# yumcyaWiz/fredholm

Measured on AMD Instinct MI355X. Metric: Msamples/s at 1920x1080, max_depth=8, higher is better.
Workload: dtype f32; 1 GPU; configs[2]: 1M random-triangle soup (PCG32 seed 0x853c49e6748fea9b), Hosek sky turbidity 3 albedo 0.3, 1920x1080, max_depth 8, seed 1; triangles=1000000, parallelism=single GPU, gather=none, post=none

## Files before the change

fredholm_amd/csrc/capi.hip:

```cpp
#include <hip/hip_runtime.h>

#include <cmath>
#include <cstdlib>
#include <cstring>

#include "../../include/fredholm/image_io.h"
#include <hip/hip_gl_interop.h>

#include "context.h"
#include "fh_bsdf.h"
#include "fh_trace.h"

#include "gen/tables.inc"

namespace fh {

static thread_local std::string g_create_error;

int fail(fh_ctx* ctx, int code, const std::string& msg)
{
  g_create_error = msg;
  if (ctx) ctx->err = msg;
  if (ctx && ctx->owner) ctx->owner->err = "member " + std::to_string(ctx->member_index) + ": " + msg;
  return code;
// ... 342 lines not shown
          for (uint32_t x = bx; x < bx + blk && x < x0 + tw && x < width; ++x) { owned.push_back(x + width * y); if (owned_xy) owned_xy->push_back(x | (y << 16)); }
  }
}

int rebuild_ownership(fh_ctx* ctx)
{
  if (ctx->d_owned) { (void)hipFree(ctx->d_owned); ctx->d_owned = nullptr; }
  if (ctx->d_owned_xy) { (void)hipFree(ctx->d_owned_xy); ctx->d_owned_xy = nullptr; }
  ctx->n_owned = 0;
  if (ctx->width == 0 || ctx->height == 0) return FH_OK;
  if (ctx->width > 65535u || ctx->height > 65535u) return fail(ctx, FH_E_UNSUPPORTED, "frames wider or higher than 65535 pixels are not supported");
  std::vector<uint32_t> owned, owned_xy;
  owned_list(ctx->width, ctx->height, ctx->tile_w, ctx->tile_h, ctx->shard_rank, ctx->shard_world, owned, &owned_xy);
  ctx->n_owned = (uint32_t)owned.size();
  FH_HIP(hipMalloc((void**)&ctx->d_owned, owned.empty() ? 16 : owned.size() * 4));
  FH_HIP(hipMalloc((void**)&ctx->d_owned_xy, owned.empty() ? 16 : owned.size() * 4));
  if (!owned.empty()) FH_HIP(hipMemcpy(ctx->d_owned, owned.data(), owned.size() * 4, hipMemcpyHostToDevice));
  if (!owned.empty()) FH_HIP(hipMemcpy(ctx->d_owned_xy, owned_xy.data(), owned_xy.size() * 4, hipMemcpyHostToDevice));
  return FH_OK;
}

}

int frame_map_ensure(fh_ctx* ctx, uint32_t world)
{
  fh_ctx::FrameMap& fm = ctx->frame_map;
  if (!(fm.d_all && fm.world == world && fm.width == ctx->width && fm.height == ctx->height && fm.tile_w == ctx->tile_w && fm.tile_h == ctx->tile_h)) {
    (void)hipStreamSynchronize(ctx->stream);
    if (fm.d_all) (void)hipFree(fm.d_all);
    fm = fh_ctx::FrameMap{};
    std::vector<uint32_t> all;
    fm.start.assign(world + 1u, 0u);
    for (uint32_t r = 0; r < world; ++r) { owned_list(ctx->width, ctx->height, ctx->tile_w, ctx->tile_h, r, world, all, nullptr); fm.start[r + 1u] = (uint32_t)all.size(); }
    FH_HIP(hipMalloc((void**)&fm.d_all, all.empty() ? 16 : all.size() * 4));
    if (!all.empty()) FH_HIP(hipMemcpy(fm.d_all, all.data(), all.size() * 4, hipMemcpyHostToDevice));
    fm.world = world; fm.width = ctx->width; fm.height = ctx->height; fm.tile_w = ctx->tile_w; fm.tile_h = ctx->tile_h;
  }
  return FH_OK;
}

uint32_t owned_count(uint32_t width, uint32_t height, uint32_t tw, uint32_t th, uint32_t rank, uint32_t world)
{
  std::vector<uint32_t> owned;
  owned_list(width, height, tw, th, rank, world, owned, nullptr);
  return (uint32_t)owned.size();
}

namespace {

__global__ void k_pack(const float* layer, const uint32_t* owned, uint32_t n, uint32_t fpp, float* packed)
{
  for (uint32_t i = blockIdx.x * blockDim.x + threadIdx.x; i < n * fpp; i += gridDim.x * blockDim.x) packed[i] = layer[(size_t)owned[i / fpp] * fpp + i % fpp];
}
__global__ void k_unpack(const float* packed, const uint32_t* owned, uint32_t n, uint32_t fpp, float* layer)
{
  for (uint32_t i = blockIdx.x * blockDim.x + threadIdx.x; i < n * fpp; i += gridDim.x * blockDim.x) layer[(size_t)owned[i / fpp] * fpp + i % fpp] = packed[i];
}
struct ShardSources { const float* packed[kMaxShardsPerLaunch]; uint32_t start[kMaxShardsPerLaunch + 1]; uint32_t world; };
__global__ void k_unpack_all(ShardSources src, const uint32_t* all_owned, uint32_t n, uint32_t fpp, float* layer)
{
  for (uint32_t i = blockIdx.x * blockDim.x + threadIdx.x; i < n * fpp; i += gridDim.x * blockDim.x) {
    const uint32_t j = i / fpp, c = i % fpp;
    uint32_t r = 0;
    while (r + 1u < src.world && j >= src.start[r + 1u]) ++r;
    layer[(size_t)all_owned[j] * fpp + c] = src.packed[r][(size_t)(j - src.start[r]) * fpp + c];
  }
}

}
}

using namespace fh;

#define CTX_CHECK(ctx)                      \
  if (!(ctx)) return FH_E_INVALID;          \
  if (hipSetDevice((ctx)->device) != hipSuccess) return fh::fail(ctx, FH_E_HIP, "hipSetDevice failed")

namespace fh {
uint64_t pool_bytes_per_path(const fh_ctx* ctx)
{
  const uint32_t sec = 2u + (ctx->has_dir ? 1u : 0u) + (ctx->n_lights > 0 ? 1u : 0u);
  const uint32_t classes = ctx->n_classes < 1u ? 1u : ctx->n_classes;
  return 64u + 16u + 8u + 4u + 64u + 48u * sec + (ctx->n_lights > 0 ? 32u : 0u) + 20u + 4u + 4u + 4u * classes;
}
}

extern "C" {

int fh_ctx_create(int device, fh_ctx** out)
{
  if (!out) return FH_E_INVALID;
  *out = nullptr;
  int n_dev = 0;
  if (hipGetDeviceCount(&n_dev) != hipSuccess || n_dev <= 0) { g_create_error = "no HIP device available: the fredholm HIP path has no CPU fallback"; return FH_E_HIP; }
  if (device < 0 || device >= n_dev) { g_create_error = "device index out of range"; return FH_E_INVALID; }
  if (hipSetDevice(device) != hipSuccess) { g_create_error = "hipSetDevice failed"; return FH_E_HIP; }
  fh_ctx* ctx = new fh_ctx;
  ctx->device = device;
  auto bail = [&](const char* what) { g_create_error = what; delete ctx; return FH_E_HIP; };
  auto make_stream = [&](hipStream_t* s) { return hipStreamCreateWithFlags(s, hipStreamNonBlocking); };
  if (make_stream(&ctx->stream) != hipSuccess) return bail("hipStreamCreate failed");
  if (hipMalloc((void**)&ctx->d_sobol, kSobolMatricesBytes) != hipSuccess) return bail("hipMalloc failed");
  if (hipMalloc((void**)&ctx->d_lut_refl, kLutReflectionBytes) != hipSuccess) return bail("hipMalloc failed");
  if (hipMalloc((void**)&ctx->d_lut_sheen, kLutSheenBytes) != hipSuccess) return bail("hipMalloc failed");
  if (hipMalloc((void**)&ctx->d_trace_counters, 32 * sizeof(unsigned long long)) != hipSuccess) return bail("hipMalloc failed");
  if (hipMalloc((void**)&ctx->d_hosek, sizeof(fh::HosekSky)) != hipSuccess || hipMemsetAsync(ctx->d_hosek, 0, sizeof(fh::HosekSky), ctx->stream) != hipSuccess) return bail("hipMalloc failed");
  if (hipMemcpy(ctx->d_sobol, kSobolMatrices, kSobolMatricesBytes, hipMemcpyHostToDevice) != hipSuccess) return bail("table upload failed");
  {
    std::vector<uint32_t> bytes((size_t)1024 * 4 * 256);
    const uint32_t* mat = kSobolMatrices;
    for (uint32_t dim = 0; dim < 1024u; ++dim)
      for (uint32_t k = 0; k < 4u; ++k) {
        uint32_t* t = &bytes[((size_t)dim * 4 + k) * 256];
        t[0] = 0u;
        for (uint32_t b = 1; b < 256u; ++b) t[b] = t[b & (b - 1u)] ^ mat[dim * 52u + 8u * k + (uint32_t)__builtin_ctz(b)];
      }
    if (hipMalloc((void**)&ctx->d_sobol_bytes, bytes.size() * sizeof(uint32_t)) != hipSuccess) return bail("hipMalloc failed");
    if (hipMemcpy(ctx->d_sobol_bytes, bytes.data(), bytes.size() * sizeof(uint32_t), hipMemcpyHostToDevice) != hipSuccess) return bail("table upload failed");
  }
  if (hipMemcpy(ctx->d_lut_refl, kLutReflection, kLutReflectionBytes, hipMemcpyHostToDevice) != hipSuccess) return bail("table upload failed");
  if (hipMemcpy(ctx->d_lut_sheen, kLutSheen, kLutSheenBytes, hipMemcpyHostToDevice) != hipSuccess) return bail("table upload failed");
  (void)hipMemsetAsync(ctx->d_trace_counters, 0, 32 * sizeof(unsigned long long), ctx->stream);
  for (int k = 0; k < 2; ++k)
    if (make_stream(&ctx->aux_stream[k]) != hipSuccess) return bail("hipStreamCreate failed");
  for (int k = 0; k < 3; ++k) {
    (void)hipHostMalloc((void**)&ctx->h_counters[k], sizeof(uint32_t) * fh::kCounterStride * 66);
    (void)hipEventCreate(&ctx->ev_counters[k]);
    (void)hipEventCreateWithFlags(&ctx->ev_gen[k], hipEventDisableTiming);
    (void)hipEventCreateWithFlags(&ctx->ev_acc[k], hipEventDisableTiming);
  }
  (void)hipEventCreateWithFlags(&ctx->ev_enter, hipEventDisableTiming);
  if (const char* e = getenv("FH_PIPELINE")) ctx->n_slots = e[0] == '0' ? 1 : (e[0] == '2' ? 2 : 3);
  {
    fh_ctx::Tunables& t = ctx->tun;
    hipDeviceProp_t prop;
    if (hipGetDeviceProperties(&prop, device) == hipSuccess && prop.multiProcessorCount > 0) t.n_cus = (uint32_t)prop.multiProcessorCount;
    int v = 0;
    if (hipDeviceGetAttribute(&v, hipDeviceAttributeMaxSharedMemoryPerMultiprocessor, device) == hipSuccess && v >= 64 * 1024) t.lds_per_cu = (uint32_t)v;
    if (hipDeviceGetAttribute(&v, hipDeviceAttributeSharedMemPerBlockOptin, device) == hipSuccess && v >= 64 * 1024) t.lds_per_block = (uint32_t)v;
    if (t.lds_per_block > t.lds_per_cu) t.lds_per_block = t.lds_per_cu;
    auto env_uint = [](const char* name, int lo, int hi, uint32_t& dst) { if (const char* e = getenv(name)) { const int v = atoi(e); if (v >= lo && v <= hi) dst = (uint32_t)v; } };
    auto env_off = [](const char* name, bool& dst) { if (const char* e = getenv(name)) dst = e[0] != '0'; };
    env_uint("FH_COOP_T", 1, 64, t.coop_flush);
    t.coop_flush_fixed = getenv("FH_COOP_T") != nullptr;
    env_off("FH_COOP", t.coop);
    env_off("FH_STREAM", t.stream);
    t.stream_forced = t.stream && getenv("FH_STREAM") != nullptr;
    env_uint("FH_STREAM_REFILL", 1, 64, t.stream_refill);
    env_uint("FH_STREAM_MIN_RAYS", 0, 65535, t.stream_min_rays);
    env_off("FH_SORT_SMALL", t.sort_small);
    env_off("FH_OVERLAP", t.overlap_secondary);
    env_off("FH_MERGE", t.merge_trace);
    env_uint("FH_SKY_BLOCKS", 0, 64, t.sky_blocks_per_cu);
    if (const char* e = getenv("FH_POISON")) t.poison_pools = e[0] == '1';
    env_off("FH_SKY_SPLIT", t.sky_split);
    env_uint("FH_SKY_SPLIT_MIN_LOG2", 0, 40, t.sky_split_min_log2);
    env_uint("FH_STACK_LDS", 1, 99, t.stack_lds_entries);
    env_uint("FH_SHADE_WGS", 2, 3, t.shade_wgs);
    env_uint("FH_STREAM_CHUNK", 16, 65535, t.stream_chunk);
    t.stream_chunk_fixed = getenv("FH_STREAM_CHUNK") != nullptr;
    if (t.stream_chunk_fixed) t.stream_chunk_closest = t.stream_chunk;
    env_uint("FH_STREAM_CHUNK_CLOSEST", 16, 65535, t.stream_chunk_closest);
    env_uint("FH_TAIL_DEPTH", 0, 64, t.tail_depth);
    env_uint("FH_TAIL_PATHS", 64, 1 << 30, t.tail_paths);
    env_off("FH_SORT", t.sort_queues);
    env_uint("FH_SORT_ONEPASS", 0, 2, t.sort_onepass);
    env_uint("FH_BOTTOM_UP", 0, 2, t.bottom_up);
    t.debug_tail = getenv("FH_DEBUG_TAIL") != nullptr;
    if (const char* e = getenv("FH_FORCE_ALPHA")) t.force_alpha = e[0] == '1';
  }
  {
    int least = 0, greatest = 0;
    const char* e = getenv("FH_SKY_PRIO");
    const bool low = !(e && e[0] == '0') && hipDeviceGetStreamPriorityRange(&least, &greatest) == hipSuccess;
    if ((low ? hipStreamCreateWithPriority(&ctx->sky_stream, hipStreamNonBlocking, least) : hipStreamCreateWithFlags(&ctx->sky_stream, hipStreamNonBlocking)) != hipSuccess) return bail("hipStreamCreate failed");
  }
  (void)hipEventCreateWithFlags(&ctx->ev_sky, hipEventDisableTiming);
  if (hipMalloc((void**)&ctx->d_split_counters, 16) != hipSuccess) return bail("hipMalloc failed");
  (void)hipMemsetAsync(ctx->d_split_counters, 0, 16, ctx->stream);
  (void)hipEventCreate(&ctx->ev_render_begin);
  (void)hipEventCreate(&ctx->ev_render_end);
  if (hipStreamSynchronize(ctx->stream) != hipSuccess) return bail("hipStreamSynchronize failed");
  *out = ctx;
  return FH_OK;
}

int fh_ctx_destroy(fh_ctx* ctx)
{
  FH_GROUP(ctx, group_destroy(ctx));
  if (!ctx) return FH_E_INVALID;
  (void)hipSetDevice(ctx->device);
  (void)hipStreamSynchronize(ctx->stream);
  pool_release(ctx);
  void* ptrs[] = {ctx->d_sample_issued, ctx->d_sobol, ctx->d_sobol_bytes, ctx->d_alpha_rec, ctx->d_lut_refl, ctx->d_lut_sheen, ctx->d_face_rec, ctx->d_face_cls, ctx->d_materials, ctx->d_lights, ctx->d_bvh2_nodes, ctx->d_bvh2_tris,
                  ctx->d_bvh8_nodes, ctx->d_bvh8_tris, ctx->d_sample_count, ctx->d_owned, ctx->d_trace_counters, ctx->d_texels, ctx->d_textures, ctx->d_srgb_lut, ctx->d_ibl,
                  ctx->d_bloom_weights, ctx->d_quirk_seen, ctx->d_quirk_aov, ctx->d_obj_vertices, ctx->d_obj_normals, ctx->d_obj_texcoords, ctx->d_obj_indices, ctx->d_face_meta, ctx->d_o2w, ctx->d_w2o,
                  ctx->d_bvh8_box, ctx->d_denoise_tmp[0], ctx->d_denoise_tmp[1], ctx->d_hosek, ctx->d_owned_xy, ctx->d_stack_spill, ctx->d_bvh8_parent, ctx->d_face_node,
                  ctx->d_moments, ctx->d_active[0], ctx->d_active[1], ctx->d_active[2], ctx->d_active[3], ctx->d_block_marks, ctx->d_active_blocks, ctx->d_sky_taken, ctx->d_sky_adaptive};
  for (void* p : ptrs)
    if (p) (void)hipFree(p);
  for (fh_ctx::ShardList& c : ctx->shard_lists)
    if (c.d_owned) (void)hipFree(c.d_owned);
  if (ctx->frame_map.d_all) (void)hipFree(ctx->frame_map.d_all);
  for (int k = 0; k < 4; ++k) if (ctx->d_split[k]) (void)hipFree(ctx->d_split[k]);
  if (ctx->d_split_counters) (void)hipFree(ctx->d_split_counters);
  if (ctx->h_active_count) (void)hipHostFree(ctx->h_active_count);
  if (ctx->sky_stream) { (void)hipStreamSynchronize(ctx->sky_stream); (void)hipStreamDestroy(ctx->sky_stream); }
  if (ctx->ev_sky) (void)hipEventDestroy(ctx->ev_sky);
  for (auto& s : ctx->spans) { (void)hipEventDestroy(s.a); (void)hipEventDestroy(s.b); }
  for (auto e : ctx->event_pool) (void)hipEventDestroy(e);
  for (auto e : ctx->ev_bounce) (void)hipEventDestroy(e);
  for (int k = 0; k < 3; ++k) {
  }
  for (int k = 0; k < 3; ++k) {
    if (ctx->h_counters[k]) (void)hipHostFree(ctx->h_counters[k]);
    (void)hipEventDestroy(ctx->ev_counters[k]);
    (void)hipEventDestroy(ctx->ev_gen[k]);
    (void)hipEventDestroy(ctx->ev_acc[k]);
  }
  (void)hipEventDestroy(ctx->ev_enter);
  for (int k = 0; k < 2; ++k) (void)hipStreamDestroy(ctx->aux_stream[k]);
  (void)hipEventDestroy(ctx->ev_render_begin);
  (void)hipEventDestroy(ctx->ev_render_end);
  (void)hipStreamDestroy(ctx->stream);
  delete ctx;
  return FH_OK;
}

const char* fh_last_error(fh_ctx* ctx) { return ctx ? ctx->err.c_str() : g_create_error.c_str(); }

int fh_set_flags(fh_ctx* ctx, uint32_t flags)
{
  FH_GROUP_EACH(ctx, kGroupCallPlain, fh_set_flags(m_, flags));
  CTX_CHECK(ctx);
  ctx->flags = flags;
  return FH_OK;
}
int fh_get_flags(fh_ctx* ctx, uint32_t* flags)
{
  FH_GROUP_LEAD(ctx);
  CTX_CHECK(ctx);
  if (!flags) return fail(ctx, FH_E_INVALID, "fh_get_flags: null argument");
  *flags = ctx->flags;
  return FH_OK;
}

int fh_set_path_pool(fh_ctx* ctx, uint32_t target)
{
  FH_GROUP_EACH(ctx, kGroupCallFrame, fh_set_path_pool(m_, target));
  CTX_CHECK(ctx);
  if (target == 0) return fail(ctx, FH_E_INVALID, "fh_set_path_pool: zero");
  (void)hipStreamSynchronize(ctx->stream);
  pool_release(ctx);
  ctx->pool_target = target;
  ctx->pool_target_by_caller = true;
  return FH_OK;
}

int fh_path_pool_bytes(fh_ctx* ctx, uint64_t* bytes_per_path, uint32_t* pools)
{
  FH_GROUP_LEAD(ctx);
  CTX_CHECK(ctx);
  if (!bytes_per_path || !pools) return fail(ctx, FH_E_INVALID, "fh_path_pool_bytes: null argument");
  *bytes_per_path = pool_bytes_per_path(ctx);
  *pools = (uint32_t)ctx->n_slots;
  return FH_OK;
}

int fh_kat_face_classes(fh_ctx* ctx, uint8_t* out, uint32_t n)
{
  FH_GROUP_REFUSE(ctx, "fh_kat_face_classes");
  CTX_CHECK(ctx);
  if (!out || n != ctx->n_faces) return fail(ctx, FH_E_INVALID, "fh_kat_face_classes: one byte per face of the uploaded scene");
  if (n) FH_HIP(hipMemcpy(out, ctx->d_face_cls, n, hipMemcpyDeviceToHost));
  return FH_OK;
}

int fh_alpha_face_counts(fh_ctx* ctx, uint32_t counts[4])
{
  FH_GROUP_LEAD(ctx);
  CTX_CHECK(ctx);
  if (!counts) return fail(ctx, FH_E_INVALID, "fh_alpha_face_counts: null argument");
  for (int k = 0; k < 4; ++k) counts[k] = ctx->alpha_face_counts[k];
  return FH_OK;
}

int fh_alpha_cell_counts(fh_ctx* ctx, uint64_t counts[3])
{
  FH_GROUP_LEAD(ctx);
  CTX_CHECK(ctx);
  if (!counts) return fail(ctx, FH_E_INVALID, "fh_alpha_cell_counts: null argument");
  for (int k = 0; k < 3; ++k) counts[k] = ctx->alpha_cell_counts[k];
  return FH_OK;
}

int fh_kat_alpha_records(fh_ctx* ctx, uint32_t* out, uint32_t n_faces)
{
  FH_GROUP_REFUSE(ctx, "fh_kat_alpha_records");
  CTX_CHECK(ctx);
  if (!out || n_faces != ctx->n_faces) return fail(ctx, FH_E_INVALID, "fh_kat_alpha_records: 32 words per face of the uploaded scene");
  if (!ctx->d_alpha_rec) { std::memset(out, 0, 128ull * n_faces); return FH_OK; }
  FH_HIP(hipMemcpy(out, ctx->d_alpha_rec, 128ull * n_faces, hipMemcpyDeviceToHost));
  return FH_OK;
}

int fh_path_pool_allocated(fh_ctx* ctx, uint64_t* bytes, uint64_t* paths)
{
  FH_GROUP(ctx, group_path_pool_allocated(ctx, bytes, paths));
  CTX_CHECK(ctx);
  if (!bytes || !paths) return fail(ctx, FH_E_INVALID, "fh_path_pool_allocated: null argument");
  *bytes = 0; *paths = 0;
  for (int k = 0; k < 3; ++k) { *bytes += ctx->pool_alloc_bytes[k]; *paths += ctx->pool[k].capacity; }
  return FH_OK;
}

int fh_set_tail_depth(fh_ctx* ctx, uint32_t depth)
{
  FH_GROUP_EACH(ctx, kGroupCallPlain, fh_set_tail_depth(m_, depth));
  CTX_CHECK(ctx);
  ctx->tail_depth = depth;
  return FH_OK;
}

int fh_scene_upload(fh_ctx* ctx, const fh_scene_desc* s)
{
  FH_GROUP_EACH(ctx, kGroupCallUpload, fh_scene_upload(m_, s));
  CTX_CHECK(ctx);
  if (!s || !s->vertices || !s->normals || !s->texcoords || !s->indices || !s->material_ids || !s->materials || s->n_materials == 0)
    return fail(ctx, FH_E_INVALID, "fh_scene_upload: missing arrays");
  for (uint32_t i = 0; i < s->n_materials; ++i) {
    const fh_material& m = s->materials[i];
    const int32_t ids[11] = {m.base_color_texture_id, m.specular_color_texture_id, m.specular_roughness_texture_id, m.metalness_texture_id, m.metallic_roughness_texture_id, m.coat_texture_id,
                             m.coat_roughness_texture_id, m.emission_texture_id, m.heightmap_texture_id, m.normalmap_texture_id, m.alpha_texture_id};
    for (int32_t id : ids)
      if (id < -1 || id >= (int32_t)s->n_textures) return fail(ctx, FH_E_INVALID, "fh_scene_upload: material references a texture id outside [0, n_textures)");
  }
  if (s->n_textures && !s->textures) return fail(ctx, FH_E_INVALID, "fh_scene_upload: n_textures > 0 but textures == NULL");
  {
    const int rc = upload_textures(ctx, s->n_textures, s->textures);
    if (rc) return rc;
  }
  ctx->h_vertices.assign(s->vertices, s->vertices + 3ull * s->n_vertices);
  ctx->h_normals.assign(s->normals, s->normals + 3ull * s->n_vertices);
  ctx->h_texcoords.assign(s->texcoords, s->texcoords + 2ull * s->n_vertices);
  ctx->h_indices.assign(s->indices, s->indices + 3ull * s->n_faces);
  ctx->h_material_ids.assign(s->material_ids, s->material_ids + s->n_faces);
  if (s->instance_ids) ctx->h_instance_ids.assign(s->instance_ids, s->instance_ids + s->n_faces);
  else ctx->h_instance_ids.clear();
  ctx->h_materials.assign(s->materials, s->materials + s->n_materials);
  if (s->n_instances && s->object_to_world && s->world_to_object) {
    ctx->h_o2w.assign(s->object_to_world, s->object_to_world + 12ull * s->n_instances);
    ctx->h_w2o.assign(s->world_to_object, s->world_to_object + 12ull * s->n_instances);
  } else {
    ctx->h_o2w.assign(kIdentity12, kIdentity12 + 12);
    ctx->h_w2o.assign(kIdentity12, kIdentity12 + 12);
  }
  const int rc = rebuild_device_scene(ctx);
  if (rc) return rc;
  ctx->scene_loaded = true;
  ctx->builder_choice = 0;
  return FH_OK;
// ... 580 lines not shown
```

fredholm_amd/csrc/context.h:

```cpp
#pragma once
#include <hip/hip_runtime.h>

#include <functional>
#include <string>
#include <vector>

#include "../../include/fredholm_hip.h"
#include "fh_device.h"

struct fh_group;

struct fh_ctx {
  fh_group* group = nullptr;
  fh_ctx* owner = nullptr;
  uint32_t member_index = 0;
  int device = 0;
  hipStream_t stream = nullptr;
  hipStream_t aux_stream[2] = {nullptr, nullptr};
  std::string err;
  uint32_t flags = 0;

  uint32_t* d_sobol = nullptr;
  uint32_t* d_sobol_bytes = nullptr;
  float* d_lut_refl = nullptr;
  float* d_lut_sheen = nullptr;

  std::vector<float> h_vertices, h_normals, h_texcoords;
  std::vector<uint32_t> h_indices, h_material_ids, h_instance_ids;
  std::vector<fh_material> h_materials;
  std::vector<float> h_o2w, h_w2o;
  bool scene_loaded = false, bvh_valid = false;

  float4* d_face_rec = nullptr;
  uint8_t* d_face_cls = nullptr;
  fh::MaterialDev* d_materials = nullptr;
  fh::AreaLightDev* d_lights = nullptr;
  float* d_obj_vertices = nullptr;
  float* d_obj_normals = nullptr;
  float* d_obj_texcoords = nullptr;
  uint32_t* d_obj_indices = nullptr;
  uint2* d_face_meta = nullptr;
  float4* d_o2w = nullptr;
  float4* d_w2o = nullptr;
  uint32_t n_xf_alloc = 0;
  std::vector<uint8_t> h_tex_alpha_cuts, h_tex_red_cuts;
  std::vector<fht_texture> h_tex_desc;
  struct HostTexture { uint32_t width = 0, height = 0, srgb = 0; std::vector<uint8_t> rgba8; };
  std::vector<HostTexture> h_tex_host;
  unsigned long long alpha_cell_counts[3] = {0, 0, 0};
  uint32_t alpha_face_counts[4] = {0, 0, 0, 0};
  uint4* d_alpha_rec = nullptr;
  uint8_t* d_texels = nullptr;
  fht_texture* d_textures = nullptr;
  float* d_srgb_lut = nullptr;
  uint32_t n_textures = 0;
  bool has_alpha = false;
  float* d_ibl = nullptr;
  uint32_t ibl_w = 0, ibl_h = 0;
  uint32_t n_faces = 0, n_lights = 0, n_materials = 0;
  uint32_t n_classes = 0;
  uint32_t class_lobes[fh::kMaxClasses] = {};

  float4* d_bvh2_nodes = nullptr;
  float4* d_bvh2_tris = nullptr;
  uint32_t bvh2_n_nodes = 0, bvh2_n_tris = 0;
  uint4* d_bvh8_nodes = nullptr;
  float4* d_bvh8_tris = nullptr;
  uint32_t bvh8_n_nodes = 0, bvh8_n_tris = 0;
  uint32_t* d_bvh8_parent = nullptr;
  uint32_t* d_face_node = nullptr;
  float4* d_bvh8_box = nullptr;
  std::vector<uint32_t> bvh8_level_start;
  bool refit_ok = false;
  double bvh8_area_built = 0.0;
  uint32_t n_refits = 0;
  uint32_t bvh8_depth = 0;
  uint32_t occupancy_key = 0xffffffffu, occupancy_blocks = 0, occupancy_blocks_secondary = 0;
  uint32_t info_blocks[2] = {0, 0}, info_entries[2] = {0, 0};
  uint32_t lds_configured_bytes = 0;
  uint32_t stream_lds_entries = 0, stream_lds_entries_secondary = 0;
  uint2* d_stack_spill = nullptr;
  size_t stack_spill_capacity = 0;
  uint32_t lds_static_max = 0;
  bool use_bvh8 = false;
  int builder_choice = 0;
  double bvh_build_ms = 0.0;
  float scene_lo[3] = {0, 0, 0}, scene_hi[3] = {0, 0, 0};

  uint32_t width = 0, height = 0;
  uint32_t* d_sample_count = nullptr;
  uint32_t* d_sample_issued = nullptr;
  uint32_t shard_rank = 0, shard_world = 1, tile_w = 32, tile_h = 32;
  uint32_t* d_owned = nullptr;
  uint32_t* d_owned_xy = nullptr;
  uint32_t n_owned = 0;
  uint32_t* d_split[4] = {nullptr, nullptr, nullptr, nullptr};
  uint32_t split_capacity = 0, n_wave_px = 0, n_sky_px = 0;
  uint32_t* d_split_counters = nullptr;
  bool split_valid = false;
  float split_key[32] = {};
  hipStream_t sky_stream = nullptr;
  hipEvent_t ev_sky = nullptr;
  struct ShardList { uint32_t rank, world, width, height, tile_w, tile_h; uint32_t* d_owned; uint32_t n_owned; };
  struct FrameMap { uint32_t world = 0, width = 0, height = 0, tile_w = 0, tile_h = 0; uint32_t* d_all = nullptr; std::vector<uint32_t> start; };
  FrameMap frame_map;
  std::vector<ShardList> shard_lists;
  bool adaptive = false;
  fh_adaptive_params adapt{};
  float2* d_moments = nullptr;
  bool accumulated = false;
  uint32_t adapt_total = 0;
  uint32_t* d_active[4] = {nullptr, nullptr, nullptr, nullptr};
  uint32_t* d_active_blocks = nullptr;
  uint32_t active_capacity = 0;
  uint32_t* h_active_count = nullptr;
  uint32_t adapt_block = 1, adapt_growth = 1;
  uint32_t* d_block_marks = nullptr;
  size_t marks_capacity = 0;
  uint32_t mark_seq = 0;
  unsigned long long* d_sky_taken = nullptr;
  bool sky_taken_pending = false;
  void* d_sky_adaptive = nullptr;

  bool has_dir = false;
  float dir_le[3] = {0, 0, 0}, dir_dir[3] = {0, 1, 0}, dir_angle = 0;
  float sky_intensity = 1.0f;
  float sun_dir[3] = {0.0f, 1.0f, 0.0f};
  bool has_hosek = false;
  fh::HosekSky hosek{};
  fh::HosekSky* d_hosek = nullptr;

  fh::PoolDev pool[3] = {};
  struct PoolShape { bool dir = false, lights = false; uint32_t classes = 0; };
  PoolShape pool_shape[3];
  std::vector<void*> pool_allocs[3];
  unsigned long long pool_alloc_bytes[3] = {0, 0, 0};
  uint32_t pool_target_default = 1u << 25, pool_target = 1u << 25;
  bool pool_target_by_caller = false;
  uint32_t pool_share = 1;
  uint32_t tail_depth = 0;
  uint32_t auto_wave_depth = 2;
  double survival[66] = {};
  uint32_t survival_n = 0;
  uint32_t* h_counters[3] = {nullptr, nullptr, nullptr};
  hipEvent_t ev_counters[3] = {nullptr, nullptr, nullptr};
  bool counters_in_flight[3] = {false, false, false};
  uint32_t counters_wave_depth[3] = {0, 0, 0};
  uint32_t counters_paths[3] = {0, 0, 0};
  int counters_bu[3] = {-1, -1, -1};
  int bu_choice = 0;
  uint32_t bu_toggle = 0;
  double bu_cost[2] = {0.0, 0.0}, bu_items[2] = {0.0, 0.0};
  unsigned long long pass_seq = 0;
  hipEvent_t ev_gen[3] = {nullptr, nullptr, nullptr}, ev_acc[3] = {nullptr, nullptr, nullptr}, ev_enter = nullptr;
  bool gen_valid[3] = {false, false, false}, acc_valid[3] = {false, false, false};
  int n_slots = 3;
  int last_slot_used = 0;
  std::vector<hipEvent_t> ev_bounce;
  uint32_t* d_quirk_seen = nullptr;
  float4* d_quirk_aov = nullptr;
  size_t quirk_pixels = 0;

  struct Tunables {
    uint32_t n_cus = 256;
    uint32_t lds_per_cu = 160u * 1024u, lds_per_block = 160u * 1024u;
    uint32_t coop_flush = 48;
    bool coop_flush_fixed = false;
    bool coop = true;
    bool stream = true;
    bool stream_forced = false;
    uint32_t stream_refill = 24;
    uint32_t stream_min_rays = 64;
    bool overlap_secondary = true;
    bool sky_split = true;
    uint32_t sky_split_min_log2 = 27;
    uint32_t sky_blocks_per_cu = 0;
    bool poison_pools = false;
    bool merge_trace = true;
    uint32_t shade_wgs = 0;
    uint32_t stack_lds_entries = 0;
    bool sort_small = false;
    uint32_t stream_chunk = 64;
    bool stream_chunk_fixed = false;
    uint32_t stream_chunk_closest = 128;
    uint32_t tail_depth = 0;
    uint32_t tail_paths = 0;
    uint32_t bottom_up = 2;
    bool sort_queues = true;
    uint32_t sort_onepass = 2;
    bool debug_tail = false;
    bool force_alpha = false;
  } tun;

  float* d_bloom_weights = nullptr;
  float bloom_sigma_cached = -1.0f, bloom_wsum = 0.0f;

  float4* d_denoise_tmp[2] = {nullptr, nullptr};
  size_t denoise_pixels = 0;

  fh_stats stats{};
  unsigned long long* d_trace_counters = nullptr;
  struct TimedSpan { hipEvent_t a, b; int kind; };
  std::vector<TimedSpan> spans;
  std::vector<hipEvent_t> event_pool;
  hipEvent_t ev_render_begin = nullptr, ev_render_end = nullptr;
  bool render_pending = false;
};

namespace fh {
int fail(fh_ctx* ctx, int code, const std::string& msg);
#define FH_HIP(call)                                                                                                   \
  do {                                                                                                                 \
    hipError_t e_ = (call);                                                                                            \
    if (e_ != hipSuccess) return fh::fail(ctx, FH_E_HIP, std::string(#call) + ": " + hipGetErrorString(e_));            \
  } while (0)

#define FH_GROUP(ctx, call) \
  if ((ctx) && (ctx)->group) return fh::call
#define FH_GROUP_EACH(ctx, kind, call) \
  if ((ctx) && (ctx)->group) return fh::group_each(ctx, kind, [&](fh_ctx* m_, uint32_t i_) { (void)i_; return call; })
#define FH_GROUP_LEAD(ctx) \
  if ((ctx) && (ctx)->group) ctx = fh::group_lead(ctx)
#define FH_GROUP_REFUSE(ctx, name) \
  if ((ctx) && (ctx)->group) return fh::fail(ctx, FH_E_UNSUPPORTED, name ": not available on a group (a plain context does hand-rolled gathers and known-answer runs)")
enum { kGroupCallPlain = 0, kGroupCallScene = 1, kGroupCallFrame = 2, kGroupCallUpload = 3 };
fh_ctx* group_lead(fh_ctx* g);
int group_each(fh_ctx* g, int kind, const std::function<int(fh_ctx*, uint32_t)>& call);
int group_destroy(fh_ctx* g);
int group_set_resolution(fh_ctx* g, uint32_t w, uint32_t h);
int group_set_tile_shard(fh_ctx* g, uint32_t rank, uint32_t world, uint32_t tw, uint32_t th);
int group_init_render_states(fh_ctx* g);
int group_render(fh_ctx* g, const fh_camera* cam, const float* bg, const fh_render_layers* layers, uint32_t n_samples, uint32_t max_depth, uint32_t seed);
int group_get_sample_counts(fh_ctx* g, uint32_t* counts);
int group_get_luminance_moments(fh_ctx* g, float* moments);
int group_active_pixel_count(fh_ctx* g, uint32_t* out);
int group_owned_pixel_count(fh_ctx* g, uint32_t* out);
int group_get_stats(fh_ctx* g, fh_stats* out);
int group_path_pool_allocated(fh_ctx* g, uint64_t* bytes, uint64_t* paths);
int frame_map_ensure(fh_ctx* ctx, uint32_t world);
uint32_t owned_count(uint32_t width, uint32_t height, uint32_t tw, uint32_t th, uint32_t rank, uint32_t world);

SceneDev scene_dev(const fh_ctx* ctx);
int bvh_build_device(fh_ctx* ctx);
int render_submit(fh_ctx* ctx, const fh_camera* cam, const float* bg, const fh_render_layers* layers, uint32_t n_samples, uint32_t max_depth, uint32_t seed);
int adaptive_upload(fh_ctx* ctx);
int adaptive_select(fh_ctx* ctx, hipStream_t st, const uint32_t* base_px, const uint32_t* base_xy, uint32_t n_base, uint32_t* n_active, const uint32_t* sky_px = nullptr,
                    const uint32_t* sky_xy = nullptr, uint32_t n_sky = 0, uint32_t* n_sky_active = nullptr);
uint32_t adaptive_to_boundary(const fh_ctx* ctx);
int pool_ensure(fh_ctx* ctx, int slot, uint32_t capacity);
uint64_t pool_bytes_per_path(const fh_ctx* ctx);
void pool_release(fh_ctx* ctx);
int kernel_info(fh_ctx* ctx, int which, uint32_t out[6]);
int post_process_submit(fh_ctx* ctx, const float* in, float* hi, float* tmp, int w, int h, const fh_post_params* pp, float* out);
int denoise_submit(fh_ctx* ctx, int w, int h, const float* beauty, const float* normal, const float* albedo, float* out, int upscale);
}
```

fredholm_amd/csrc/fh_sky.h:

```cpp
#pragma once
#include "../../include/fh_elementary.h"
#include "fh_vec.h"

namespace fh {

struct HosekSky { float cfg[3][9]; float rad[3]; };

inline float hosek_bezier(const float* m, int stride, float e)
{
  const float ie = 1.0f - e;
  return fhe_pow(ie, 5.0f) * m[0] + 5.0f * fhe_pow(ie, 4.0f) * e * m[stride] + 10.0f * fhe_pow(ie, 3.0f) * fhe_pow(e, 2.0f) * m[2 * stride] +
         10.0f * fhe_pow(ie, 2.0f) * fhe_pow(e, 3.0f) * m[3 * stride] + 5.0f * ie * fhe_pow(e, 4.0f) * m[4 * stride] + fhe_pow(e, 5.0f) * m[5 * stride];
}

inline HosekSky hosek_cook(const float* table, float turbidity, float albedo, float elevation)
{
  HosekSky st{};
  const int it = (int)turbidity;
  const float tr = turbidity - (float)it;
  const float e = fhe_pow(elevation / (kPi / 2.0f), (1.0f / 3.0f));
  for (int ch = 0; ch < 3; ++ch) {
    const float* ds = table + 1080 * ch;
    const float* dr = table + 3240 + 120 * ch;
    for (int i = 0; i < 9; ++i) {
      float c = (1.0f - albedo) * (1.0f - tr) * hosek_bezier(ds + 54 * (it - 1) + i, 9, e);
      c += albedo * (1.0f - tr) * hosek_bezier(ds + 540 + 54 * (it - 1) + i, 9, e);
      if (it != 10) {
        c += (1.0f - albedo) * tr * hosek_bezier(ds + 54 * it + i, 9, e);
        c += albedo * tr * hosek_bezier(ds + 540 + 54 * it + i, 9, e);
      }
      st.cfg[ch][i] = c;
    }
    float r = (1.0f - albedo) * (1.0f - tr) * hosek_bezier(dr + 6 * (it - 1), 1, e);
    r += albedo * (1.0f - tr) * hosek_bezier(dr + 60 + 6 * (it - 1), 1, e);
    if (it != 10) {
      r += (1.0f - albedo) * tr * hosek_bezier(dr + 6 * it, 1, e);
      r += albedo * tr * hosek_bezier(dr + 60 + 6 * it, 1, e);
    }
    st.rad[ch] = r;
  }
  return st;
}

FH_HD f3 hosek_radiance(const HosekSky& st, f3 sun_dir, float intensity, f3 v)
{
  const float theta = fhe_acos(clampf(v.y, -1.0f, 1.0f));
  const float gamma = fhe_acos(dot(sun_dir, v));
  const float cg = fhe_cos(gamma), ct = fhe_cos(theta);
  const float rayM = cg * cg;
  const float zenith = sqrt_cr(ct);
  float out[3];
#pragma unroll
  for (int ch = 0; ch < 3; ++ch) {
    const float* c = st.cfg[ch];
    const float expM = fhe_exp(c[4] * gamma);
    const float mieM = (1.0f + cg * cg) / fhe_pow1p5(1.0f + c[8] * c[8] - 2.0f * c[8] * cg);
    out[ch] = (1.0f + c[0] * fhe_exp(c[1] / (ct + 0.01f))) * (c[2] + c[3] * expM + c[5] * rayM + c[6] * mieM + c[7] * zenith) * st.rad[ch];
  }
  return intensity * mk3(out[0], out[1], out[2]);
}

}
```

fredholm_amd/csrc/render.hip:

```cpp
#include <hip/hip_runtime.h>

#include <cmath>
#include <cstdio>
#include <cstdlib>
#include <cstring>
#include <type_traits>

#include "context.h"
#include "fh_bsdf.h"
#include "fh_tonemap.h"
#include "fh_trace.h"

namespace fh {

namespace {

constexpr int kBlock = 256;
constexpr uint32_t kLutReflFloats = 16 * 16 * 2, kLutSheenFloats = 16 * 16;
constexpr uint32_t kMatLds = 32;
#ifndef FH_SECONDARY_BLOCKS_HEAVY
#define FH_SECONDARY_BLOCKS_HEAVY 5
#endif
#ifndef FH_STREAM_BLOCKS
#define FH_STREAM_BLOCKS 7
#endif
#ifndef FH_STREAM_BLOCKS_ALPHA
#define FH_STREAM_BLOCKS_ALPHA FH_STREAM_BLOCKS
#endif
#ifndef FH_STREAM_BLOCKS_CLOSEST
#define FH_STREAM_BLOCKS_CLOSEST FH_STREAM_BLOCKS
#endif
#ifndef FH_SHADE_BLOCKS
#define FH_SHADE_BLOCKS 2
#endif

template <int N>
struct SobolRows {
  uint32_t m[N][1024];
};

template <int N>
FH_D void load_sobol_rows(SobolRows<N>& rows, const uint32_t* tables, const uint32_t* dims)
{
  static_assert(kBlock == 256, "one uint4 per thread and dimension");
#pragma unroll
  for (int r = 0; r < N; ++r)
    reinterpret_cast<uint4*>(rows.m[r])[threadIdx.x] = reinterpret_cast<const uint4*>(tables + (size_t)(dims[r] & 1023u) * 1024u)[threadIdx.x];
  __syncthreads();
}

FH_D void stage_sky(FrameDev& fr, HosekSky& lds_sky)
{
  if (!fr.has_hosek) return;
  if (threadIdx.x < sizeof(HosekSky) / 4u) reinterpret_cast<float*>(&lds_sky)[threadIdx.x] = reinterpret_cast<const float*>(fr.hosek)[threadIdx.x];
  fr.hosek = &lds_sky;
}

FH_D f3 env_radiance(const FrameDev& fr, f3 d)
{
  if (fr.has_ibl) {
    const float theta = fhe_acos(clampf(d.y, -1.0f, 1.0f));
    float phi = fhe_atan2(d.z, d.x);
    if (phi < 0) phi += 2.0f * kPi;
    float o[4];
    fht_tex2d(&fr.ibl, nullptr, phi / (2.0f * kPi), theta / kPi, o);
    return fr.sky_intensity * mk3(o[0], o[1], o[2]);
  }
  return fr.has_hosek ? hosek_radiance(*fr.hosek, fr.sun_dir, fr.sky_intensity, d) : fr.bg;
}

FH_D bool camera_ray(const FrameDev& fr, const uint32_t* sobol_dim1, uint32_t image_idx, uint32_t px, uint32_t py, uint32_t n_spp, f2 u, f2 u_lens, f3& org, f3& dir);
FH_D bool camera_sample(const FrameDev& fr, const uint32_t* sobol_dim1, uint32_t image_idx, uint32_t px, uint32_t py, uint32_t n_spp, f3& org, f3& dir)
{
  return camera_ray(fr, sobol_dim1, image_idx, px, py, n_spp, cmj_draw(n_spp, image_idx, 0u, fr.seed_hash), cmj_draw(n_spp, image_idx, 1u, fr.seed_hash), org, dir);
}
FH_D bool camera_ray(const FrameDev& fr, const uint32_t* sobol_dim1, uint32_t image_idx, uint32_t px, uint32_t py, uint32_t n_spp, f2 u, f2 u_lens, f3& org, f3& dir)
{
  float uvx = (2.0f * (px + u.x) - fr.width) / fr.height;
  const float uvy = (2.0f * (py + u.y) - fr.height) / fr.height;
  uvx = -uvx;
  u = u_lens;
  const float f = fr.cam_inv_tan;
  const f3 p_sensor = mk3(uvx, uvy, 0.0f);
  const f3 p_lens_center = mk3(0.0f, 0.0f, f);
  const f2 pd = fr.cam_lens_radius * concentric_disk(u);
  const f3 p_lens = p_lens_center + mk3(pd.x, pd.y, 0.0f);
  const f3 s2c = normalize(p_lens_center - p_sensor);
  const f3 p_object = p_sensor + (fr.cam_a_plus_b / s2c.z) * s2c;
  org = xform_point(fr.cam_xf, p_lens);
  f3 d = normalize(p_object - p_lens);
  d.z *= -1.0f;
  dir = xform_dir(fr.cam_xf, d);
  const uint32_t sidx = image_idx + n_spp * fr.width * fr.height;
  const float rr = sobol_draw_bytes(sobol_dim1, sidx, 1u, fr.seed_hash);
  return fr.max_depth > 0 && !(rr >= 1.0f);
}

constexpr int kGenChunks = 4;
__global__ void __launch_bounds__(kBlock) k_generate(FrameDev fr, PoolDev pool, const uint32_t* issued, const uint32_t* owned, const uint32_t* owned_xy, uint32_t n_owned)
{
  __shared__ SobolRows<1> rows;
  __shared__ HosekSky s_sky;
  stage_sky(fr, s_sky);
  const uint32_t dims[1] = {1u};
  load_sobol_rows<1>(rows, fr.sobol_bytes, dims);
  const uint32_t stride = gridDim.x * blockDim.x * kGenChunks;
  const uint32_t k = blockIdx.y;
  __shared__ uint32_t s_reserve[2][5 * kGenChunks];
  uint32_t iter = 0;
  for (uint32_t base = blockIdx.x * blockDim.x * kGenChunks; base < n_owned; base += stride) {
   uint32_t packed = 0u;
   uint32_t* const scratch = s_reserve[iter & 1u];
#pragma unroll 1
   for (int c = 0; c < kGenChunks; ++c) {
    const uint32_t i = base + (uint32_t)c * blockDim.x + threadIdx.x;
    const bool valid = i < n_owned;
    const uint32_t p = k * n_owned + i;
    bool enter = false;
    if (valid) {
      const uint32_t image_idx = owned[i];
      const uint32_t n_spp = issued[image_idx] + k;
      const uint32_t xy = owned_xy[i];
      f3 org, dir;
      const bool alive = camera_sample(fr, rows.m[0], image_idx, xy & 0xffffu, xy >> 16, n_spp, org, dir);
      RayPre rp;
      rp.o = org;
      rp.inv = safe_reciprocal(dir);
      float tn;
      enter = alive && slab_test(rp, fr.scene_lo.x, fr.scene_lo.y, fr.scene_lo.z, fr.scene_hi.x, fr.scene_hi.y, fr.scene_hi.z, 1e9f, tn);
      if (enter) {
        pool.ray_o[p] = mk4(org, 1e9f);
        pool.ray_d[p] = mk4(dir, 0.0f);
        pool.thr[p] = make_float4(1.0f, 1.0f, 1.0f, 0.0f);
        pool.rad[p] = make_float4(0.0f, 0.0f, 0.0f, 0.0f);
        pool.pixel[p] = image_idx;
        pool.nspp[p] = n_spp;
        pool.flags[p] = 0u;
      } else {
        const f3 r = alive ? mk3(0.0f) + mk3(1.0f) * env_radiance(fr, dir) : mk3(0.0f);
        pool.rad[p] = mk4(r, 0.0f);
        pool.flags[p] = 2u;
      }
    }
    const unsigned long long m = __ballot(enter);
    if ((threadIdx.x & 63u) == 0u) scratch[4 * c + (threadIdx.x >> 6)] = (uint32_t)__popcll(m);
    packed |= ((enter ? 0x80u : 0u) | (uint32_t)__popcll(m & ((1ull << (threadIdx.x & 63u)) - 1ull))) << (8 * c);
   }
   __syncthreads();
   if (threadIdx.x == 0u) {
     uint32_t total = 0;
     for (uint32_t c = 0; c < 4u * kGenChunks; ++c) { const uint32_t v = scratch[c]; scratch[c] = total; total += v; }
     scratch[4 * kGenChunks] = total ? atomicAdd(&pool.counters[CNT_RAD], total) : 0u;
   }
   __syncthreads();
   ++iter;
#pragma unroll
   for (int c = 0; c < kGenChunks; ++c)
     if ((packed >> (8 * c)) & 0x80u)
       pool.q_rad[0][scratch[4 * kGenChunks] + scratch[4 * c + (threadIdx.x >> 6)] + ((packed >> (8 * c)) & 63u)] = k * n_owned + base + (uint32_t)c * blockDim.x + threadIdx.x;
  }
}

__global__ void __launch_bounds__(kBlock) k_bump_issued(uint32_t* issued, const uint32_t* owned, uint32_t n_owned, uint32_t n_batch)
{
  const uint32_t i = blockIdx.x * blockDim.x + threadIdx.x;
  if (i < n_owned) issued[owned[i]] += n_batch;
}

struct SplitDev {
  f3 centre;
  float radius;
  float far;
  uint32_t* wave_px; uint32_t* wave_xy; uint32_t* sky_px; uint32_t* sky_xy;
  uint32_t* counters;
};
__global__ void __launch_bounds__(kBlock) k_split_pixels(FrameDev fr, SplitDev sp, const uint32_t* owned, const uint32_t* owned_xy, uint32_t n_owned)
{
  __shared__ uint32_t s_reserve[2][10];
  uint32_t iter = 0;
  for (uint32_t base = blockIdx.x * blockDim.x; base < n_owned; base += gridDim.x * blockDim.x) {
    const uint32_t i = base + threadIdx.x;
    bool sky = false, wave = false;
    uint32_t px = 0, xy = 0;
    if (i < n_owned) {
      px = owned[i]; xy = owned_xy[i];
      const float x = (float)(xy & 0xffffu) + 0.5f, y = (float)(xy >> 16) + 0.5f;
      const float uvx = -(2.0f * x - (float)fr.width) / (float)fr.height, uvy = (2.0f * y - (float)fr.height) / (float)fr.height;
      const float f = fr.cam_inv_tan, k = 1.0f - fr.cam_a_plus_b / f;
      const f3 a0 = mk3(0.0f, 0.0f, f), b0 = mk3(k * uvx, k * uvy, 2.0f * f - fr.cam_a_plus_b);
      const f3 ab = b0 - a0;
      const float L = length(ab);
      const float m = fabsf(fr.cam_lens_radius) + 1.41421357f * fabsf(k) / (float)fr.height * 1.001f;
      const f3 w = sp.centre - a0;
      const float tau = dot(w, ab) / L;
      const float d0 = sqrt_cr(fmaxf(dot(w, w) - tau * tau, 0.0f));
      const float q = 1.0f - (m / L) * (m / L);
      const float nearest = d0 * sqrt_cr(fmaxf(q, 0.0f)) - fabsf(fr.cam_lens_radius) - m * fabsf(tau) / L;
      sky = L > 0.0f && q > 0.0f && nearest > sp.radius * 1.001f + 1e-3f * (length(w) + 1.0f);
      if (!sky && L > m * 1.01f) {
        const float d = (fabsf(fr.cam_lens_radius) + m * (sp.far + fabsf(fr.cam_lens_radius)) / (L - m)) * 1.001f + 1e-3f * (sp.far + 1.0f);
        const f3 o = xform_point(fr.cam_xf, a0), dir = xform_dir(fr.cam_xf, (1.0f / L) * ab);
        float tn = -3.0e38f, tf = 3.0e38f;
        bool miss = false;
        const float oo[3] = {o.x, o.y, o.z}, dd[3] = {dir.x, dir.y, dir.z}, lo[3] = {fr.scene_lo.x - d, fr.scene_lo.y - d, fr.scene_lo.z - d}, hi[3] = {fr.scene_hi.x + d, fr.scene_hi.y + d, fr.scene_hi.z + d};
#pragma unroll
        for (int a = 0; a < 3; ++a) {
          if (fabsf(dd[a]) < 1e-12f) miss = miss || oo[a] < lo[a] || oo[a] > hi[a];
          else {
            const float t0 = (lo[a] - oo[a]) / dd[a], t1 = (hi[a] - oo[a]) / dd[a];
            tn = fmaxf(tn, fminf(t0, t1)); tf = fminf(tf, fmaxf(t0, t1));
          }
        }
        miss = miss || tn - 1e-3f * (fabsf(tn) + sp.far) > tf + 1e-3f * (fabsf(tf) + sp.far);
        sky = miss && dd[0] == dd[0] && dd[1] == dd[1] && dd[2] == dd[2] && d == d;
      }
      wave = !sky;
    }
    uint32_t* const counters2[2] = {sp.counters, sp.counters + 1};
    const bool act[2] = {wave, sky};
    uint32_t pos[2];
    block_queue_reserve<2>(counters2, act, pos, s_reserve[iter & 1u]);
    ++iter;
    if (wave) { sp.wave_px[pos[0]] = px; sp.wave_xy[pos[0]] = xy; }
    if (sky) { sp.sky_px[pos[1]] = px; sp.sky_xy[pos[1]] = xy; }
  }
}

struct AdaptiveDev {
  float2* moments;
  const uint32_t* count;
  float threshold, floor;
  uint32_t min_samples, step;
  uint32_t growth, b0;
  uint32_t* marks;
  uint32_t tag, block_shift, blocks_x, width;
};

FH_D bool adaptive_boundary(const AdaptiveDev& ad, uint32_t n)
{
  if (ad.growth == 1u) return n >= ad.min_samples && n % ad.step == 0u;
  if (ad.b0 == 0u || n < ad.b0 || n % ad.b0 != 0u) return false;
  const uint32_t q = n / ad.b0;
  return (q & (q - 1u)) == 0u;
}

FH_D bool adaptive_converged(const AdaptiveDev& ad, uint32_t n, float m1, float m2)
{
  if (!adaptive_boundary(ad, n)) return false;
  float d = m2 - m1 * m1;
  if (d < 0.0f) d = 0.0f;
  const float var = d * ((float)n / (float)(n - 1u));
  const float e2 = var / (float)n;
  const float ref = m1 > ad.floor ? m1 : ad.floor;
  const float t = ad.threshold * ref;
  return ad.threshold > 0.0f && e2 <= t * t;
}

FH_D void moments_update(float& m1, float& m2, float coef, float fn, f3 radiance)
{
  const float y = luminance_rgb(radiance.x, radiance.y, radiance.z);
  m1 = coef * (fn * m1 + y);
  m2 = coef * (fn * m2 + y * y);
}

struct SkyAdaptive {
  AdaptiveDev ad;
  uint32_t* violations;
  unsigned long long* taken;
};
template <bool ADAPTIVE>
__global__ void __launch_bounds__(kBlock) k_sky_pixels(FrameDev fr, LayersDev layers, uint32_t* issued, const uint32_t* sky_px, const uint32_t* sky_xy, uint32_t n_sky, uint32_t n_samples,
                                                     std::conditional_t<ADAPTIVE, const SkyAdaptive*, uint32_t*> violations_or_adaptive)
{
  uint32_t* violations;
  AdaptiveDev ad{};
  if constexpr (ADAPTIVE) { ad = violations_or_adaptive->ad; violations = violations_or_adaptive->violations; }
  else violations = violations_or_adaptive;
  unsigned long long n_taken = 0;
  __shared__ SobolRows<1> rows;
  __shared__ HosekSky s_sky;
  stage_sky(fr, s_sky);
  const uint32_t dims[1] = {1u};
  load_sobol_rows<1>(rows, fr.sobol_bytes, dims);
  for (uint32_t i = blockIdx.x * blockDim.x + threadIdx.x; i < n_sky; i += gridDim.x * blockDim.x) {
    const uint32_t image_idx = sky_px[i], xy = sky_xy[i];
    const uint32_t first = issued[image_idx];
    uint32_t n_spp = layers.sample_count[image_idx];
    f3 beauty = mk3(layers.beauty[image_idx]), position = mk3(layers.position[image_idx]), normal = mk3(layers.normal[image_idx]), albedo = mk3(layers.albedo[image_idx]);
    float depth = layers.depth[image_idx];
    const float4 tc4 = layers.texcoord[image_idx];
    float tcx = tc4.x, tcy = tc4.y;
    bool violated = false;
    uint32_t blk = 0xffffffffu;
    CmjBlock b0{}, b1{};
    float2 m = make_float2(0.0f, 0.0f);
    if constexpr (ADAPTIVE) m = ad.moments[image_idx];
    uint32_t taken = n_samples;
    for (uint32_t k = 0; k < n_samples; ++k) {
      if constexpr (ADAPTIVE) { if (!ad.marks && adaptive_converged(ad, n_spp, m.x, m.y)) { taken = k; break; } }
      f3 org, dir;
      const uint32_t n = first + k;
      if ((n >> 4) != blk) {
        blk = n >> 4;
        b0 = cmj_block(blk, image_idx, 0u, fr.seed_hash);
        b1 = cmj_block(blk, image_idx, 1u, fr.seed_hash);
      }
      const bool alive = camera_ray(fr, rows.m[0], image_idx, xy & 0xffffu, xy >> 16, n, cmj_draw_in_block(b0, n), cmj_draw_in_block(b1, n), org, dir);
      RayPre rp;
      rp.o = org;
      rp.inv = safe_reciprocal(dir);
      float tn;
      violated = violated || (alive && slab_test(rp, fr.scene_lo.x, fr.scene_lo.y, fr.scene_lo.z, fr.scene_hi.x, fr.scene_hi.y, fr.scene_hi.z, 1e9f, tn));
      const f3 L = alive ? mk3(0.0f) + mk3(1.0f) * env_radiance(fr, dir) : mk3(0.0f);
      const f3 radiance = bad3(L) ? mk3(0.0f) : L;
      const float coef = 1.0f / (n_spp + 1.0f);
      const float fn = (float)n_spp;
      beauty = coef * (fn * beauty + radiance);
      position = coef * (fn * position + mk3(0.0f));
      normal = coef * (fn * normal + mk3(0.0f));
      depth = coef * (fn * depth + 0.0f);
      tcx = coef * (fn * tcx + 0.0f);
      tcy = coef * (fn * tcy + 0.0f);
      albedo = coef * (fn * albedo + mk3(0.0f));
      if constexpr (ADAPTIVE) moments_update(m.x, m.y, coef, fn, radiance);
      n_spp++;
    }
    if (violated) atomicAdd(violations, 1u);
    if constexpr (ADAPTIVE) { ad.moments[image_idx] = m; n_taken += taken; issued[image_idx] = first + taken; }
    else issued[image_idx] = first + n_samples;
    layers.sample_count[image_idx] = n_spp;
    layers.beauty[image_idx] = mk4(beauty, 1.0f);
    layers.position[image_idx] = mk4(position, 1.0f);
    layers.normal[image_idx] = mk4(normal, 1.0f);
    layers.depth[image_idx] = depth;
    layers.texcoord[image_idx] = make_float4(tcx, tcy, 0.0f, 1.0f);
    layers.albedo[image_idx] = mk4(albedo, 1.0f);
  }  if constexpr (ADAPTIVE) {
    __shared__ unsigned long long s_taken;
    if (threadIdx.x == 0u) s_taken = 0ull;
    __syncthreads();
    if (n_taken) atomicAdd(&s_taken, n_taken);
    __syncthreads();
    if (threadIdx.x == 0u && s_taken) atomicAdd(violations_or_adaptive->taken, s_taken);
  }
}

FH_D bool adaptive_unconverged(const AdaptiveDev& ad, uint32_t image_idx)
{
  const float2 m = ad.moments[image_idx];
  return !adaptive_converged(ad, ad.count[image_idx], m.x, m.y);
}

FH_D bool adaptive_active(const AdaptiveDev& ad, uint32_t image_idx)
{
  if (ad.marks) {
    const uint32_t y = image_idx / ad.width, x = image_idx - y * ad.width;
    return ad.marks[(y >> ad.block_shift) * ad.blocks_x + (x >> ad.block_shift)] == ad.tag;
  }
  return adaptive_unconverged(ad, image_idx);
}

__global__ void __launch_bounds__(kBlock) k_adaptive_mark(AdaptiveDev ad, const uint32_t* owned_px, const uint32_t* owned_xy, uint32_t n_owned)
{
  const uint32_t i = blockIdx.x * kBlock + threadIdx.x;
  uint32_t key = 0xffffffffu;
  if (i < n_owned && adaptive_unconverged(ad, owned_px[i])) {
    const uint32_t xy = owned_xy[i];
    key = ((xy >> 16) >> ad.block_shift) * ad.blocks_x + ((xy & 0xffffu) >> ad.block_shift);
  }
  const uint32_t below = __shfl_up(key, 1);
  if (key != 0xffffffffu && ((threadIdx.x & 63u) == 0u || below != key)) ad.marks[key] = ad.tag;
}

__global__ void __launch_bounds__(kBlock) k_adaptive_count(AdaptiveDev ad, const uint32_t* base_px, uint32_t n_base, uint32_t* blocks)
{
  __shared__ uint32_t s_w[kBlock / 64];
  const uint32_t i = blockIdx.x * kBlock + threadIdx.x;
  const bool act = i < n_base && adaptive_active(ad, base_px[i]);
  const unsigned long long m = __ballot(act);
  if ((threadIdx.x & 63u) == 0u) s_w[threadIdx.x >> 6] = (uint32_t)__popcll(m);
  __syncthreads();
  if (threadIdx.x == 0u) blocks[blockIdx.x] = s_w[0] + s_w[1] + s_w[2] + s_w[3];
}

__global__ void __launch_bounds__(kBlock) k_adaptive_scan(uint32_t* blocks, uint32_t n_blocks)
{
  __shared__ uint32_t s[kBlock];
  const uint32_t per = (n_blocks + kBlock - 1u) / kBlock;
  const uint32_t lo = threadIdx.x * per < n_blocks ? threadIdx.x * per : n_blocks;
  const uint32_t hi = lo + per < n_blocks ? lo + per : n_blocks;
  uint32_t sum = 0;
  for (uint32_t b = lo; b < hi; ++b) sum += blocks[b];
  s[threadIdx.x] = sum;
  __syncthreads();
  if (threadIdx.x == 0u) {
    uint32_t t = 0;
    for (uint32_t k = 0; k < (uint32_t)kBlock; ++k) { const uint32_t v = s[k]; s[k] = t; t += v; }
    blocks[n_blocks] = t;
  }
  __syncthreads();
  uint32_t run = s[threadIdx.x];
  for (uint32_t b = lo; b < hi; ++b) { const uint32_t v = blocks[b]; blocks[b] = run; run += v; }
}

__global__ void __launch_bounds__(kBlock) k_adaptive_select(AdaptiveDev ad, const uint32_t* base_px, const uint32_t* base_xy, uint32_t n_base, const uint32_t* blocks,
                                                          uint32_t* out_px, uint32_t* out_xy)
{
  __shared__ uint32_t s_w[kBlock / 64];
  const uint32_t i = blockIdx.x * kBlock + threadIdx.x;
  const uint32_t lane = threadIdx.x & 63u, wave = threadIdx.x >> 6;
  uint32_t px = 0;
  bool act = false;
  if (i < n_base) { px = base_px[i]; act = adaptive_active(ad, px); }
  const unsigned long long m = __ballot(act);
  if (lane == 0u) s_w[wave] = (uint32_t)__popcll(m);
  __syncthreads();
  uint32_t pos = blocks[blockIdx.x] + (uint32_t)__popcll(m & ((1ull << lane) - 1ull));
  for (uint32_t w = 0; w < wave; ++w) pos += s_w[w];
  if (act) { out_px[pos] = px; out_xy[pos] = base_xy[i]; }
}

template <bool COUNT, bool WIDE, bool ALPHA>
__global__ void __launch_bounds__(kBlock) k_trace_closest_static(SceneDev sc, PoolDev pool, uint32_t depth, TraceCounters tc)
{
  const uint32_t* cnt = pool.counters + depth * kCounterStride;
  const uint32_t count = cnt[CNT_RAD];
  const uint32_t* q = pool.q_rad[depth & 1u];
  uint32_t nn = 0, nt = 0, nr = 0;
  WaveSteps ws;
  for (uint32_t i = blockIdx.x * blockDim.x + threadIdx.x; i < count; i += gridDim.x * blockDim.x) {
    const uint32_t p = q[i];
    if (COUNT) nr++;
    const float4 o = pool.ray_o[p], d = pool.ray_d[p];
    HitRec h;
    const uint32_t nn0 = nn;
    if (WIDE) traverse_bvh8<false, COUNT, false, ALPHA>(sc.bvh8, mk3(o), mk3(d), o.w, h, nn, nt, &ws, nullptr, 0, &sc);
    else traverse_bvh2<false, COUNT, ALPHA>(sc.bvh2, mk3(o), mk3(d), o.w, h, nn, nt, &sc);
    if (COUNT) { const uint32_t k = nn - nn0; int b = 0; while (b < 7 && k > (8u << b)) ++b; atomicAdd(tc.hist + b, 1ull); }
    pool.hit[p] = make_float4(h.t, h.u, h.v, __uint_as_float(h.prim));
    pool.q_prim[i] = h.prim;
  }
  if (COUNT) {
    atomicAdd(tc.nodes, (unsigned long long)nn);
    atomicAdd(tc.tris, (unsigned long long)nt);
    atomicAdd(tc.rays, (unsigned long long)nr);
    if (ws.node) atomicAdd(tc.wave_nodes, (unsigned long long)ws.node);
    if (ws.tri) atomicAdd(tc.wave_tris, (unsigned long long)ws.tri);
  }
}

template <bool COUNT, bool ALPHA>
__global__ void __launch_bounds__(kBlock) k_trace_closest_coop(SceneDev sc, PoolDev pool, uint32_t depth, TraceCounters tc, uint32_t flush)
{
  extern __shared__ __attribute__((aligned(16))) uint2 lds_stack[];
  __shared__ __attribute__((aligned(16))) unsigned char lds[(kBlock / 64) * kCoopLdsBytesPerWave];
  const CoopLds cl = coop_lds(lds, threadIdx.x >> 6);
  const uint32_t* cnt = pool.counters + depth * kCounterStride;
  const uint32_t count = cnt[CNT_RAD];
  const uint32_t* q = pool.q_rad[depth & 1u];
  uint32_t nn = 0, nt = 0, nr = 0;
  WaveSteps ws;
  for (uint32_t base = blockIdx.x * blockDim.x + (threadIdx.x & ~63u); base < count; base += gridDim.x * blockDim.x) {
    const uint32_t i = base + (threadIdx.x & 63u);
    const bool valid = i < count;
    const uint32_t p = valid ? q[i] : 0u;
    if (COUNT && valid) nr++;
    const float4 o = valid ? pool.ray_o[p] : make_float4(0.0f, 0.0f, 0.0f, 0.0f), d = valid ? pool.ray_d[p] : make_float4(0.0f, 0.0f, 1.0f, 0.0f);
    HitRec h;
    const uint32_t nn0 = nn;
    traverse_bvh8_coop<false, COUNT, true, ALPHA>(sc.bvh8, valid, mk3(o), mk3(d), o.w, h, nn, nt, &ws, cl, flush, lds_stack, (int)sc.bvh8.depth, &sc);
    if (COUNT && valid) { const uint32_t k = nn - nn0; int b = 0; while (b < 7 && k > (8u << b)) ++b; atomicAdd(tc.hist + b, 1ull); }
    if (valid) { pool.hit[p] = make_float4(h.t, h.u, h.v, __uint_as_float(h.prim)); pool.q_prim[i] = h.prim; }
  }
  if (COUNT) {
    atomicAdd(tc.nodes, (unsigned long long)nn);
    atomicAdd(tc.tris, (unsigned long long)nt);
    atomicAdd(tc.rays, (unsigned long long)nr);
    if (ws.node) atomicAdd(tc.wave_nodes, (unsigned long long)ws.node);
    if (ws.tri) atomicAdd(tc.wave_tris, (unsigned long long)ws.tri);
  }
}


struct HistPack {
  unsigned long long w[2] = {0ull, 0ull};
  FH_D void add(uint32_t nodes) { int b = 0; while (b < 7 && nodes > (8u << b)) ++b; if (b < 4) w[0] += 1ull << (16 * b); else w[1] += 1ull << (16 * (b - 4)); }
  FH_D void flush(unsigned long long* hist) const
  {
    for (int b = 0; b < 8; ++b) { const unsigned long long v = (w[b >> 2] >> (16 * (b & 3))) & 0xffffull; if (v) atomicAdd(hist + b, v); }
  }
};

FH_D uint32_t stream_chunk_for(uint32_t count, uint32_t chunk)
{
  const uint32_t lo = chunk & 0xffffu, hi = chunk >> 16;
  if (hi <= lo) return lo;
  const uint32_t share = count / (gridDim.x * (kBlock / 64u) * 4u);
  const uint32_t c = share & ~63u;
  return c < lo ? lo : (c > hi ? hi : c);
}

FH_D bool stream_block_idle(uint32_t count, uint32_t min_rays) { return blockIdx.x != 0u && (unsigned long long)blockIdx.x * (kBlock / 64u) * min_rays >= count; }

template <bool ALPHA>
struct AlphaLds { static FH_D void attach(CoopLds&) {} };
template <>
struct AlphaLds<true> {
  static FH_D void attach(CoopLds& cl)
  {
    __shared__ __attribute__((aligned(16))) unsigned char lds_alpha[kAlphaLdsBytesPerBlock];
    alpha_ring(cl, lds_alpha, threadIdx.x >> 6);
  }
};

FH_D bool sec_present(const float4& d4) { return __float_as_uint(d4.w) != 0u; }
FH_D uint32_t start_node_of(const float4& d4) { const uint32_t b = __float_as_uint(d4.w); return b ? b - 1u : 0u; }

template <bool COUNT>
struct ClosestStream {
  static constexpr bool all_any = false;
  static constexpr bool can_climb = false;
  const PoolDev& pool;
  const uint32_t* q;
  ChunkFeed feed;
  uint32_t p = 0, qi = 0;
  uint32_t start = 0;
  uint32_t n_rays = 0;
  unsigned long long* hist;
  HistPack hp;
  FH_D ClosestStream(const PoolDev& pl, const uint32_t* qq, const ChunkFeed& f, unsigned long long* hs) : pool(pl), q(qq), feed(f), hist(hs) {}
  FH_D bool advance(f3&, f3&, float&, bool&) { return false; }
  FH_D bool take(uint32_t i, f3& o, f3& d, float& tmax, bool& any)
  {
    if (i >= feed.end) return false;
    p = q[i];
    qi = i;
    const float4 o4 = pool.ray_o[p], d4 = pool.ray_d[p];
    o = mk3(o4); d = mk3(d4); tmax = o4.w; any = false;
    start = start_node_of(d4);
    if (COUNT) n_rays++;
    return true;
  }
  FH_D void commit(bool, const HitRec& h, uint32_t nodes)
  {
    pool.hit[p] = make_float4(h.t, h.u, h.v, __uint_as_float(h.prim));
    pool.q_prim[qi] = h.prim;
    if (COUNT) hp.add(nodes);
  }
  FH_D bool drained() const { return feed.drained(); }
  FH_D bool followup() const { return false; }
  FH_D uint32_t start_node() const { return start; }
};

template <bool COUNT, bool ALPHA>
__global__ void __launch_bounds__(kBlock, COUNT ? 1 : FH_STREAM_BLOCKS_CLOSEST) k_trace_closest_stream(SceneDev sc, PoolDev pool, uint32_t depth, TraceCounters tc, uint32_t flush, uint32_t refill, uint32_t chunk, uint32_t min_rays,
                                                                 StackSpill spill)
{
  __shared__ __attribute__((aligned(16))) unsigned char lds[(kBlock / 64) * kCoopLdsBytesPerWave];
  const uint32_t count = pool.counters[depth * kCounterStride + CNT_RAD];
  if (stream_block_idle(count, min_rays)) return;
  const ClockStamp stamp;
  CoopLds cl = coop_lds(lds, threadIdx.x >> 6);
  AlphaLds<AlphaDefer<false, ALPHA>::value>::attach(cl);
  uint32_t nn = 0, nt = 0;
  WaveSteps ws;
  ClosestStream<COUNT> pol(pool, pool.q_rad[depth & 1u], ChunkFeed(pool.counters + depth * kCounterStride + CNT_CUR_CLOSEST, count, stream_chunk_for(count, chunk)), tc.hist);
  extern __shared__ __attribute__((aligned(16))) uint2 lds_stack[];
  traverse_stream<false, COUNT, true, ALPHA>(sc.bvh8, pol, nn, nt, &ws, cl, flush, refill, lds_stack, (int)sc.bvh8.depth, &sc, spill);
  stamp.commit(tc.clk);
  if (COUNT) {
    atomicAdd(tc.nodes, (unsigned long long)nn);
    atomicAdd(tc.tris, (unsigned long long)nt);
    atomicAdd(tc.rays, (unsigned long long)pol.n_rays);
    pol.hp.flush(tc.hist);
    if (ws.node) atomicAdd(tc.wave_nodes, (unsigned long long)ws.node);
    if (ws.tri) atomicAdd(tc.wave_tris, (unsigned long long)ws.tri);
  }
}

constexpr int kRouteChunks = 8;
__global__ void __launch_bounds__(kBlock) k_route(SceneDev sc, PoolDev pool, uint32_t depth, uint32_t n_classes, unsigned long long* hit_counter)
{
  __shared__ uint32_t wave_cnt[kMaxClasses][kRouteChunks * (kBlock / 64)];
  __shared__ uint32_t block_base[kMaxClasses];
  uint32_t* cnt = pool.counters + depth * kCounterStride;
  const uint32_t count = cnt[CNT_RAD];
  const uint32_t* q = pool.q_rad[depth & 1u];
  const uint32_t lane = threadIdx.x & 63u, wave = threadIdx.x >> 6;
  for (uint32_t base = blockIdx.x * blockDim.x * kRouteChunks; base < count; base += gridDim.x * blockDim.x * kRouteChunks) {
    uint32_t p[kRouteChunks], cls[kRouteChunks], rank[kRouteChunks];
#pragma unroll
    for (int c = 0; c < kRouteChunks; ++c) {
      const uint32_t i = base + (uint32_t)c * blockDim.x + threadIdx.x;
      p[c] = 0u; cls[c] = 0xffu; rank[c] = 0u;
      if (i < count) {
        p[c] = q[i];
        const uint32_t prim = pool.q_prim[i];
        if (prim != 0xffffffffu) cls[c] = sc.face_cls[prim] & 0x1fu;
      }
    }
#pragma unroll
    for (int c = 0; c < kRouteChunks; ++c)
      for (uint32_t k = 0; k < n_classes; ++k) {
        const unsigned long long m = __ballot(cls[c] == k);
        if (lane == 0) wave_cnt[k][c * (kBlock / 64) + wave] = (uint32_t)__popcll(m);
        if (cls[c] == k) rank[c] = (uint32_t)__popcll(m & ((1ull << lane) - 1ull));
      }
    __syncthreads();
    if (threadIdx.x < n_classes) {
      uint32_t total = 0;
      for (uint32_t w = 0; w < kRouteChunks * (kBlock / 64); ++w) { const uint32_t v = wave_cnt[threadIdx.x][w]; wave_cnt[threadIdx.x][w] = total; total += v; }
      block_base[threadIdx.x] = total ? atomicAdd(&cnt[CNT_CLS + threadIdx.x], total) : 0u;
      if (hit_counter && total) atomicAdd(hit_counter, (unsigned long long)total);
    }
    __syncthreads();
#pragma unroll
    for (int c = 0; c < kRouteChunks; ++c)
      if (cls[c] < n_classes) pool.q_cls[(size_t)cls[c] * pool.capacity + block_base[cls[c]] + wave_cnt[cls[c]][c * (kBlock / 64) + wave] + rank[c]] = p[c];
    __syncthreads();
  }
}

__global__ void __launch_bounds__(kBlock) k_miss_primary(FrameDev fr, PoolDev pool)
{
  __shared__ HosekSky s_sky;
  stage_sky(fr, s_sky);
  __syncthreads();
  const uint32_t count = pool.counters[CNT_RAD];
  const uint32_t* q = pool.q_rad[0];
  for (uint32_t i = blockIdx.x * blockDim.x + threadIdx.x; i < count; i += gridDim.x * blockDim.x) {
    if (pool.q_prim[i] != 0xffffffffu) continue;
    const uint32_t p = q[i];
    if (pool.flags[p] & 4u) continue;
    const f3 T = mk3(pool.thr[p]);
    const f3 d = mk3(pool.ray_d[p]);
    const f3 r = mk3(pool.rad[p]) + T * env_radiance(fr, d);
    pool.rad[p] = mk4(r, 0.0f);
  }
}

FH_D int tex_id(const MaterialDev& m, int word) { return __float_as_int(m.w[word]); }

FH_D MatParams load_params(const SceneDev& sc, const MaterialDev& m, float tu, float tv)
{
  MatParams p;
  p.diffuse = m.w[0];
  p.base_color = tex_id(m, 4) >= 0 ? tex_rgb(sc, tex_id(m, 4), tu, tv) : mk3(m.w[1], m.w[2], m.w[3]);
  p.diffuse_roughness = m.w[5];
  p.specular = m.w[6];
  p.specular_color = tex_id(m, 10) >= 0 ? tex_rgb(sc, tex_id(m, 10), tu, tv) : mk3(m.w[7], m.w[8], m.w[9]);
  p.specular_roughness = clampf(tex_id(m, 12) >= 0 ? tex_rgba(sc, tex_id(m, 12), tu, tv).x : m.w[11], 0.01f, 1.0f);
  p.metalness = tex_id(m, 14) >= 0 ? tex_rgba(sc, tex_id(m, 14), tu, tv).x : m.w[13];
  if (tex_id(m, 15) >= 0) {
    const float4 mr = tex_rgba(sc, tex_id(m, 15), tu, tv);
    p.specular_roughness = clampf(mr.y, 0.01f, 1.0f);
    p.metalness = clampf(mr.z, 0.0f, 1.0f);
  }
  p.coat = clampf(tex_id(m, 17) >= 0 ? tex_rgba(sc, tex_id(m, 17), tu, tv).x : m.w[16], 0.0f, 1.0f);
  p.coat_color = mk3(1.0f, 1.0f, 1.0f);
  p.coat_roughness = clampf(tex_id(m, 22) >= 0 ? tex_rgba(sc, tex_id(m, 22), tu, tv).y : m.w[21], 0.0f, 1.0f);
  p.transmission = m.w[23];
  p.transmission_color = mk3(m.w[24], m.w[25], m.w[26]);
  p.sheen = m.w[27];
  p.sheen_color = mk3(m.w[28], m.w[29], m.w[30]);
  p.sheen_roughness = m.w[31];
  p.subsurface = m.w[32];
  p.subsurface_color = mk3(m.w[33], m.w[34], m.w[35]);
  p.thin_walled = m.w[36];
  return p;
}

FH_D f3 emission_of(const SceneDev& sc, const MaterialDev& m, float tu, float tv)
{
  return tex_id(m, 41) >= 0 ? tex_rgb(sc, tex_id(m, 41), tu, tv) : mk3(m.w[38], m.w[39], m.w[40]);
}

FH_D void store_secondary(const PoolDev& pool, uint32_t slot, uint32_t p, f3 o, float tmax, f3 d, bool active, f3 c, uint32_t start_bits = 1u)
{
  const size_t k = pool.sec_at(slot, p);
  pool.sec[k + 1] = mk4(d, __uint_as_float(active ? start_bits : 0u));
  if (!active) return;
  pool.sec[k] = mk4(o, tmax);
  pool.sec[k + 2] = mk4(c, 0.0f);
}


struct BounceSlots {
  uint32_t has_lights;
  uint32_t dim_area, dim_light, dim_next, dim_rr;
  uint32_t slot_dir, slot_sky, slot_area, slot_light, slot_next;
  FH_D void set(const FrameDev& fr, uint32_t n_lights, uint32_t depth)
  {
    has_lights = n_lights > 0 ? 1u : 0u;
    const uint32_t dim0 = 1u + depth * fr.n1;
    dim_area = dim0 + 1u;
    dim_light = dim0 + 1u + has_lights;
    dim_next = dim_light + 1u;
    dim_rr = 1u + (depth + 1u) * fr.n1;
    const uint32_t slot0 = 2u + depth * fr.n2;
    slot_dir = slot0;
    slot_sky = slot0 + fr.has_dir;
    slot_area = slot_sky + 1u;
    slot_light = slot_sky + 1u + has_lights;
    slot_next = slot_light + 1u;
  }
  FH_D void load_rows(SobolRows<4>& rows, const uint32_t* tables) const
  {
    const uint32_t dims[4] = {dim_area, dim_light, dim_next, dim_rr};
    load_sobol_rows<4>(rows, tables, dims);
  }
};

struct SecRay { f3 o; float tmax; f3 d; bool active; f3 c; };

FH_D bool contributes(f3 c) { return !(c.x == 0.0f && c.y == 0.0f && c.z == 0.0f); }

struct ShadeOut {
  bool emissive_done = false;
  bool shaded = false;
  bool cont = false;
  f3 L;
  f3 T;
  SecRay sec[SEC_COUNT];
  f3 lp_T, lp_f;
  float lp_cos, lp_pdf;
  f3 next_o, next_d;
  FH_D ShadeOut() { for (uint32_t k = 0; k < SEC_COUNT; ++k) sec[k].active = false; }
  FH_D void aov(f3, f3, f3, float, float) {}
  FH_D void emissive(f3 l) { L = l; emissive_done = true; }
  FH_D void secondary(uint32_t slot, f3 o, float tmax, f3 d, bool active, f3 c) { shaded = true; sec[slot] = SecRay{o, tmax, d, active, c}; }
  FH_D void light_pending(f3 t, float c, f3 f, float pdf) { lp_T = t; lp_cos = c; lp_f = f; lp_pdf = pdf; }
  FH_D void next(f3 o, f3 d, f3 t) { cont = true; next_o = o; next_d = d; T = t; }
  FH_D void start_node(uint32_t) {}
};

struct PoolSink {
  const PoolDev& pool;
  uint32_t p;
  float hit_t;
  bool shaded = false, cont = false;
  f3 origin;
  uint32_t start_bits;
  FH_D PoolSink(const PoolDev& pl, uint32_t slot, float t, uint32_t sb = 1u) : pool(pl), p(slot), hit_t(t), origin(mk3(0.0f)), start_bits(sb) {}
  FH_D void aov(f3 position, f3 normal, f3 albedo, float u, float v)
  {
    pool.aov_position[p] = mk4(position, 0.0f);
    pool.aov_normal[p] = mk4(normal, 0.0f);
    pool.aov_albedo[p] = mk4(albedo, 0.0f);
    pool.aov_texdepth[p] = make_float4(u, v, hit_t, 0.0f);
    pool.flags[p] |= 1u;
  }
  FH_D void emissive(f3 l) { pool.rad[p] = mk4(l, 0.0f); }
  FH_D void start_node(uint32_t bits) { start_bits = bits ? bits : 1u; }
  FH_D void secondary(uint32_t slot, f3 o, float tmax, f3 d, bool active, f3 c)
  {
    store_secondary(pool, slot, p, o, tmax, d, active, c, start_bits);
    if (!shaded) origin = o;
    shaded = true;
  }
  FH_D void light_pending(f3 t, float c, f3 f, float pdf) { pool.lp_a[p] = mk4(t, c); pool.lp_b[p] = mk4(f, pdf); }
  FH_D void next(f3 o, f3 d, f3 t)
  {
    pool.ray_o[p] = mk4(o, 1e9f);
    pool.ray_d[p] = mk4(d, __uint_as_float(start_bits));
    pool.thr[p] = mk4(t, 0.0f);
    if (!shaded) origin = o;
    cont = true;
  }
};

template <uint32_t LOBES, class Sink>
FH_D void shade_hit(const SceneDev& sc, const FrameDev& fr, const SobolRows<4>& rows, const BounceSlots& bs, uint32_t depth, float4 hit, f3 rd, f3 T, f3 L, uint32_t image_idx, uint32_t n_spp,
                    Sink& out, bool first = true)
{
  const uint32_t has_lights = bs.has_lights;
  const uint32_t prim = __float_as_uint(hit.w);
  const float bu = hit.y, bv = hit.z;
// ... 2 lines not shown
  const float4 r0 = sc.face_rec[kFaceRec * (size_t)prim], r1 = sc.face_rec[kFaceRec * (size_t)prim + 1], r2 = sc.face_rec[kFaceRec * (size_t)prim + 2];
  const float4 r3 = sc.face_rec[kFaceRec * (size_t)prim + 3], r4 = sc.face_rec[kFaceRec * (size_t)prim + 4], r5 = sc.face_rec[kFaceRec * (size_t)prim + 5];
  const float4 r6 = sc.face_rec[kFaceRec * (size_t)prim + 6];
  out.start_node(sc.face_node ? __float_as_uint(r6.z) : 0u);
  const f3 p0 = mk3(r0), p1 = mk3(r1), p2 = mk3(r2);
  const float bw = 1.0f - bu - bv;
  const f3 x = bw * p0 + bu * p1 + bv * p2;
  f3 ng = normalize(cross(p1 - p0, p2 - p0));
  f3 ns = normalize(bw * mk3(r3) + bu * mk3(r4) + bv * mk3(r5));
  const float tu = bw * r0.w + bu * r2.w + bv * r4.w;
  const float tv = bw * r1.w + bu * r3.w + bv * r5.w;
  const bool entering = dot(-rd, ng) > 0;
  ns = entering ? ns : -ns;
  ng = entering ? ng : -ng;
  f3 tangent, bitangent;
  onb(ns, tangent, bitangent);
  const MaterialDev& mat = sc.materials[__float_as_uint(r6.x)];
  const MatParams sp = load_params(sc, mat, tu, tv);
  const f3 ns_geo = ns, tangent_geo = tangent, bitangent_geo = bitangent;
  if (tex_id(mat, 42) >= 0) {
    const fht_texture& hm = sc.textures[tex_id(mat, 42)];
    const float du = 1.0f / hm.width, dv = 1.0f / hm.height;
    const float hv = tex_rgba(sc, tex_id(mat, 42), tu, tv).x;
    const float dfdu = tex_rgba(sc, tex_id(mat, 42), tu + du, tv).x - hv;
    const float dfdv = tex_rgba(sc, tex_id(mat, 42), tu, tv + dv).x - hv;
    tangent = normalize(tangent_geo + dfdu * ns_geo);
    bitangent = normalize(bitangent_geo + dfdv * ns_geo);
    ns = normalize(cross(tangent, bitangent));
  }
  if (tex_id(mat, 43) >= 0) {
    f3 value = tex_rgb(sc, tex_id(mat, 43), tu, tv);
    value = 2.0f * value - 1.0f;
    ns = normalize(to_world(value, tangent_geo, bitangent_geo, ns_geo));
    onb(ns, tangent, bitangent);
  }

  if (depth == 0 && first) {
    out.aov(x, ns, sp.base_color, tu, tv);
    if (mat.emissive) {
      out.emissive(L + T * emission_of(sc, mat, tu, tv));
      return;
    }
  }
  const f3 wo = to_local(-rd, tangent, ns, bitangent);
  Bsdf<LOBES> bsdf;
  bsdf.init(wo, sp, entering, fr.lut);
  const f3 so = offset_origin(x, ng);

  if (fr.has_dir) {
    const f2 pdisk = concentric_disk(cmj_draw(n_spp, image_idx, bs.slot_dir, fr.seed_hash));
    f3 t, b;
    onb(fr.dir_dir, t, b);
    const f3 pl = 1e9f * fr.dir_dir + fr.dir_disk_radius * (t * pdisk.x + b * pdisk.y);
    const f3 sd = normalize(pl - so);
    const f3 wi = to_local(sd, tangent, ns, bitangent);
    const f3 f = bsdf.eval(wo, wi);
    const float pdf = 1.0f;
    const float w = pdf / (pdf + bsdf.eval_pdf(wo, wi));
    const f3 c = clamp01(T * w * f * abs_cos(wi) / pdf) * fr.dir_le;
    out.secondary(SEC_DIR, so, 1e9f - 0.001f, sd, contributes(c), c);
  }
  {
    const f3 wi = cosine_hemisphere(cmj_draw(n_spp, image_idx, bs.slot_sky, fr.seed_hash));
    const f3 sd = to_world(wi, tangent, ns, bitangent);
    const f3 f = bsdf.eval(wo, wi);
    const float pdf = abs_cos(wi) / kPi;
    const float w = pdf / (pdf + bsdf.eval_pdf(wo, wi));
    const f3 c = clamp01(T * w * f * abs_cos(wi) / pdf) * env_radiance(fr, sd);
    out.secondary(SEC_SKY, so, 1e9f - 0.001f, sd, contributes(c), c);
  }
  if (has_lights) {
    const float u1 = sobol_draw_bytes(rows.m[0], sidx, bs.dim_area, fr.seed_hash);
    const f2 u2 = cmj_draw(n_spp, image_idx, bs.slot_area, fr.seed_hash);
    uint32_t li = (uint32_t)(u1 * sc.n_lights);
    li = li < sc.n_lights - 1u ? li : sc.n_lights - 1u;
    const AreaLightDev lt = sc.lights[li];
    const f2 bc = triangle_barycentric(u2);
    const float4 l0 = sc.face_rec[kFaceRec * (size_t)lt.face], l1 = sc.face_rec[kFaceRec * (size_t)lt.face + 1], l2 = sc.face_rec[kFaceRec * (size_t)lt.face + 2];
    const float4 l3 = sc.face_rec[kFaceRec * (size_t)lt.face + 3], l4 = sc.face_rec[kFaceRec * (size_t)lt.face + 4], l5 = sc.face_rec[kFaceRec * (size_t)lt.face + 5];
    const float lw = 1.0f - bc.x - bc.y;
    const f3 lp = lw * mk3(l0) + bc.x * mk3(l1) + bc.y * mk3(l2);
    const f3 ln = lw * mk3(l3) + bc.x * mk3(l4) + bc.y * mk3(l5);
    const float area = 0.5f * length(cross(mk3(l1) - mk3(l0), mk3(l2) - mk3(l0)));
    const MaterialDev& lm = sc.materials[lt.material];
    const f3 le = emission_of(sc, lm, lw * l0.w + bc.x * l2.w + bc.y * l4.w, lw * l1.w + bc.x * l3.w + bc.y * l5.w);
    const float pdf_area = 1.0f / (sc.n_lights * area);
    const f3 sd = normalize(lp - so);
    const float r = length(lp - so);
    const bool facing = dot(-sd, ln) > 0.0f;
    const f3 wi = to_local(sd, tangent, ns, bitangent);
    const f3 f = bsdf.eval(wo, wi);
    const float pdf = r * r / fabsf(dot(-sd, ln)) * pdf_area;
    const float w = pdf / (pdf + bsdf.eval_pdf(wo, wi));
    const f3 c = clamp01(T * w * f * abs_cos(wi) / pdf) * le;
    out.secondary(SEC_AREA, so, r - 0.001f, sd, facing && contributes(c), c);
  }
  {
    f3 f;
    float pdf;
    const float u1 = sobol_draw_bytes(rows.m[1], sidx, bs.dim_light, fr.seed_hash);
    const f2 u2 = cmj_draw(n_spp, image_idx, bs.slot_light, fr.seed_hash);
    const f3 wi = bsdf.sample(wo, u1, u2, f, pdf);
    const f3 ld = to_world(wi, tangent, ns, bitangent);
    const bool transmitted = dot(ld, ng) < 0;
    const f3 lo = offset_origin(x, transmitted ? -ng : ng);
    if (has_lights) {
      out.light_pending(T, abs_cos(wi), f, pdf);
      out.secondary(SEC_LIGHT, lo, 1e9f, ld, true, mk3(0.0f));
    } else {
      const float pdf_light = abs_cos(wi) / kPi;
      const float w = pdf / (pdf + pdf_light);
      const f3 c = clamp01(T * w * f * abs_cos(wi) / pdf) * env_radiance(fr, ld);
      out.secondary(SEC_LIGHT, lo, 1e9f, ld, contributes(c), c);
    }
  }
  {
    f3 f;
    float pdf;
    const float u1 = sobol_draw_bytes(rows.m[2], sidx, bs.dim_next, fr.seed_hash);
    const f2 u2 = cmj_draw(n_spp, image_idx, bs.slot_next, fr.seed_hash);
    const f3 wi = bsdf.sample(wo, u1, u2, f, pdf);
    const f3 wd = to_world(wi, tangent, ns, bitangent);
    f3 Tn = T;
    Tn *= f * abs_cos(wi) / pdf;
    const bool transmitted = dot(wd, ng) < 0;
    const f3 no = offset_origin(x, transmitted ? -ng : ng);
    if (!bad3(Tn) && depth + 1u < fr.max_depth) {
      const float prr = clampf(lum(Tn), 0.0f, 1.0f);
      const float u = sobol_draw_bytes(rows.m[3], sidx, bs.dim_rr, fr.seed_hash);
      if (!(u >= prr)) out.next(no, wd, Tn / prr);
    }
  }
}

FH_D uint32_t spread3(uint32_t v) { return (v & 1u) | ((v & 2u) << 2) | ((v & 4u) << 4) | ((v & 8u) << 6); }
FH_D uint32_t cell_of(const FrameDev& fr, f3 p)
{
  const float m = (float)((1u << kCellBits) - 1u);
  const float fx = fminf(fmaxf((p.x - fr.scene_lo.x) * fr.cell_scale.x, 0.0f), m), fy = fminf(fmaxf((p.y - fr.scene_lo.y) * fr.cell_scale.y, 0.0f), m),
              fz = fminf(fmaxf((p.z - fr.scene_lo.z) * fr.cell_scale.z, 0.0f), m);
  return spread3((uint32_t)fx) | (spread3((uint32_t)fy) << 1) | (spread3((uint32_t)fz) << 2);
}

constexpr int kSortBlock = 1024;
FH_D void block_share(uint32_t n, uint32_t& lo, uint32_t& hi)
{
  const uint32_t per = (n + gridDim.x - 1u) / gridDim.x;
  lo = blockIdx.x * per < n ? blockIdx.x * per : n;
  hi = lo + per < n ? lo + per : n;
}

__global__ void __launch_bounds__(kSortBlock) k_cell_hist(const uint32_t* count_ptr, const uint16_t* keys, uint32_t* hist)
{
  __shared__ uint32_t h[kCells];
  for (uint32_t b = threadIdx.x; b < kCells; b += kSortBlock) h[b] = 0u;
  __syncthreads();
  uint32_t lo, hi;
  block_share(*count_ptr, lo, hi);
  for (uint32_t i = lo + threadIdx.x; i < hi; i += kSortBlock) atomicAdd(&h[keys[i] & (kCells - 1u)], 1u);
  __syncthreads();
  for (uint32_t b = threadIdx.x; b < kCells; b += kSortBlock)
    if (h[b]) atomicAdd(&hist[b], h[b]);
}

__global__ void __launch_bounds__(kSortBlock) k_cell_scan(uint32_t* hist, uint32_t* cursor)
{
  __shared__ uint32_t part[kSortBlock];
  constexpr uint32_t per = kCells / kSortBlock;
  uint32_t v[per], sum = 0;
  for (uint32_t k = 0; k < per; ++k) { v[k] = hist[threadIdx.x * per + k]; hist[threadIdx.x * per + k] = 0u; sum += v[k]; }
  part[threadIdx.x] = sum;
  __syncthreads();
  for (uint32_t off = 1; off < kSortBlock; off <<= 1) {
    const uint32_t add = threadIdx.x >= off ? part[threadIdx.x - off] : 0u;
    __syncthreads();
    part[threadIdx.x] += add;
    __syncthreads();
  }
  uint32_t run = part[threadIdx.x] - sum;
  for (uint32_t k = 0; k < per; ++k) { cursor[threadIdx.x * per + k] = run; run += v[k]; }
}

__global__ void __launch_bounds__(kSortBlock) k_cell_scatter(const uint32_t* count_ptr, const uint32_t* q_in, const uint16_t* keys, uint32_t* cursor, uint32_t* q_out)
{
  __shared__ uint32_t h[kCells];
  __shared__ uint32_t base[kCells];
  for (uint32_t b = threadIdx.x; b < kCells; b += kSortBlock) h[b] = 0u;
  __syncthreads();
  uint32_t lo, hi;
  block_share(*count_ptr, lo, hi);
  for (uint32_t i = lo + threadIdx.x; i < hi; i += kSortBlock) atomicAdd(&h[keys[i] & (kCells - 1u)], 1u);
  __syncthreads();
  for (uint32_t b = threadIdx.x; b < kCells; b += kSortBlock) {
    base[b] = h[b] ? atomicAdd(&cursor[b], h[b]) : 0u;
    h[b] = 0u;
  }
  __syncthreads();
  for (uint32_t i = lo + threadIdx.x; i < hi; i += kSortBlock) {
    const uint32_t b = keys[i] & (kCells - 1u);
    q_out[base[b] + atomicAdd(&h[b], 1u)] = q_in[i];
  }
}

template <uint32_t LOBES, int BLOCKS = FH_SHADE_BLOCKS>
__global__ void __launch_bounds__(kBlock, (LOBES == L_ALL ? 1 : BLOCKS)) k_shade(SceneDev sc, FrameDev fr, PoolDev pool, uint32_t cls, uint32_t depth)
{
  if (blockIdx.x * blockDim.x >= pool.counters[depth * kCounterStride + CNT_CLS + cls]) return;
  __shared__ SobolRows<4> rows;
  __shared__ float s_lut[kLutReflFloats + kLutSheenFloats];
  __shared__ MaterialDev s_mat[kMatLds];
  for (uint32_t i = threadIdx.x; i < kLutReflFloats; i += blockDim.x) s_lut[i] = fr.lut.reflection[i];
  for (uint32_t i = threadIdx.x; i < kLutSheenFloats; i += blockDim.x) s_lut[kLutReflFloats + i] = fr.lut.sheen[i];
  fr.lut.reflection = s_lut;
  fr.lut.sheen = s_lut + kLutReflFloats;
  if (sc.n_materials <= kMatLds) {
    const uint32_t* src = reinterpret_cast<const uint32_t*>(sc.materials);
    uint32_t* dst = reinterpret_cast<uint32_t*>(s_mat);
    for (uint32_t i = threadIdx.x; i < sc.n_materials * (uint32_t)(sizeof(MaterialDev) / 4); i += blockDim.x) dst[i] = src[i];
    sc.materials = s_mat;
  }
  __shared__ float s_srgb[256];
  if (sc.n_textures) {
    s_srgb[threadIdx.x] = sc.srgb_lut[threadIdx.x];
    sc.srgb_lut = s_srgb;
  }
  __shared__ HosekSky s_sky;
  stage_sky(fr, s_sky);
  BounceSlots bs;
  bs.set(fr, sc.n_lights, depth);
  bs.load_rows(rows, fr.sobol_bytes);

  uint32_t* cnt = pool.counters + depth * kCounterStride;
  uint32_t* cnt_next = cnt + kCounterStride;
  const uint32_t count = cnt[CNT_CLS + cls];
  const uint32_t* q = pool.q_cls + (size_t)cls * pool.capacity;
  const uint32_t qnext = (depth + 1u) & 1u;
  const uint32_t stride = gridDim.x * blockDim.x;
  __shared__ uint32_t s_reserve[2][10];
  uint32_t iter = 0;
  for (uint32_t base = blockIdx.x * blockDim.x; base < count; base += stride) {
    const uint32_t i = base + threadIdx.x;
    const bool valid = i < count;
    bool shaded = false, cont = false;
    uint32_t p = 0, cell = 0;
    if (valid) {
      p = q[i];
      const float4 hit = pool.hit[p];
      PoolSink o(pool, p, hit.x);
      const bool first = depth != 0 || (pool.flags[p] & 4u) == 0u;
      const f3 L = depth == 0u ? mk3(pool.rad[p]) : mk3(0.0f);
      shade_hit<LOBES>(sc, fr, rows, bs, depth, hit, mk3(pool.ray_d[p]), mk3(pool.thr[p]), L, pool.pixel[p], pool.nspp[p], o, first);
      shaded = o.shaded;
      cont = o.cont;
      if (shaded || cont) cell = cell_of(fr, o.origin);
    }
    uint32_t* const counters2[2] = {&cnt[CNT_SEC], &cnt_next[CNT_RAD]};
    const bool act[2] = {shaded, cont};
    uint32_t pos[2];
    block_queue_reserve<2>(counters2, act, pos, s_reserve[iter & 1u]);
    ++iter;
    if (shaded) { pool.q_sec[pos[0]] = p; pool.key_sec[pos[0]] = (uint16_t)cell; }
    if (cont) { pool.q_rad[qnext][pos[1]] = p; pool.key_rad[pos[1]] = (uint16_t)cell; }
  }
}

FH_D f3 resolve_light_ray(const SceneDev& sc, const FrameDev& fr, f3 T, float cosw, f3 f, float pdf, f3 ro, f3 ld, bool hit, const HitRec& h)
{
  f3 le = mk3(0.0f);
  float pdf_light = cosw / kPi;
  bool add = false;
  if (hit) {
    if (sc.face_cls[h.prim] & 0x80u) {
      const size_t fb = kFaceRec * (size_t)h.prim;
      const float4 l0 = sc.face_rec[fb], l1 = sc.face_rec[fb + 1], l2 = sc.face_rec[fb + 2], l3 = sc.face_rec[fb + 3], l4 = sc.face_rec[fb + 4], l5 = sc.face_rec[fb + 5];
      const float lw = 1.0f - h.u - h.v;
      const f3 lp = lw * mk3(l0) + h.u * mk3(l1) + h.v * mk3(l2);
      const f3 ln = lw * mk3(l3) + h.u * mk3(l4) + h.v * mk3(l5);
      if (dot(-ld, ln) > 0.0f) {
        const MaterialDev& lm = sc.materials[__float_as_uint(sc.face_rec[fb + 6].x)];
        le = emission_of(sc, lm, lw * l0.w + h.u * l2.w + h.v * l4.w, lw * l1.w + h.u * l3.w + h.v * l5.w);
        const float area = 0.5f * length(cross(mk3(l1) - mk3(l0), mk3(l2) - mk3(l0)));
        const f3 dl = lp - ro;
        const float r2 = dot(dl, dl);
        const float pdf_area = 1.0f / (sc.n_lights * area);
        pdf_light = r2 / fabsf(dot(-ld, ln)) * pdf_area;
        add = true;
      }
    }
  } else {
    le = env_radiance(fr, ld);
    add = true;
  }
  if (!add) return mk3(0.0f);
  const float w = pdf / (pdf + pdf_light);
  return clamp01(T * w * f * cosw / pdf) * le;
}

template <bool COUNT, bool WIDE, bool LIGHTS, bool ALPHA>
__global__ void __launch_bounds__(kBlock) k_trace_secondary_static(SceneDev sc, FrameDev fr, PoolDev pool, uint32_t depth, TraceCounters tc)
{
  extern __shared__ __attribute__((aligned(16))) uint2 lds_stack[];
  __shared__ HosekSky s_sky;
  if (LIGHTS) { stage_sky(fr, s_sky); __syncthreads(); }
  const uint32_t count = pool.counters[depth * kCounterStride + CNT_SEC];
  constexpr bool has_lights = LIGHTS;
  uint32_t nn = 0, nt = 0, nr = 0;
  WaveSteps ws;
  for (uint32_t i = blockIdx.x * blockDim.x + threadIdx.x; i < count; i += gridDim.x * blockDim.x) {
    const uint32_t p = pool.q_sec[i];
    f3 L = mk3(pool.rad[p]);
#pragma unroll
    for (uint32_t slot = SEC_DIR; slot <= SEC_LIGHT; ++slot) {
      if (slot == SEC_DIR && !fr.has_dir) continue;
      if (slot == SEC_AREA && !has_lights) continue;
      const size_t k = pool.sec_at(slot, p);
      const float4 d = pool.sec[k + 1];
      if (!sec_present(d)) continue;
      const float4 o = pool.sec[k];
      HitRec h;
      if (COUNT) nr++;
      if (slot == SEC_LIGHT && has_lights) {
        const bool hit = WIDE ? traverse_bvh8<false, COUNT, true, ALPHA>(sc.bvh8, mk3(o), mk3(d), o.w, h, nn, nt, &ws, lds_stack, (int)sc.bvh8.depth, &sc)
                              : traverse_bvh2<false, COUNT, ALPHA>(sc.bvh2, mk3(o), mk3(d), o.w, h, nn, nt, &sc);
        const float4 la = pool.lp_a[p], lb = pool.lp_b[p];
        L += resolve_light_ray(sc, fr, mk3(la), la.w, mk3(lb), lb.w, mk3(o), mk3(d), hit, h);
      } else {
        const uint32_t nn0 = nn;
        const bool occluded = WIDE ? traverse_bvh8<true, COUNT, true, ALPHA>(sc.bvh8, mk3(o), mk3(d), o.w, h, nn, nt, &ws, lds_stack, (int)sc.bvh8.depth, &sc)
                                   : traverse_bvh2<true, COUNT, ALPHA>(sc.bvh2, mk3(o), mk3(d), o.w, h, nn, nt, &sc);
        if (COUNT) { const uint32_t kk = nn - nn0; int b = 0; while (b < 7 && kk > (8u << b)) ++b; atomicAdd(tc.hist + b, 1ull); }
        if (!occluded) L += mk3(pool.sec[k + 2]);
      }
    }
    pool.rad[p] = mk4(L, 0.0f);
  }
  if (COUNT) {
    atomicAdd(tc.nodes, (unsigned long long)nn);
    atomicAdd(tc.tris, (unsigned long long)nt);
    atomicAdd(tc.rays, (unsigned long long)nr);
    if (ws.node) atomicAdd(tc.wave_nodes, (unsigned long long)ws.node);
    if (ws.tri) atomicAdd(tc.wave_tris, (unsigned long long)ws.tri);
  }
}

template <bool COUNT, bool LIGHTS, bool ALPHA>
__global__ void __launch_bounds__(kBlock, COUNT ? 1 : (LIGHTS ? 5 : 6)) k_trace_secondary_coop(SceneDev sc, FrameDev fr, PoolDev pool, uint32_t depth, TraceCounters tc, uint32_t flush)
{
  extern __shared__ __attribute__((aligned(16))) uint2 lds_stack[];
  __shared__ __attribute__((aligned(16))) unsigned char lds[(kBlock / 64) * kCoopLdsBytesPerWave];
  const CoopLds cl = coop_lds(lds, threadIdx.x >> 6);
  __shared__ HosekSky s_sky;
  if (LIGHTS) { stage_sky(fr, s_sky); __syncthreads(); }
  const uint32_t count = pool.counters[depth * kCounterStride + CNT_SEC];
  constexpr bool has_lights = LIGHTS;
  uint32_t nn = 0, nt = 0, nr = 0;
  WaveSteps ws;
  for (uint32_t base = blockIdx.x * blockDim.x + (threadIdx.x & ~63u); base < count; base += gridDim.x * blockDim.x) {
    const uint32_t i = base + (threadIdx.x & 63u);
    const bool in_range = i < count;
    const uint32_t p = in_range ? pool.q_sec[i] : 0u;
    f3 L = in_range ? mk3(pool.rad[p]) : mk3(0.0f);
#pragma unroll
    for (uint32_t slot = SEC_DIR; slot <= SEC_LIGHT; ++slot) {
      if (slot == SEC_DIR && !fr.has_dir) continue;
      if (slot == SEC_AREA && !has_lights) continue;
      const size_t k = pool.sec_at(slot, p);
      const float4 d = in_range ? pool.sec[k + 1] : make_float4(0.0f, 0.0f, 1.0f, 0.0f);
      const bool valid = in_range && sec_present(d);
      if (__ballot(valid) == 0ull) continue;
      const float4 o = valid ? pool.sec[k] : make_float4(0.0f, 0.0f, 0.0f, 0.0f);
      HitRec h;
      if (COUNT && valid) nr++;
      if (slot == SEC_LIGHT && has_lights) {
        const bool hit = traverse_bvh8_coop<false, COUNT, true, ALPHA>(sc.bvh8, valid, mk3(o), mk3(d), o.w, h, nn, nt, &ws, cl, flush, lds_stack, (int)sc.bvh8.depth, &sc);
        if (valid) {
          const float4 la = pool.lp_a[p], lb = pool.lp_b[p];
          L += resolve_light_ray(sc, fr, mk3(la), la.w, mk3(lb), lb.w, mk3(o), mk3(d), hit, h);
        }
      } else {
        const uint32_t nn0 = nn;
        const bool occluded = traverse_bvh8_coop<true, COUNT, true, ALPHA>(sc.bvh8, valid, mk3(o), mk3(d), o.w, h, nn, nt, &ws, cl, flush, lds_stack, (int)sc.bvh8.depth, &sc);
        if (COUNT && valid) { const uint32_t kk = nn - nn0; int b = 0; while (b < 7 && kk > (8u << b)) ++b; atomicAdd(tc.hist + b, 1ull); }
        if (valid && !occluded) L += mk3(pool.sec[k + 2]);
      }
    }
    if (in_range) pool.rad[p] = mk4(L, 0.0f);
  }
  if (COUNT) {
    atomicAdd(tc.nodes, (unsigned long long)nn);
    atomicAdd(tc.tris, (unsigned long long)nt);
    atomicAdd(tc.rays, (unsigned long long)nr);
    if (ws.node) atomicAdd(tc.wave_nodes, (unsigned long long)ws.node);
    if (ws.tri) atomicAdd(tc.wave_tris, (unsigned long long)ws.tri);
  }
}

template <bool COUNT, bool LIGHTS>
struct SecondaryStream {
  static constexpr bool all_any = !LIGHTS;
  static constexpr bool can_climb = true;
  const SceneDev& sc;
  const FrameDev& fr;
  const PoolDev& pool;
  ChunkFeed feed;
  uint32_t p = 0, slot = 0;
  uint32_t start = 0;
  bool active = false;
  f3 L;
  uint32_t n_rays = 0;
  unsigned long long* hist;
  HistPack hp;
  FH_D SecondaryStream(const SceneDev& s, const FrameDev& f, const PoolDev& pl, const ChunkFeed& cf, unsigned long long* hs) : sc(s), fr(f), pool(pl), feed(cf), L(mk3(0.0f)), hist(hs) {}
  FH_D bool scan(uint32_t from, f3& o, f3& d, float& tmax, bool& any)
  {
    for (uint32_t s = from; s <= SEC_LIGHT; ++s) {
      if (s == SEC_DIR && !fr.has_dir) continue;
      if (s == SEC_AREA && !LIGHTS) continue;
      const size_t k = pool.sec_at(s, p);
      const float4 d4 = pool.sec[k + 1];
      if (!sec_present(d4)) continue;
      const float4 o4 = pool.sec[k];
      o = mk3(o4); d = mk3(d4); tmax = o4.w;
      start = start_node_of(d4);
      any = !(s == SEC_LIGHT && LIGHTS);
      slot = s;
      if (COUNT) n_rays++;
      return true;
    }
    return false;
  }
  FH_D void finish() { if (active) { pool.rad[p] = mk4(L, 0.0f); active = false; } }
  FH_D bool advance(f3& o, f3& d, float& tmax, bool& any)
  {
    if (!active) return false;
    if (scan(slot + 1u, o, d, tmax, any)) return true;
    finish();
    return false;
  }
  FH_D bool take(uint32_t i, f3& o, f3& d, float& tmax, bool& any)
  {
    if (i >= feed.end) return false;
    return take_item(i, o, d, tmax, any);
  }
  FH_D bool take_item(uint32_t i, f3& o, f3& d, float& tmax, bool& any)
  {
    p = pool.q_sec[i];
    L = mk3(pool.rad[p]);
    active = true;
    if (scan(0u, o, d, tmax, any)) return true;
    active = false;
    return false;
  }
  FH_D void commit(bool hit, const HitRec& h, uint32_t nodes)
  {
    const size_t k = pool.sec_at(slot, p);
    if (slot == SEC_LIGHT && LIGHTS) {
      const float4 o = pool.sec[k], d = pool.sec[k + 1];
      const float4 la = pool.lp_a[p], lb = pool.lp_b[p];
      L += resolve_light_ray(sc, fr, mk3(la), la.w, mk3(lb), lb.w, mk3(o), mk3(d), hit, h);
    } else {
      if (COUNT) hp.add(nodes);
      if (!hit) L += mk3(pool.sec[k + 2]);
    }
  }
  FH_D bool drained() const { return feed.drained(); }
  FH_D bool followup() const { return active && slot < SEC_LIGHT; }
  FH_D uint32_t start_node() const { return start; }
};

template <bool COUNT, bool LIGHTS, bool ALPHA>
__global__ void __launch_bounds__(kBlock, COUNT ? 1 : (LIGHTS ? FH_SECONDARY_BLOCKS_HEAVY : (ALPHA ? FH_STREAM_BLOCKS_ALPHA : FH_STREAM_BLOCKS))) k_trace_secondary_stream(SceneDev sc, FrameDev fr, PoolDev pool, uint32_t depth, TraceCounters tc, uint32_t flush, uint32_t refill, uint32_t chunk, uint32_t min_rays, StackSpill spill)
{
  extern __shared__ __attribute__((aligned(16))) uint2 lds_stack[];
  __shared__ __attribute__((aligned(16))) unsigned char lds[(kBlock / 64) * kCoopLdsBytesPerWave];
  const uint32_t count = pool.counters[depth * kCounterStride + CNT_SEC];
  if (stream_block_idle(count, min_rays)) return;
  __shared__ HosekSky s_sky;
  if (LIGHTS) { stage_sky(fr, s_sky); __syncthreads(); }
  const ClockStamp stamp;
  CoopLds cl = coop_lds(lds, threadIdx.x >> 6);
  AlphaLds<AlphaDefer<true, ALPHA>::value>::attach(cl);
  uint32_t nn = 0, nt = 0;
  WaveSteps ws;
  SecondaryStream<COUNT, LIGHTS> pol(sc, fr, pool, ChunkFeed(pool.counters + depth * kCounterStride + CNT_CUR_SEC, count, stream_chunk_for(count, chunk)), tc.hist);
  __shared__ uint4 lds_top[kTopNodes * 4];
  stage_top_nodes(sc.bvh8, lds_top);
  traverse_stream<true, COUNT, true, ALPHA>(sc.bvh8, pol, nn, nt, &ws, cl, flush, refill, lds_stack, (int)sc.bvh8.depth, &sc, spill, lds_top,
                                            spill.probe ? pool.counters + depth * kCounterStride + CNT_COST_NODE : nullptr);
  pol.finish();
  stamp.commit(tc.clk);
  if (COUNT) {
    atomicAdd(tc.nodes, (unsigned long long)nn);
    atomicAdd(tc.tris, (unsigned long long)nt);
    atomicAdd(tc.rays, (unsigned long long)pol.n_rays);
    pol.hp.flush(tc.hist);
    if (ws.node) atomicAdd(tc.wave_nodes, (unsigned long long)ws.node);
    if (ws.tri) atomicAdd(tc.wave_tris, (unsigned long long)ws.tri);
  }
}

template <bool LIGHTS>
struct MergedStream {
  static constexpr bool all_any = false;
  static constexpr bool can_climb = false;
  SecondaryStream<false, LIGHTS> sec;
  const PoolDev& next;
  const uint32_t* q_closest;
  uint32_t n_sec;
  ChunkFeed feed;
  uint32_t pc = 0, qc = 0;
  uint32_t start_closest = 0;
  bool closest = false;
  FH_D MergedStream(const SceneDev& s, const FrameDev& f, const PoolDev& ps, const PoolDev& pn, const uint32_t* qc, uint32_t ns, const ChunkFeed& cf)
      : sec(s, f, ps, cf, nullptr), next(pn), q_closest(qc), n_sec(ns), feed(cf) {}
  FH_D bool advance(f3& o, f3& d, float& tmax, bool& any) { return closest ? false : sec.advance(o, d, tmax, any); }
  FH_D bool take(uint32_t i, f3& o, f3& d, float& tmax, bool& any)
  {
    if (i >= feed.end) return false;
    if (i < n_sec) { closest = false; return sec.take_item(i, o, d, tmax, any); }
    closest = true;
    qc = i - n_sec;
    pc = q_closest[qc];
    const float4 o4 = next.ray_o[pc], d4 = next.ray_d[pc];
    o = mk3(o4); d = mk3(d4); tmax = o4.w; any = false;
    start_closest = start_node_of(d4);
    return true;
  }
  FH_D uint32_t start_node() const { return closest ? start_closest : sec.start; }
  FH_D void commit(bool hit, const HitRec& h, uint32_t nodes)
  {
    if (closest) { next.hit[pc] = make_float4(h.t, h.u, h.v, __uint_as_float(h.prim)); next.q_prim[qc] = h.prim; }
    else sec.commit(hit, h, nodes);
  }
  FH_D bool drained() const { return feed.drained(); }
  FH_D bool followup() const { return !closest && sec.followup(); }
};

template <bool LIGHTS, bool ALPHA>
__global__ void __launch_bounds__(kBlock, LIGHTS ? FH_SECONDARY_BLOCKS_HEAVY : (ALPHA ? FH_STREAM_BLOCKS_ALPHA : FH_STREAM_BLOCKS)) k_trace_merged_stream(SceneDev sc, FrameDev fr, PoolDev ps, PoolDev pn, uint32_t depth, TraceCounters tc, uint32_t flush, uint32_t refill, uint32_t chunk, uint32_t min_rays, StackSpill spill)
{
  extern __shared__ __attribute__((aligned(16))) uint2 lds_stack[];
  __shared__ __attribute__((aligned(16))) unsigned char lds[(kBlock / 64) * kCoopLdsBytesPerWave];
  const uint32_t n_sec = ps.counters[depth * kCounterStride + CNT_SEC], n_closest = ps.counters[(depth + 1u) * kCounterStride + CNT_RAD];
  const uint32_t count = n_sec + n_closest;
  if (stream_block_idle(count, min_rays)) return;
  __shared__ HosekSky s_sky;
  if (LIGHTS) { stage_sky(fr, s_sky); __syncthreads(); }
  const ClockStamp stamp;
  CoopLds cl = coop_lds(lds, threadIdx.x >> 6);
  AlphaLds<AlphaDefer<true, ALPHA>::value>::attach(cl);
  uint32_t nn = 0, nt = 0;
  MergedStream<LIGHTS> pol(sc, fr, ps, pn, pn.q_rad[(depth + 1u) & 1u], n_sec, ChunkFeed(ps.counters + depth * kCounterStride + CNT_CUR_SEC, count, stream_chunk_for(count, chunk)));
  __shared__ uint4 lds_top[kTopNodes * 4];
  stage_top_nodes(sc.bvh8, lds_top);
  traverse_stream<true, false, true, ALPHA>(sc.bvh8, pol, nn, nt, nullptr, cl, flush, refill, lds_stack, (int)sc.bvh8.depth, &sc, spill, lds_top,
                                            spill.probe ? ps.counters + depth * kCounterStride + CNT_COST_NODE : nullptr);
  pol.sec.finish();
  stamp.commit(tc.clk);
}

constexpr uint32_t kTailRays = SEC_COUNT + 1u;
static_assert(kTailRays == 5u, "trace_all spells its per-lane fallback out ray by ray");
__device__ __attribute__((noinline)) bool tail_trace_lane(const SceneDev& sc, uint2* lds_stack, bool any, f3 o, f3 d, float tmax, HitRec& h)
{
  uint32_t a = 0, b = 0;
  if (!sc.use_bvh8) return any ? traverse<true, false>(sc, o, d, tmax, h, a, b) : traverse<false, false>(sc, o, d, tmax, h, a, b);
  if (sc.has_alpha) return any ? traverse_bvh8<true, false, true, true>(sc.bvh8, o, d, tmax, h, a, b, nullptr, lds_stack, (int)sc.bvh8.depth, &sc)
                               : traverse_bvh8<false, false, true, true>(sc.bvh8, o, d, tmax, h, a, b, nullptr, lds_stack, (int)sc.bvh8.depth, &sc);
  return any ? traverse_bvh8<true, false, true, false>(sc.bvh8, o, d, tmax, h, a, b, nullptr, lds_stack, (int)sc.bvh8.depth, &sc)
             : traverse_bvh8<false, false, true, false>(sc.bvh8, o, d, tmax, h, a, b, nullptr, lds_stack, (int)sc.bvh8.depth, &sc);
}
struct TailRay { bool has = false; bool any = true; f3 o = mk3(0.0f), d = mk3(0.0f, 0.0f, 1.0f); float tmax = 0.0f; HitRec h = HitRec{0.0f, 0.0f, 0.0f, 0xffffffffu}; bool hit = false; };

template <uint32_t LOBES>
__global__ void __launch_bounds__(kBlock, LOBES == L_ALL ? 1 : 2) k_tail(SceneDev sc, FrameDev fr, PoolDev pool, uint32_t first_depth, uint32_t coop_flush)
{
  extern __shared__ __attribute__((aligned(16))) uint2 lds_stack[];
  __shared__ __attribute__((aligned(16))) unsigned char lds_coop[(kBlock / 64) * kCoopLdsBytesPerWave];
  __shared__ float4 s_in[kBlock / 64][2][64];
  __shared__ float4 s_out[kBlock / 64][64];
  if (blockIdx.x * blockDim.x >= pool.counters[first_depth * kCounterStride + CNT_RAD]) return;
  const CoopLds cl = coop_lds(lds_coop, threadIdx.x >> 6);
  const uint32_t lane = threadIdx.x & 63u, wave = threadIdx.x >> 6;
  const bool coop = sc.use_bvh8 && coop_flush != 0u;
  auto trace_all = [&](TailRay (&rays)[kTailRays]) {
    if (!coop) {
      HitRec t;
      if (rays[0].has) { rays[0].hit = tail_trace_lane(sc, lds_stack, rays[0].any, rays[0].o, rays[0].d, rays[0].tmax, t); rays[0].h = t; }
      if (rays[1].has) { rays[1].hit = tail_trace_lane(sc, lds_stack, rays[1].any, rays[1].o, rays[1].d, rays[1].tmax, t); rays[1].h = t; }
      if (rays[2].has) { rays[2].hit = tail_trace_lane(sc, lds_stack, rays[2].any, rays[2].o, rays[2].d, rays[2].tmax, t); rays[2].h = t; }
      if (rays[3].has) { rays[3].hit = tail_trace_lane(sc, lds_stack, rays[3].any, rays[3].o, rays[3].d, rays[3].tmax, t); rays[3].h = t; }
      if (rays[4].has) { rays[4].hit = tail_trace_lane(sc, lds_stack, rays[4].any, rays[4].o, rays[4].d, rays[4].tmax, t); rays[4].h = t; }
      return;
    }
    uint32_t idx[kTailRays], total = 0;
#pragma unroll
    for (uint32_t k = 0; k < kTailRays; ++k) {
      const unsigned long long m = __ballot(rays[k].has);
      idx[k] = total + __builtin_amdgcn_mbcnt_hi((uint32_t)(m >> 32), __builtin_amdgcn_mbcnt_lo((uint32_t)m, 0u));
      total += (uint32_t)__popcll(m);
    }
    for (uint32_t lo = 0; lo < total; lo += 64u) {
#pragma unroll
      for (uint32_t k = 0; k < kTailRays; ++k)
        if (rays[k].has && idx[k] - lo < 64u) {
          s_in[wave][0][idx[k] - lo] = mk4(rays[k].o, rays[k].tmax);
          s_in[wave][1][idx[k] - lo] = mk4(rays[k].d, rays[k].any ? 1.0f : 0.0f);
        }
      const bool valid = lo + lane < total;
      const float4 a = valid ? s_in[wave][0][lane] : make_float4(0.0f, 0.0f, 0.0f, 0.0f), b = valid ? s_in[wave][1][lane] : make_float4(0.0f, 0.0f, 1.0f, 0.0f);
      HitRec h;
      uint32_t na = 0, nb = 0;
      if (sc.has_alpha) traverse_bvh8_coop_mode<2, false, true, true>(sc.bvh8, valid, b.w != 0.0f, mk3(a), mk3(b), a.w, h, na, nb, nullptr, cl, coop_flush, lds_stack, (int)sc.bvh8.depth, &sc);
      else traverse_bvh8_coop_mode<2, false, true, false>(sc.bvh8, valid, b.w != 0.0f, mk3(a), mk3(b), a.w, h, na, nb, nullptr, cl, coop_flush, lds_stack, (int)sc.bvh8.depth, &sc);
      if (valid) s_out[wave][lane] = make_float4(h.t, h.u, h.v, __uint_as_float(h.prim));
#pragma unroll
      for (uint32_t k = 0; k < kTailRays; ++k)
        if (rays[k].has && idx[k] - lo < 64u) {
          const float4 r = s_out[wave][idx[k] - lo];
          rays[k].h.t = r.x; rays[k].h.u = r.y; rays[k].h.v = r.z; rays[k].h.prim = __float_as_uint(r.w);
          rays[k].hit = rays[k].h.prim != 0xffffffffu;
        }
    }
  };
  __shared__ SobolRows<4> rows;
  __shared__ float s_lut[kLutReflFloats + kLutSheenFloats];
  __shared__ MaterialDev s_mat[kMatLds];
  for (uint32_t i = threadIdx.x; i < kLutReflFloats; i += blockDim.x) s_lut[i] = fr.lut.reflection[i];
  for (uint32_t i = threadIdx.x; i < kLutSheenFloats; i += blockDim.x) s_lut[kLutReflFloats + i] = fr.lut.sheen[i];
  fr.lut.reflection = s_lut;
  fr.lut.sheen = s_lut + kLutReflFloats;
  if (sc.n_materials <= kMatLds) {
    const uint32_t* src = reinterpret_cast<const uint32_t*>(sc.materials);
    uint32_t* dst = reinterpret_cast<uint32_t*>(s_mat);
    for (uint32_t i = threadIdx.x; i < sc.n_materials * (uint32_t)(sizeof(MaterialDev) / 4); i += blockDim.x) dst[i] = src[i];
    sc.materials = s_mat;
  }
  __shared__ HosekSky s_sky;
  stage_sky(fr, s_sky);
  __syncthreads();
  const uint32_t count = pool.counters[first_depth * kCounterStride + CNT_RAD];
  const uint32_t* q = pool.q_rad[first_depth & 1u];
  const bool has_lights = sc.n_lights > 0;
  const uint32_t stride = gridDim.x * blockDim.x;
  for (uint32_t base = blockIdx.x * blockDim.x; base < count; base += stride) {
    const uint32_t i = base + threadIdx.x;
    bool alive = i < count;
    uint32_t p = 0, image_idx = 0, n_spp = 0;
    f3 ro = mk3(0.0f), rd = mk3(0.0f, 0.0f, 1.0f), T = mk3(0.0f), L = mk3(0.0f);
    if (alive) {
      p = q[i];
      const float4 o = pool.ray_o[p];
      ro = mk3(o); rd = mk3(pool.ray_d[p]); T = mk3(pool.thr[p]); L = mk3(pool.rad[p]);
      image_idx = pool.pixel[p]; n_spp = pool.nspp[p];
    }
    HitRec h;
    bool hit = false;
    {
      TailRay rays[kTailRays];
      rays[SEC_COUNT].has = alive; rays[SEC_COUNT].any = false; rays[SEC_COUNT].o = ro; rays[SEC_COUNT].d = rd; rays[SEC_COUNT].tmax = 1e9f;
      trace_all(rays);
      h = rays[SEC_COUNT].h; hit = rays[SEC_COUNT].hit;
    }
    for (uint32_t depth = first_depth; depth < fr.max_depth; ++depth) {
      BounceSlots bs;
      bs.set(fr, sc.n_lights, depth);
      __syncthreads();
      bs.load_rows(rows, fr.sobol_bytes);
      if (__ballot(alive) == 0ull) continue;
      ShadeOut o;
      if (alive) {
        if (!hit) alive = false;
        else shade_hit<LOBES>(sc, fr, rows, bs, depth, make_float4(h.t, h.u, h.v, __uint_as_float(h.prim)), rd, T, L, image_idx, n_spp, o);
      }
      TailRay rays[kTailRays];
#pragma unroll
      for (uint32_t slot = SEC_DIR; slot <= SEC_LIGHT; ++slot) {
        if (slot == SEC_DIR && !fr.has_dir) continue;
        if (slot == SEC_AREA && !has_lights) continue;
        rays[slot].has = alive && o.sec[slot].active;
        rays[slot].any = !(slot == SEC_LIGHT && has_lights);
        rays[slot].o = o.sec[slot].o; rays[slot].d = o.sec[slot].d; rays[slot].tmax = o.sec[slot].tmax;
      }
      rays[SEC_COUNT].has = alive && o.cont; rays[SEC_COUNT].any = false; rays[SEC_COUNT].o = o.next_o; rays[SEC_COUNT].d = o.next_d; rays[SEC_COUNT].tmax = 1e9f;
      trace_all(rays);
#pragma unroll
      for (uint32_t slot = SEC_DIR; slot <= SEC_LIGHT; ++slot) {
        if (!rays[slot].has) continue;
        if (slot == SEC_LIGHT && has_lights) L += resolve_light_ray(sc, fr, o.lp_T, o.lp_cos, o.lp_f, o.lp_pdf, o.sec[slot].o, o.sec[slot].d, rays[slot].hit, rays[slot].h);
        else if (!rays[slot].hit) L += o.sec[slot].c;
      }
      if (alive) {
        if (o.cont) { rd = o.next_d; T = o.T; h = rays[SEC_COUNT].h; hit = rays[SEC_COUNT].hit; }
        else alive = false;
      }
    }
    if (i < count) pool.rad[p] = mk4(L, 0.0f);
  }
}

__global__ void __launch_bounds__(kBlock) k_firsthit_scan(PoolDev pool, const uint32_t* owned, uint32_t n_owned, uint32_t n_batch, uint32_t* seen_state)
{
  for (uint32_t i = blockIdx.x * blockDim.x + threadIdx.x; i < n_owned; i += gridDim.x * blockDim.x) {
    const uint32_t image_idx = owned[i];
    bool seen = seen_state[image_idx] != 0u;
    for (uint32_t k = 0; k < n_batch; ++k) {
      const uint32_t p = k * n_owned + i;
      const uint32_t fl = pool.flags[p];
      const bool in_queue = (fl & 2u) == 0u;
      if (seen) {
        pool.flags[p] = fl | 4u;
        if (!in_queue) pool.rad[p] = make_float4(0.0f, 0.0f, 0.0f, 0.0f);
      } else if (in_queue && __float_as_uint(pool.hit[p].w) != 0xffffffffu) {
        seen = true;
      }
    }
    seen_state[image_idx] = seen ? 1u : 0u;
  }
}

template <bool QUIRK, bool ADAPTIVE = false>
__global__ void __launch_bounds__(kBlock) k_accumulate(PoolDev pool, LayersDev layers, const uint32_t* owned, uint32_t n_owned, uint32_t n_batch,
                                                     std::conditional_t<ADAPTIVE, float2, float4>* carry)
{
  static_assert(!(QUIRK && ADAPTIVE), "FH_FLAG_REFERENCE_FIRSTHIT does not combine with adaptive sampling");
  for (uint32_t i = blockIdx.x * blockDim.x + threadIdx.x; i < n_owned; i += gridDim.x * blockDim.x) {
    const uint32_t image_idx = owned[i];
    uint32_t n_spp = layers.sample_count[image_idx];
    f3 beauty = mk3(layers.beauty[image_idx]), position = mk3(layers.position[image_idx]), normal = mk3(layers.normal[image_idx]), albedo = mk3(layers.albedo[image_idx]);
    float depth = layers.depth[image_idx];
    const float4 tc4 = layers.texcoord[image_idx];
    float tcx = tc4.x, tcy = tc4.y;
    f3 apos = mk3(0.0f), anrm = mk3(0.0f), aalb = mk3(0.0f);
    float au = 0.0f, av = 0.0f, ad = 0.0f;
    if constexpr (QUIRK) {
      apos = mk3(carry[4 * (size_t)image_idx]); anrm = mk3(carry[4 * (size_t)image_idx + 1]); aalb = mk3(carry[4 * (size_t)image_idx + 2]);
      const float4 td = carry[4 * (size_t)image_idx + 3];
      au = td.x; av = td.y; ad = td.z;
    }
    float2 m = make_float2(0.0f, 0.0f);
    if constexpr (ADAPTIVE) m = carry[image_idx];
    for (uint32_t k = 0; k < n_batch; ++k) {
      const uint32_t p = k * n_owned + i;
      const f3 L = mk3(pool.rad[p]);
      const f3 radiance = bad3(L) ? mk3(0.0f) : L;
      if (!QUIRK) { apos = mk3(0.0f); anrm = mk3(0.0f); aalb = mk3(0.0f); au = av = ad = 0.0f; }
      if (pool.flags[p] & 1u) {
        apos = mk3(pool.aov_position[p]);
        anrm = mk3(pool.aov_normal[p]);
        aalb = mk3(pool.aov_albedo[p]);
        const float4 td = pool.aov_texdepth[p];
        au = td.x; av = td.y; ad = td.z;
      }
      const float coef = 1.0f / (n_spp + 1.0f);
      const float fn = (float)n_spp;
      beauty = coef * (fn * beauty + radiance);
      position = coef * (fn * position + apos);
      normal = coef * (fn * normal + anrm);
      depth = coef * (fn * depth + ad);
      tcx = coef * (fn * tcx + au);
      tcy = coef * (fn * tcy + av);
      albedo = coef * (fn * albedo + aalb);
      if constexpr (ADAPTIVE) moments_update(m.x, m.y, coef, fn, radiance);
      n_spp++;
    }
    if constexpr (ADAPTIVE) carry[image_idx] = m;
    if constexpr (QUIRK) {
      carry[4 * (size_t)image_idx] = mk4(apos, 0.0f); carry[4 * (size_t)image_idx + 1] = mk4(anrm, 0.0f); carry[4 * (size_t)image_idx + 2] = mk4(aalb, 0.0f);
      carry[4 * (size_t)image_idx + 3] = make_float4(au, av, ad, 0.0f);
    }
    layers.sample_count[image_idx] = n_spp;
    layers.beauty[image_idx] = mk4(beauty, 1.0f);
    layers.position[image_idx] = mk4(position, 1.0f);
    layers.normal[image_idx] = mk4(normal, 1.0f);
    layers.depth[image_idx] = depth;
    layers.texcoord[image_idx] = make_float4(tcx, tcy, 0.0f, 1.0f);
    layers.albedo[image_idx] = mk4(albedo, 1.0f);
  }
}

void sort_queue_by_cell(hipStream_t st, uint32_t blocks, const uint32_t* count_ptr, const uint32_t* q_in, const uint16_t* keys, uint32_t* bins, uint32_t* q_out)
{
  hipLaunchKernelGGL(k_cell_hist, dim3(blocks), dim3(kSortBlock), 0, st, count_ptr, keys, bins);
  hipLaunchKernelGGL(k_cell_scan, dim3(1), dim3(kSortBlock), 0, st, bins, bins + kCells);
  hipLaunchKernelGGL(k_cell_scatter, dim3(blocks), dim3(kSortBlock), 0, st, count_ptr, q_in, keys, bins + kCells, q_out);
}

template <typename F>
void with_bool(bool b, F&& f)
{
  if (b) f(std::true_type{});
  else f(std::false_type{});
}

uint32_t grid_for(uint32_t n)
{
  uint32_t b = (n + kBlock - 1) / kBlock;
  b = (b + 7u) & ~7u;
  return b < 8 ? 8 : (b > 8192 ? 8192 : b);
}

template <uint32_t LOBES>
void launch_shade(hipStream_t st, uint32_t grid, const SceneDev& sc, const FrameDev& fr, const PoolDev& pool, uint32_t cls, uint32_t depth, bool three)
{
  if (three && LOBES != L_ALL) hipLaunchKernelGGL((k_shade<LOBES, (LOBES == L_ALL ? FH_SHADE_BLOCKS : 3)>), dim3(grid), dim3(kBlock), 0, st, sc, fr, pool, cls, depth);
  else hipLaunchKernelGGL(k_shade<LOBES>, dim3(grid), dim3(kBlock), 0, st, sc, fr, pool, cls, depth);
}

void dispatch_shade(hipStream_t st, uint32_t grid, uint32_t lobes, const SceneDev& sc, const FrameDev& fr, const PoolDev& pool, uint32_t cls, uint32_t depth, bool three)
{
  if ((lobes & ~(uint32_t)L_DIFF) == 0) return launch_shade<L_DIFF>(st, grid, sc, fr, pool, cls, depth, three);
  if ((lobes & ~(uint32_t)L_METAL) == 0) return launch_shade<L_METAL>(st, grid, sc, fr, pool, cls, depth, three);
  if ((lobes & ~(uint32_t)(L_SPEC | L_DIFF)) == 0) return launch_shade<L_SPEC | L_DIFF>(st, grid, sc, fr, pool, cls, depth, three);
  if ((lobes & ~(uint32_t)(L_METAL | L_SPEC | L_DIFF)) == 0) return launch_shade<L_METAL | L_SPEC | L_DIFF>(st, grid, sc, fr, pool, cls, depth, three);
  if ((lobes & ~(uint32_t)(L_COAT | L_METAL | L_SPEC | L_DIFF)) == 0) return launch_shade<L_COAT | L_METAL | L_SPEC | L_DIFF>(st, grid, sc, fr, pool, cls, depth, three);
  return launch_shade<L_ALL>(st, grid, sc, fr, pool, cls, depth, three);
}

template <uint32_t LOBES>
hipError_t shade_attributes_of(bool three, hipFuncAttributes& at, int& blocks)
{
  const void* fn = (three && LOBES != L_ALL) ? (const void*)k_shade<LOBES, (LOBES == L_ALL ? FH_SHADE_BLOCKS : 3)> : (const void*)k_shade<LOBES>;
  const hipError_t e = hipFuncGetAttributes(&at, fn);
  if (e != hipSuccess) return e;
  if (three && LOBES != L_ALL) return hipOccupancyMaxActiveBlocksPerMultiprocessor(&blocks, k_shade<LOBES, (LOBES == L_ALL ? FH_SHADE_BLOCKS : 3)>, kBlock, 0);
  return hipOccupancyMaxActiveBlocksPerMultiprocessor(&blocks, k_shade<LOBES>, kBlock, 0);
}
hipError_t shade_attributes(uint32_t lobes, bool three, hipFuncAttributes& at, int& blocks, uint32_t& compiled_lobes)
{
  if ((lobes & ~(uint32_t)L_DIFF) == 0) { compiled_lobes = L_DIFF; return shade_attributes_of<L_DIFF>(three, at, blocks); }
  if ((lobes & ~(uint32_t)L_METAL) == 0) { compiled_lobes = L_METAL; return shade_attributes_of<L_METAL>(three, at, blocks); }
  if ((lobes & ~(uint32_t)(L_SPEC | L_DIFF)) == 0) { compiled_lobes = L_SPEC | L_DIFF; return shade_attributes_of<L_SPEC | L_DIFF>(three, at, blocks); }
  if ((lobes & ~(uint32_t)(L_METAL | L_SPEC | L_DIFF)) == 0) { compiled_lobes = L_METAL | L_SPEC | L_DIFF; return shade_attributes_of<L_METAL | L_SPEC | L_DIFF>(three, at, blocks); }
  if ((lobes & ~(uint32_t)(L_COAT | L_METAL | L_SPEC | L_DIFF)) == 0) { compiled_lobes = L_COAT | L_METAL | L_SPEC | L_DIFF; return shade_attributes_of<L_COAT | L_METAL | L_SPEC | L_DIFF>(three, at, blocks); }
  compiled_lobes = L_ALL;
  return shade_attributes_of<L_ALL>(three, at, blocks);
}

hipEvent_t take_event(fh_ctx* ctx)
{
  if (!ctx->event_pool.empty()) { hipEvent_t e = ctx->event_pool.back(); ctx->event_pool.pop_back(); return e; }
  hipEvent_t e = nullptr;
  (void)hipEventCreate(&e);
  return e;
}

struct Span {
  fh_ctx* ctx; hipStream_t st; int kind; hipEvent_t a = nullptr, b = nullptr; bool on;
  Span(fh_ctx* c, hipStream_t s, int k) : ctx(c), st(s), kind(k), on((c->flags & FH_FLAG_TIME_KERNELS) != 0)
  {
    if (on) { a = take_event(ctx); b = take_event(ctx); (void)hipEventRecord(a, st); }
  }
  ~Span()
  {
    if (on) { (void)hipEventRecord(b, st); ctx->spans.push_back({a, b, kind}); }
  }
};

}

SceneDev scene_dev(const fh_ctx* ctx)
{
  SceneDev s{};
  s.face_rec = ctx->d_face_rec;
  s.face_cls = ctx->d_face_cls;
  s.materials = ctx->d_materials;
  s.lights = ctx->d_lights;
  s.n_faces = ctx->n_faces;
  s.n_lights = ctx->n_lights;
  s.n_materials = ctx->n_materials;
  s.textures = ctx->d_textures;
  s.srgb_lut = ctx->d_srgb_lut;
  s.n_textures = ctx->n_textures;
  s.alpha_rec = ctx->d_alpha_rec;
  s.has_alpha = (ctx->has_alpha || ctx->tun.force_alpha) ? 1u : 0u;
  s.bvh2.nodes = ctx->d_bvh2_nodes;
  s.bvh2.tris = ctx->d_bvh2_tris;
// ... 301 lines not shown
  auto compact = [&](const uint32_t* px, const uint32_t* xy, uint32_t n, uint32_t* scan, uint32_t* out_px, uint32_t* out_xy, uint32_t* h_count) -> int {
    const uint32_t n_blocks = (n + kBlock - 1u) / kBlock;
    hipLaunchKernelGGL(k_adaptive_count, dim3(n_blocks), dim3(kBlock), 0, st, ad, px, n, scan);
    hipLaunchKernelGGL(k_adaptive_scan, dim3(1), dim3(kBlock), 0, st, scan, n_blocks);
    hipLaunchKernelGGL(k_adaptive_select, dim3(n_blocks), dim3(kBlock), 0, st, ad, px, xy, n, scan, out_px, out_xy);
    FH_HIP(hipMemcpyAsync(h_count, scan + n_blocks, 4, hipMemcpyDeviceToHost, st));
    return FH_OK;
  };
  if (n_base) { const int rc = compact(base_px, base_xy, n_base, ctx->d_active_blocks, ctx->d_active[0], ctx->d_active[1], ctx->h_active_count); if (rc) return rc; }
  if (n_sky) { const int rc = compact(sky_px, sky_xy, n_sky, scan_sky, ctx->d_active[2], ctx->d_active[3], ctx->h_active_count + 1); if (rc) return rc; }
  FH_HIP(hipStreamSynchronize(st));
  if (n_base) *n_active = ctx->h_active_count[0];
  if (n_sky) *n_sky_active = ctx->h_active_count[1];
  if (*n_active > n_base || (n_sky && *n_sky_active > n_sky)) return fail(ctx, FH_E_HIP, "adaptive_select: count beyond the base list");
  return FH_OK;
}

int render_submit(fh_ctx* ctx, const fh_camera* cam, const float* bg, const fh_render_layers* layers, uint32_t n_samples, uint32_t max_depth, uint32_t seed)
{
  if (!ctx->scene_loaded || !ctx->bvh_valid) return fail(ctx, FH_E_INVALID, "fh_render: scene not uploaded or BVH not built");
  if (ctx->width == 0 || ctx->height == 0 || !ctx->d_sample_count) return fail(ctx, FH_E_INVALID, "fh_render: resolution not set");
  if (max_depth > 64) return fail(ctx, FH_E_INVALID, "fh_render: max_depth > 64 is not supported");
  if (ctx->n_owned == 0 || n_samples == 0) return FH_OK;
  const bool adaptive = ctx->adaptive;
  const bool guard_blocks = adaptive && ctx->adapt_block > 1u;
  if (adaptive && (ctx->flags & FH_FLAG_REFERENCE_FIRSTHIT) != 0 && n_samples > 1)
    return fail(ctx, FH_E_INVALID, "fh_render: FH_FLAG_REFERENCE_FIRSTHIT with n_samples > 1 does not combine with adaptive sampling (its first-hit state is per launch)");
  ctx->accumulated = true;
  if (!ctx->pool_target_by_caller) {
    bool allocating = false;
    unsigned long long held = 0;
    for (int k = 0; k < (((ctx->flags & FH_FLAG_SERIAL_PASSES) != 0) ? 1 : ctx->n_slots); ++k) {
      const fh_ctx::PoolShape& have = ctx->pool_shape[k];
      if (ctx->pool[k].capacity == 0 || (ctx->has_dir && !have.dir) || (ctx->n_lights > 0 && !have.lights) || have.classes < (ctx->n_classes < 1u ? 1u : ctx->n_classes)) allocating = true;
      held += (unsigned long long)ctx->pool[k].capacity * pool_bytes_per_path(ctx);
    }
    if (allocating) {
      size_t free_b = 0, total_b = 0;
      ctx->pool_target = ctx->pool_target_default;
      if (hipMemGetInfo(&free_b, &total_b) == hipSuccess) {
        const unsigned long long cap = ((unsigned long long)free_b + held) / (4ull * ctx->pool_share) / ((unsigned long long)ctx->n_slots * pool_bytes_per_path(ctx));
        if (cap < ctx->pool_target) ctx->pool_target = cap > ctx->n_owned ? (uint32_t)cap : ctx->n_owned;
      }
    }
  }

  FrameDev fr{};
  fr.width = ctx->width; fr.height = ctx->height;
  fr.seed_hash = xxhash32(seed);
  fr.max_depth = max_depth;
  fr.has_dir = ctx->has_dir ? 1u : 0u;
  fr.has_hosek = ctx->has_hosek ? 1u : 0u;
  fr.has_ibl = ctx->d_ibl ? 1u : 0u;
  fr.ibl = fht_texture{nullptr, ctx->d_ibl, ctx->ibl_w, ctx->ibl_h, 0u};
  const uint32_t has_lights = ctx->n_lights > 0 ? 1u : 0u;
  fr.n1 = 3u + has_lights;
  fr.n2 = 3u + fr.has_dir + has_lights;
  for (int r = 0; r < 3; ++r) fr.cam_xf.r[r] = make_float4(cam->transform[4 * r], cam->transform[4 * r + 1], cam->transform[4 * r + 2], cam->transform[4 * r + 3]);
  fr.cam_inv_tan = 1.0f / tanf(0.5f * cam->fov);
  fr.cam_F = cam->F; fr.cam_focus = cam->focus;
  {
    volatile float f = fr.cam_inv_tan, b = cam->focus;
    volatile float inv_b = 1.0f / b;
    volatile float den = 1.0f + f;
    den = den - inv_b;
    volatile float a = 1.0f / den;
    volatile float apb = a + b;
    volatile float two_f = 2.0f * f;
    volatile float lr = two_f / cam->F;
    fr.cam_a_plus_b = apb;
    fr.cam_lens_radius = lr;
  }
  fr.bg = mk3(bg[0], bg[1], bg[2]);
  fr.sky_intensity = ctx->sky_intensity;
  fr.sun_dir = mk3(ctx->sun_dir[0], ctx->sun_dir[1], ctx->sun_dir[2]);
  fr.hosek = ctx->d_hosek;
  fr.dir_le = mk3(ctx->dir_le[0], ctx->dir_le[1], ctx->dir_le[2]);
  fr.dir_dir = mk3(ctx->dir_dir[0], ctx->dir_dir[1], ctx->dir_dir[2]);
  fr.dir_disk_radius = 1e9f * tanf(0.5f * ctx->dir_angle * kPi / 180.0f);
  fr.scene_lo = mk3(ctx->scene_lo[0], ctx->scene_lo[1], ctx->scene_lo[2]);
  fr.scene_hi = mk3(ctx->scene_hi[0], ctx->scene_hi[1], ctx->scene_hi[2]);
  {
    const float cells = (float)(1u << kCellBits);
    const float ex = ctx->scene_hi[0] - ctx->scene_lo[0], ey = ctx->scene_hi[1] - ctx->scene_lo[1], ez = ctx->scene_hi[2] - ctx->scene_lo[2];
    fr.cell_scale = mk3(ex > 0.0f ? cells / ex : 0.0f, ey > 0.0f ? cells / ey : 0.0f, ez > 0.0f ? cells / ez : 0.0f);
  }
  fr.sobol = ctx->d_sobol;
  fr.sobol_bytes = ctx->d_sobol_bytes;
  fr.lut.reflection = ctx->d_lut_refl;
  fr.lut.sheen = ctx->d_lut_sheen;

  LayersDev L{};
  L.beauty = (float4*)layers->beauty; L.position = (float4*)layers->position; L.depth = layers->depth;
  L.normal = (float4*)layers->normal; L.texcoord = (float4*)layers->texcoord; L.albedo = (float4*)layers->albedo;
  L.sample_count = ctx->d_sample_count;

  const uint32_t* px_list = ctx->d_owned;
  const uint32_t* xy_list = ctx->d_owned_xy;
  uint32_t n_px = ctx->n_owned, n_sky = 0;
  const bool quirk_call = (ctx->flags & FH_FLAG_REFERENCE_FIRSTHIT) != 0 && n_samples > 1;
  if (ctx->tun.sky_split && !quirk_call && (unsigned long long)n_samples * ctx->n_owned >= (1ull << ctx->tun.sky_split_min_log2)) {
    const int rc = split_pixels(ctx, cam, fr);
    if (rc) return rc;
    if (ctx->split_valid && ctx->n_sky_px >= ctx->n_owned / 8u) {
      px_list = ctx->d_split[0]; xy_list = ctx->d_split[1];
      n_px = ctx->n_wave_px; n_sky = ctx->n_sky_px;
    }
  }
  const uint32_t target = ctx->pool_target > ctx->n_owned ? ctx->pool_target : ctx->n_owned;
  auto batch_for = [&](uint32_t n_px, uint32_t n_samples) {
    uint32_t batch = n_px ? target / n_px : n_samples;
    if (batch > n_samples) batch = n_samples;
    if (batch > 65535u) batch = 65535u;
    if (batch < 1) batch = 1;
    if (batch < n_samples) {
      uint32_t passes = (n_samples + batch - 1u) / batch;
      const uint32_t slots = (uint32_t)ctx->n_slots;
      if (slots > 1u && passes > slots && passes % slots != 0u && (passes / slots + 1u) * slots <= n_samples) passes = (passes / slots + 1u) * slots;
      batch = (n_samples + passes - 1u) / passes;
    }
    if (!quirk_call && (ctx->flags & FH_FLAG_SERIAL_PASSES) == 0 && (n_samples + batch - 1u) / batch < (uint32_t)ctx->n_slots && n_samples >= (uint32_t)ctx->n_slots && (unsigned long long)n_samples * n_px >= 3ull << 24) batch = (n_samples + (uint32_t)ctx->n_slots - 1u) / (uint32_t)ctx->n_slots;
    return batch;
  };

  const SceneDev sc_all = scene_dev(ctx);
  const SceneDev& sc = sc_all;
  const bool count = (ctx->flags & FH_FLAG_COUNT_TRAVERSAL) != 0;
  const bool clocks = (ctx->flags & FH_FLAG_TIME_KERNELS) != 0;
  TraceCounters tc_closest{ctx->d_trace_counters, ctx->d_trace_counters + 1, ctx->d_trace_counters + 2, ctx->d_trace_counters + 6, ctx->d_trace_counters + 7, ctx->d_trace_counters + 10,
                           clocks ? ctx->d_trace_counters + 27 : nullptr};
  TraceCounters tc_shadow{ctx->d_trace_counters + 3, ctx->d_trace_counters + 4, ctx->d_trace_counters + 5, ctx->d_trace_counters + 8, ctx->d_trace_counters + 9, ctx->d_trace_counters + 18,
                          clocks ? ctx->d_trace_counters + 29 : nullptr};

  const bool quirk = (ctx->flags & FH_FLAG_REFERENCE_FIRSTHIT) != 0 && n_samples > 1;
  if (quirk) {
    const size_t px = (size_t)ctx->width * ctx->height;
    if (ctx->quirk_pixels != px) {
      if (ctx->d_quirk_seen) (void)hipFree(ctx->d_quirk_seen);
      if (ctx->d_quirk_aov) (void)hipFree(ctx->d_quirk_aov);
      ctx->d_quirk_seen = nullptr; ctx->d_quirk_aov = nullptr; ctx->quirk_pixels = 0;
      FH_HIP(hipMalloc((void**)&ctx->d_quirk_seen, px * sizeof(uint32_t)));
      FH_HIP(hipMalloc((void**)&ctx->d_quirk_aov, px * 4 * sizeof(float4)));
      ctx->quirk_pixels = px;
    }
    FH_HIP(hipMemsetAsync(ctx->d_quirk_seen, 0, px * sizeof(uint32_t), ctx->stream));
    FH_HIP(hipMemsetAsync(ctx->d_quirk_aov, 0, px * 4 * sizeof(float4), ctx->stream));
  }
  if (!ctx->render_pending) { (void)hipEventRecord(ctx->ev_render_begin, ctx->stream); ctx->render_pending = true; }
  FH_HIP(hipEventRecord(ctx->ev_enter, ctx->stream));
  for (int k = 0; k + 1 < ctx->n_slots; ++k) FH_HIP(hipStreamWaitEvent(ctx->aux_stream[k], ctx->ev_enter, 0));
  int last_slot = 0;
  hipStream_t sky_st = ((ctx->flags & FH_FLAG_SERIAL_PASSES) != 0 || ctx->n_slots == 1) ? ctx->stream : ctx->sky_stream;
  if (n_sky && sky_st != ctx->stream) FH_HIP(hipStreamWaitEvent(sky_st, ctx->ev_enter, 0));
  if (n_sky && !guard_blocks) {
    Span sp(ctx, sky_st, 4);
    uint32_t sky_grid = grid_for(n_sky);
    if (ctx->tun.sky_blocks_per_cu && sky_grid > ctx->tun.n_cus * ctx->tun.sky_blocks_per_cu) sky_grid = ctx->tun.n_cus * ctx->tun.sky_blocks_per_cu;
    if (adaptive) {
      hipLaunchKernelGGL(k_sky_pixels<true>, dim3(sky_grid), dim3(kBlock), 0, sky_st, fr, L, ctx->d_sample_issued, ctx->d_split[2], ctx->d_split[3], n_sky, n_samples,
                         (const SkyAdaptive*)ctx->d_sky_adaptive);
      ctx->sky_taken_pending = true;
    } else {
      hipLaunchKernelGGL(k_sky_pixels<false>, dim3(sky_grid), dim3(kBlock), 0, sky_st, fr, L, ctx->d_sample_issued, ctx->d_split[2], ctx->d_split[3], n_sky, n_samples, ctx->d_split_counters + 2);
      ctx->stats.paths += (uint64_t)n_sky * n_samples;
      ctx->stats.sky_pixel_samples += (uint64_t)n_sky * n_samples;
    }
  }

  const fh_ctx::Tunables& tun = ctx->tun;
  const bool coop = sc.use_bvh8 != 0 && sc.bvh8.n_tris < kCoopMaxTris && tun.coop;
  const bool stream = coop && tun.stream && (tun.stream_forced || ctx->bvh8_n_nodes >= 4096u);
  const uint32_t stack_bytes = lds_stack_bytes(stack_entries_for(ctx->bvh8_depth));
  const uint32_t cfg_bytes = lds_stack_bytes(stack_entries_for(ctx->bvh8_depth) + 1u);
  if (sc.use_bvh8 && ctx->lds_configured_bytes != cfg_bytes) {
    const int rc = configure_traversal_lds(ctx, cfg_bytes);
    if (rc) return rc;
  }
  if (sc.use_bvh8 && stack_bytes + ctx->lds_static_max > tun.lds_per_block) return fail(ctx, FH_E_UNSUPPORTED, "fh_render: BVH too deep for the LDS traversal stack");
  const uint32_t stack_entries = stack_entries_for(ctx->bvh8_depth);
  const uint32_t stream_need = stack_entries + (sc.bvh8.parent ? 1u : 0u);
  const uint32_t static_lds_closest = kCoopLdsBytesPerBlock + (sc.has_alpha && AlphaDefer<false, true>::value ? kAlphaLdsBytesPerBlock : 0u);
  const uint32_t static_lds_secondary = kCoopLdsBytesPerBlock + kTopLdsBytes + (sc.has_alpha && AlphaDefer<true, true>::value ? kAlphaLdsBytesPerBlock : 0u);
  if (stream) {
    const uint32_t key = stack_bytes | (count ? 1u : 0u) | (sc.has_alpha ? 2u : 0u) | (sc.n_lights > 0 ? 4u : 0u) | (sc.bvh8.parent ? 8u : 0u) | (tun.stack_lds_entries << 20);
    if (ctx->occupancy_key != key) {
      auto occupancy = [&](bool secondary, uint32_t entries) {
        const uint32_t bytes = lds_stack_bytes(entries);
        int r = 0;
        with_bool(count, [&](auto C) { with_bool(sc.has_alpha != 0, [&](auto A) {
          if (!secondary) (void)hipOccupancyMaxActiveBlocksPerMultiprocessor(&r, k_trace_closest_stream<decltype(C)::value, decltype(A)::value>, kBlock, bytes);
          else with_bool(sc.n_lights > 0, [&](auto Li) {
            (void)hipOccupancyMaxActiveBlocksPerMultiprocessor(&r, k_trace_secondary_stream<decltype(C)::value, decltype(Li)::value, decltype(A)::value>, kBlock, bytes);
          });
        }); });
        return r;
      };
      auto pick = [&](bool secondary, uint32_t blocks_wanted, uint32_t& entries_out, uint32_t& blocks_out) {
        const uint32_t lds_share = tun.lds_per_cu / blocks_wanted;
        const uint32_t static_lds = secondary ? static_lds_secondary : static_lds_closest;
        const uint32_t fit = lds_share > static_lds + 1280u ? (lds_share - static_lds) / 1280u : 1u;
        const uint32_t floor_entries = fit < 8u ? fit : 8u;
        uint32_t entries = stream_need;
        int got = occupancy(secondary, entries);
        if (tun.stack_lds_entries) entries = tun.stack_lds_entries < stream_need ? tun.stack_lds_entries : stream_need;
        else if (stream_need > floor_entries) {
          const int best = occupancy(secondary, floor_entries);
          while (entries > floor_entries && got < best) { --entries; got = occupancy(secondary, entries); }
        }
        if (entries != stream_need) got = occupancy(secondary, entries);
        entries_out = entries;
        blocks_out = got > 0 ? (uint32_t)got : 0u;
      };
      pick(false, FH_STREAM_BLOCKS_CLOSEST, ctx->stream_lds_entries, ctx->occupancy_blocks);
      pick(true, sc.n_lights > 0 ? FH_SECONDARY_BLOCKS_HEAVY : (sc.has_alpha ? FH_STREAM_BLOCKS_ALPHA : FH_STREAM_BLOCKS), ctx->stream_lds_entries_secondary, ctx->occupancy_blocks_secondary);
      ctx->occupancy_key = key;
      if (!count) {
        ctx->info_blocks[0] = ctx->occupancy_blocks; ctx->info_blocks[1] = ctx->occupancy_blocks_secondary;
        ctx->info_entries[0] = ctx->stream_lds_entries; ctx->info_entries[1] = ctx->stream_lds_entries_secondary;
      }
      if (getenv("FH_DEBUG_BVH"))
        fprintf(stderr, "[trace] stack of %u entries (%s); in LDS: closest %u (%u B + %u B per workgroup, %u resident workgroups per CU), secondary %u (%u B + %u B, %u workgroups)\n", stream_need, sc.bvh8.parent ? "rays start at the node of the face they leave" : "rays start at the root",
                ctx->stream_lds_entries, lds_stack_bytes(ctx->stream_lds_entries), static_lds_closest, ctx->occupancy_blocks, ctx->stream_lds_entries_secondary,
                lds_stack_bytes(ctx->stream_lds_entries_secondary), static_lds_secondary, ctx->occupancy_blocks_secondary);
    }
  }
  const uint32_t stream_entries = stream ? ctx->stream_lds_entries : stream_need, stream_entries_secondary = stream ? ctx->stream_lds_entries_secondary : stream_need;
  const uint32_t stream_stack_bytes = lds_stack_bytes(stream_entries), stream_stack_bytes_secondary = lds_stack_bytes(stream_entries_secondary);
  auto wgs_for = [&](uint32_t bytes, uint32_t static_lds, uint32_t compiled_for, uint32_t reported) {
    uint32_t w = tun.lds_per_cu / (bytes + static_lds);
    w = w > compiled_for ? compiled_for : (w < 1u ? 1u : w);
    if (stream && reported && reported < w) w = reported;
    return w;
  };
  const uint32_t wgs_closest = wgs_for(stream_stack_bytes, static_lds_closest, FH_STREAM_BLOCKS_CLOSEST, ctx->occupancy_blocks);
  const uint32_t wgs_secondary = wgs_for(stream_stack_bytes_secondary, static_lds_secondary, FH_STREAM_BLOCKS > FH_SECONDARY_BLOCKS_HEAVY ? FH_STREAM_BLOCKS : FH_SECONDARY_BLOCKS_HEAVY, ctx->occupancy_blocks_secondary);
  const uint32_t stream_grid = tun.n_cus * wgs_closest;
  const uint32_t stream_grid_secondary = tun.n_cus * wgs_secondary;
  const uint32_t spill_entries = stream_entries < stream_need ? stream_need - stream_entries : 0u;
  const uint32_t spill_entries_secondary = stream_entries_secondary < stream_need ? stream_need - stream_entries_secondary : 0u;
  const size_t spill_threads = (size_t)(stream_grid > stream_grid_secondary ? stream_grid : stream_grid_secondary) * kBlock;
  const size_t spill_region = (size_t)(spill_entries > spill_entries_secondary ? spill_entries : spill_entries_secondary) * spill_threads;
  if (spill_region * 6u > ctx->stack_spill_capacity) {
    FH_HIP(hipDeviceSynchronize());
    if (ctx->d_stack_spill) FH_HIP(hipFree(ctx->d_stack_spill));
    ctx->d_stack_spill = nullptr;
    ctx->stack_spill_capacity = 0;
    FH_HIP(hipMalloc((void**)&ctx->d_stack_spill, sizeof(uint2) * spill_region * 6u));
    ctx->stack_spill_capacity = spill_region * 6u;
  }
  const uint32_t chunk_max = tun.stream_chunk_fixed ? tun.stream_chunk : (ctx->bvh8_n_nodes < 512u ? 256u : (ctx->bvh8_n_nodes < 4096u ? 128u : tun.stream_chunk));
  const uint32_t stream_refill = tun.stream_refill, stream_chunk = (tun.stream_chunk & 0xffffu) | ((chunk_max > tun.stream_chunk ? chunk_max : 0u) << 16);
  const uint32_t chunk_closest = tun.stream_chunk_closest ? tun.stream_chunk_closest : tun.stream_chunk;
  const uint32_t stream_chunk_closest = (chunk_closest & 0xffffu) | ((chunk_max > chunk_closest ? chunk_max : 0u) << 16);
  const uint32_t env_tail_depth = tun.tail_depth;
  const bool sort_queues = tun.sort_queues && (stream || tun.sort_small);
  const bool shade_three = tun.shade_wgs ? tun.shade_wgs == 3u : true;

  const uint32_t* const base_px = px_list;
  const uint32_t* const base_xy = xy_list;
  const uint32_t n_base = n_px;
  bool ran = false, sky_ran = false;
  for (uint32_t call_done = 0; call_done < n_samples;) {
  uint32_t n_round = n_samples - call_done, n_sky_round = 0;
  if (adaptive) {
    const uint32_t to_boundary = ctx->adapt_growth == 1u ? ctx->adapt.step - ctx->adapt_total % ctx->adapt.step : adaptive_to_boundary(ctx);
    if (n_round > to_boundary) n_round = to_boundary;
    if (ran && last_slot != 0) FH_HIP(hipStreamWaitEvent(ctx->stream, ctx->ev_acc[last_slot], 0));
    if (sky_ran && sky_st != ctx->stream) { FH_HIP(hipEventRecord(ctx->ev_sky, sky_st)); FH_HIP(hipStreamWaitEvent(ctx->stream, ctx->ev_sky, 0)); }
    const int rc = guard_blocks && n_sky ? adaptive_select(ctx, ctx->stream, base_px, base_xy, n_base, &n_px, ctx->d_split[2], ctx->d_split[3], n_sky, &n_sky_round)
                                         : adaptive_select(ctx, ctx->stream, base_px, base_xy, n_base, &n_px);
    if (rc) return rc;
    px_list = ctx->d_active[0]; xy_list = ctx->d_active[1];
    if (n_sky_round) {
      Span sp(ctx, sky_st, 4);
      uint32_t sky_grid = grid_for(n_sky_round);
      if (ctx->tun.sky_blocks_per_cu && sky_grid > ctx->tun.n_cus * ctx->tun.sky_blocks_per_cu) sky_grid = ctx->tun.n_cus * ctx->tun.sky_blocks_per_cu;
      hipLaunchKernelGGL(k_sky_pixels<true>, dim3(sky_grid), dim3(kBlock), 0, sky_st, fr, L, ctx->d_sample_issued, ctx->d_active[2], ctx->d_active[3], n_sky_round, n_round,
                         (const SkyAdaptive*)ctx->d_sky_adaptive);
      ctx->sky_taken_pending = true;
      sky_ran = true;
    }
  }
  const uint32_t batch = batch_for(n_px, n_round);
  const uint32_t coop_flush = (!tun.coop_flush_fixed && batch >= n_round && !sc.has_alpha && tun.coop_flush > 32u) ? 32u : tun.coop_flush;
  for (uint32_t done = 0; done < n_round && n_px; done += batch) {
    const uint32_t nb = (n_round - done) < batch ? (n_round - done) : batch;
    ran = true;
    const uint32_t n_paths = n_px * nb;
    const uint32_t grid = grid_for(n_paths);
    const bool serial = quirk || (ctx->flags & FH_FLAG_SERIAL_PASSES) != 0;
    const int n_slots = serial ? 1 : ctx->n_slots;
    const int slot = serial ? 0 : (int)(ctx->pass_seq % (unsigned long long)n_slots), prev = serial ? ctx->last_slot_used : (slot + n_slots - 1) % n_slots;
    ctx->pass_seq++;
    ctx->stats.n_passes++;
    ctx->last_slot_used = slot;
    hipStream_t st = slot ? ctx->aux_stream[slot - 1] : ctx->stream;
    last_slot = slot;
    const bool single_pass = !serial && batch >= n_round && n_round == nb;
    const bool merge = single_pass && stream && !count && tun.merge_trace;
    const bool overlap = single_pass && tun.overlap_secondary && !merge;
    hipStream_t sb = st;
    if (overlap) {
      sb = (st == ctx->aux_stream[0]) ? ctx->aux_stream[1] : ctx->aux_stream[0];
      while (ctx->ev_bounce.size() < 2u * (max_depth + 1u)) {
        hipEvent_t e = nullptr;
        FH_HIP(hipEventCreateWithFlags(&e, hipEventDisableTiming));
        ctx->ev_bounce.push_back(e);
      }
    }
    hipStream_t sh = st;
    { const int rc = pool_ensure(ctx, slot, n_px * batch); if (rc) return rc; }
    const PoolDev& pool = ctx->pool[slot];
    FH_HIP(hipMemsetAsync(pool.counters, 0, sizeof(uint32_t) * kCounterStride * (max_depth + 1), st));
    int pass_bu = -1;
    bool use_bu = false;
    if (sc_all.bvh8.parent && stream && (ctx->flags & FH_FLAG_ROOT_START) == 0u) {
      if (tun.bottom_up == 1u) use_bu = true;
      else if (tun.bottom_up == 2u) {
        if (ctx->bu_choice == 0 && !count && !merge && !sc_all.has_alpha) { use_bu = (ctx->bu_toggle++ & 1u) != 0u; pass_bu = use_bu ? 1 : 0; }
        else use_bu = ctx->bu_choice == 2;
      }
    }
    SceneDev sc = sc_all;
    if (!use_bu) { sc.bvh8.parent = nullptr; sc.face_node = nullptr; }
    if (prev != slot && ctx->gen_valid[prev]) FH_HIP(hipStreamWaitEvent(st, ctx->ev_gen[prev], 0));
    {
      Span sp(ctx, st, 4);
      hipLaunchKernelGGL(k_generate, dim3(grid_for((n_px + kGenChunks - 1) / kGenChunks), nb), dim3(kBlock), 0, st, fr, pool, ctx->d_sample_issued, px_list, xy_list, n_px);
      hipLaunchKernelGGL(k_bump_issued, dim3((n_px + kBlock - 1) / kBlock), dim3(kBlock), 0, st, ctx->d_sample_issued, px_list, n_px, nb);
      ctx->stats.n_generate_launches++;
    }
    FH_HIP(hipEventRecord(ctx->ev_gen[slot], st));
    ctx->gen_valid[slot] = true;
    ctx->stats.paths += n_paths;
    const uint32_t kTailPaths = tun.tail_paths ? tun.tail_paths : (n_paths <= (1u << 22) ? 262144u : 65536u);
    for (int k = 0; k < 3; ++k) {
      if (!(ctx->counters_in_flight[k] && hipEventQuery(ctx->ev_counters[k]) == hipSuccess)) continue;
      ctx->counters_in_flight[k] = false;
      const uint32_t wd = ctx->counters_wave_depth[k];
      const uint32_t* hc = ctx->h_counters[k];
      if (ctx->counters_paths[k]) {
        const uint32_t n = wd < 65u ? wd : 65u;
        for (uint32_t d = 0; d <= n; ++d) ctx->survival[d] = (double)hc[d * kCounterStride + CNT_RAD] / (double)ctx->counters_paths[k];
        if (ctx->survival_n < n + 1u) ctx->survival_n = n + 1u;
      }
      if (ctx->counters_bu[k] >= 0 && ctx->bu_choice == 0) {
        double cost = 0.0, items = 0.0;
        for (uint32_t d = 0; d < wd; ++d) { cost += 510.0 * hc[d * kCounterStride + CNT_COST_NODE] + 175.0 * hc[d * kCounterStride + CNT_COST_TRI]; items += hc[d * kCounterStride + CNT_SEC]; }
        ctx->bu_cost[ctx->counters_bu[k]] += cost; ctx->bu_items[ctx->counters_bu[k]] += items;
        if (ctx->bu_items[0] >= 65536.0 && ctx->bu_items[1] >= 65536.0) {
          const double off = ctx->bu_cost[0] / ctx->bu_items[0], on = ctx->bu_cost[1] / ctx->bu_items[1];
          ctx->bu_choice = on < 0.95 * off ? 2 : 1;
          if (getenv("FH_DEBUG_BVH")) fprintf(stderr, "[trace] rays that leave a surface start at %s: %.0f against %.0f SIMD cycles of tests per shaded path (from the root / from the face)\n", ctx->bu_choice == 2 ? "the node of their face" : "the root", off, on);
        }
      }
      ctx->counters_bu[k] = -1;
      if (tun.debug_tail) { fprintf(stderr, "[tail] slot %d wd %u paths %u survivors:", k, wd, ctx->counters_paths[k]); for (uint32_t d = 0; d <= wd; ++d) fprintf(stderr, " %u", ctx->h_counters[k][d * kCounterStride + CNT_RAD]); fprintf(stderr, "\n"); }
    }
    {
      uint32_t pick = 0;
      if (!ctx->survival_n) pick = n_paths > (1u << 22) ? max_depth : 2u;
      else {
        const uint32_t known = ctx->survival_n - 1u;
        for (uint32_t d = 1; d <= known && !pick; ++d)
          if ((double)n_paths * ctx->survival[d] <= (double)kTailPaths) pick = d;
        if (!pick) {
          const double last = (double)n_paths * ctx->survival[known], prev = known ? (double)n_paths * ctx->survival[known - 1u] : 0.0;
          uint32_t more = 1;
          if (last > 0.0 && prev > last) {
            const double steps = ceil(log((double)kTailPaths / last) / log(last / prev));
            more = steps < 1.0 ? 1u : (steps > 16.0 ? 16u : (uint32_t)steps);
          }
          pick = known + more;
        }
      }
      ctx->auto_wave_depth = pick;
    }
    uint32_t wave_depth = ctx->tail_depth ? ctx->tail_depth : ctx->auto_wave_depth;
    if (env_tail_depth) wave_depth = env_tail_depth;
    if (wave_depth < 1u) wave_depth = 1u;
    if (wave_depth > max_depth) wave_depth = max_depth;
    PoolDev pd = pool, ps = pool;
    uint32_t* q_spare = pool.q_tmp;
    const uint32_t sort_blocks = n_paths / 16384u < 1u ? 1u : (n_paths / 16384u > 512u ? 512u : n_paths / 16384u);
    for (uint32_t depth = 0; depth < wave_depth; ++depth) {
      if (!(merge && depth > 0)) {
        Span sp(ctx, st, 0);
        if (stream) {
          with_bool(count, [&](auto C) { with_bool(sc.has_alpha != 0, [&](auto A) {
            hipLaunchKernelGGL((k_trace_closest_stream<decltype(C)::value, decltype(A)::value>), dim3(grid < stream_grid ? grid : stream_grid), dim3(kBlock), stream_stack_bytes, st, sc, pd, depth, tc_closest,
                               coop_flush, stream_refill, stream_chunk_closest, tun.stream_min_rays, StackSpill{spill_entries ? ctx->d_stack_spill + (size_t)(2 * slot) * spill_region : nullptr, stream_entries});
          }); });
        } else if (coop) {
          with_bool(count, [&](auto C) { with_bool(sc.has_alpha != 0, [&](auto A) {
            hipLaunchKernelGGL((k_trace_closest_coop<decltype(C)::value, decltype(A)::value>), dim3(grid), dim3(kBlock), stack_bytes, st, sc, pd, depth, tc_closest, coop_flush);
          }); });
        } else {
          with_bool(count, [&](auto C) { with_bool(sc.use_bvh8 != 0, [&](auto W) { with_bool(sc.has_alpha != 0, [&](auto A) {
            hipLaunchKernelGGL((k_trace_closest_static<decltype(C)::value, decltype(W)::value, decltype(A)::value>), dim3(grid), dim3(kBlock), 0, st, sc, pd, depth, tc_closest);
          }); }); });
        }
        ctx->stats.n_closest_launches++;
      }
      if (quirk && depth == 0) hipLaunchKernelGGL(k_firsthit_scan, dim3(grid_for(n_px)), dim3(kBlock), 0, st, pd, px_list, n_px, nb, ctx->d_quirk_seen);
      {
        Span sp(ctx, sh, 6);
        hipLaunchKernelGGL(k_route, dim3(grid), dim3(kBlock), 0, sh, sc, pd, depth, ctx->n_classes, count ? ctx->d_trace_counters + 26 : nullptr);
      }
      if (overlap && depth > 0) FH_HIP(hipStreamWaitEvent(st, ctx->ev_bounce[2u * (depth - 1u) + 1u], 0));
      {
        Span sp(ctx, sh, 2);
        for (uint32_t c = 0; c < ctx->n_classes; ++c) dispatch_shade(sh, grid, ctx->class_lobes[c], sc, fr, pd, c, depth, shade_three);
        if (depth == 0) hipLaunchKernelGGL(k_miss_primary, dim3(grid), dim3(kBlock), 0, sh, fr, pd);
        ctx->stats.n_shade_launches += ctx->n_classes;
      }
      {
        Span sp(ctx, sh, 6);
        const bool tail_next = depth + 1u == wave_depth && wave_depth < max_depth;
        const bool sort_sec = sort_queues && (!single_pass || tun.sort_onepass == 1u);
        const bool sort_rad = sort_queues && (!single_pass || tun.sort_onepass == 1u || (tun.sort_onepass == 2u && tail_next));
        ps = pd;
        if (sort_sec) {
          sort_queue_by_cell(sh, sort_blocks, pool.counters + depth * kCounterStride + CNT_SEC, pool.q_sec, pool.key_sec, pool.bins, pool.q_sec_sorted);
          ps.q_sec = pool.q_sec_sorted;
        }
        if (sort_rad) {
          const uint32_t nxt = (depth + 1u) & 1u;
          sort_queue_by_cell(sh, sort_blocks, pool.counters + (depth + 1u) * kCounterStride + CNT_RAD, pd.q_rad[nxt], pool.key_rad, pool.bins, q_spare);
          uint32_t* const unsorted = pd.q_rad[nxt];
          pd.q_rad[nxt] = q_spare;
          q_spare = unsorted;
        }
      }
      if (merge && depth + 1u < wave_depth) {
        Span sp(ctx, st, 1);
        with_bool(sc.n_lights > 0, [&](auto Li) { with_bool(sc.has_alpha != 0, [&](auto A) {
          hipLaunchKernelGGL((k_trace_merged_stream<decltype(Li)::value, decltype(A)::value>), dim3(grid < stream_grid_secondary ? grid : stream_grid_secondary), dim3(kBlock), stream_stack_bytes_secondary, st, sc,
                             fr, ps, pd, depth, tc_shadow, coop_flush, stream_refill, stream_chunk, tun.stream_min_rays,
                             StackSpill{spill_entries_secondary ? ctx->d_stack_spill + (size_t)(2 * slot + 1) * spill_region : nullptr, stream_entries_secondary, pass_bu >= 0 ? 1u : 0u});
        }); });
        ctx->stats.n_shadow_launches++;
        ctx->stats.n_closest_launches++;
      } else {
        if (overlap) { FH_HIP(hipEventRecord(ctx->ev_bounce[2u * depth], st)); FH_HIP(hipStreamWaitEvent(sb, ctx->ev_bounce[2u * depth], 0)); }
        Span sp(ctx, sb, 1);
        if (stream) {
          with_bool(count, [&](auto C) { with_bool(sc.n_lights > 0, [&](auto Li) { with_bool(sc.has_alpha != 0, [&](auto A) {
            hipLaunchKernelGGL((k_trace_secondary_stream<decltype(C)::value, decltype(Li)::value, decltype(A)::value>), dim3(grid < stream_grid_secondary ? grid : stream_grid_secondary), dim3(kBlock), stream_stack_bytes_secondary, sb, sc,
                               fr, ps, depth, tc_shadow, coop_flush, stream_refill, stream_chunk, tun.stream_min_rays,
                               StackSpill{spill_entries_secondary ? ctx->d_stack_spill + (size_t)(2 * slot + 1) * spill_region : nullptr, stream_entries_secondary, pass_bu >= 0 ? 1u : 0u});
          }); }); });
        } else if (coop) {
          with_bool(count, [&](auto C) { with_bool(sc.n_lights > 0, [&](auto Li) { with_bool(sc.has_alpha != 0, [&](auto A) {
            hipLaunchKernelGGL((k_trace_secondary_coop<decltype(C)::value, decltype(Li)::value, decltype(A)::value>), dim3(grid), dim3(kBlock), stack_bytes, sb, sc, fr, ps, depth, tc_shadow,
                               coop_flush);
          }); }); });
        } else {
          with_bool(count, [&](auto C) { with_bool(sc.use_bvh8 != 0, [&](auto W) { with_bool(sc.n_lights > 0, [&](auto Li) { with_bool(sc.has_alpha != 0, [&](auto A) {
            hipLaunchKernelGGL((k_trace_secondary_static<decltype(C)::value, decltype(W)::value, decltype(Li)::value, decltype(A)::value>), dim3(grid), dim3(kBlock), stack_bytes, sb, sc, fr, ps,
                               depth, tc_shadow);
          }); }); }); });
        }
        ctx->stats.n_shadow_launches++;
      }
      if (overlap) FH_HIP(hipEventRecord(ctx->ev_bounce[2u * depth + 1u], sb));
    }
    if (overlap && wave_depth > 0) FH_HIP(hipStreamWaitEvent(st, ctx->ev_bounce[2u * (wave_depth - 1u) + 1u], 0));
    if (wave_depth < max_depth) {
      Span sp(ctx, st, 3);
      uint32_t lobes = 0;
      for (uint32_t c = 0; c < ctx->n_classes; ++c) lobes |= ctx->class_lobes[c];
      const dim3 tg(grid_for(n_paths / 16 + 1)), tb(kBlock);
      const uint32_t tl = sc.use_bvh8 ? stack_bytes : 0u, tf = coop ? coop_flush : 0u;
      if ((lobes & ~(uint32_t)L_DIFF) == 0) hipLaunchKernelGGL(k_tail<L_DIFF>, tg, tb, tl, st, sc, fr, pd, wave_depth, tf);
      else if ((lobes & ~(uint32_t)(L_METAL | L_SPEC | L_DIFF)) == 0) hipLaunchKernelGGL((k_tail<L_METAL | L_SPEC | L_DIFF>), tg, tb, tl, st, sc, fr, pd, wave_depth, tf);
      else if ((lobes & ~(uint32_t)(L_COAT | L_METAL | L_SPEC | L_DIFF)) == 0) hipLaunchKernelGGL((k_tail<L_COAT | L_METAL | L_SPEC | L_DIFF>), tg, tb, tl, st, sc, fr, pd, wave_depth, tf);
      else hipLaunchKernelGGL(k_tail<L_ALL>, tg, tb, tl, st, sc, fr, pd, wave_depth, tf);
      ctx->stats.n_tail_launches++;
    }
    if (prev != slot && ctx->acc_valid[prev]) FH_HIP(hipStreamWaitEvent(st, ctx->ev_acc[prev], 0));
    {
      Span sp(ctx, st, 5);
      if (quirk) hipLaunchKernelGGL((k_accumulate<true>), dim3(grid_for(n_px)), dim3(kBlock), 0, st, pool, L, px_list, n_px, nb, ctx->d_quirk_aov);
      else if (adaptive) hipLaunchKernelGGL((k_accumulate<false, true>), dim3(grid_for(n_px)), dim3(kBlock), 0, st, pool, L, px_list, n_px, nb, ctx->d_moments);
      else hipLaunchKernelGGL((k_accumulate<false>), dim3(grid_for(n_px)), dim3(kBlock), 0, st, pool, L, px_list, n_px, nb, (float4*)nullptr);
      ctx->stats.n_accumulate_launches++;
    }
    FH_HIP(hipEventRecord(ctx->ev_acc[slot], st));
    ctx->acc_valid[slot] = true;
    if (!ctx->counters_in_flight[slot] && ctx->h_counters[slot]) {
      FH_HIP(hipMemcpyAsync(ctx->h_counters[slot], pool.counters, sizeof(uint32_t) * kCounterStride * (max_depth + 1), hipMemcpyDeviceToHost, st));
      FH_HIP(hipEventRecord(ctx->ev_counters[slot], st));
      ctx->counters_in_flight[slot] = true;
      ctx->counters_wave_depth[slot] = wave_depth;
      ctx->counters_paths[slot] = n_paths;
      ctx->counters_bu[slot] = pass_bu;
    }
  }
  call_done += n_round;
  ctx->adapt_total += n_round;
  if (adaptive && n_px == 0 && n_sky_round == 0) { ctx->adapt_total += n_samples - call_done; break; }
  }
  if (last_slot != 0 && ran) FH_HIP(hipStreamWaitEvent(ctx->stream, ctx->ev_acc[last_slot], 0));
  if (n_sky && sky_st != ctx->stream) { FH_HIP(hipEventRecord(ctx->ev_sky, sky_st)); FH_HIP(hipStreamWaitEvent(ctx->stream, ctx->ev_sky, 0)); }
  FH_HIP(hipGetLastError());
  return FH_OK;
}

}
```

Baseline: 7928 Msamples/s.

## Run sky pixels as a low-priority filler with a persistent cursor and final drain

```diff
diff --git a/fredholm_amd/csrc/capi.hip b/fredholm_amd/csrc/capi.hip
--- a/fredholm_amd/csrc/capi.hip
+++ b/fredholm_amd/csrc/capi.hip
@@ -518,6 +518,7 @@
     env_off("FH_OVERLAP", t.overlap_secondary);
     env_off("FH_MERGE", t.merge_trace);
     env_uint("FH_SKY_BLOCKS", 0, 64, t.sky_blocks_per_cu);
+    env_uint("FH_SKY_FILLER_GRID", 0, 65535, t.sky_filler_grid);
     if (const char* e = getenv("FH_POISON")) t.poison_pools = e[0] == '1';
     env_off("FH_SKY_SPLIT", t.sky_split);
     env_uint("FH_SKY_SPLIT_MIN_LOG2", 0, 40, t.sky_split_min_log2);
@@ -542,6 +543,7 @@
     if ((low ? hipStreamCreateWithPriority(&ctx->sky_stream, hipStreamNonBlocking, least) : hipStreamCreateWithFlags(&ctx->sky_stream, hipStreamNonBlocking)) != hipSuccess) return bail("hipStreamCreate failed");
   }
   (void)hipEventCreateWithFlags(&ctx->ev_sky, hipEventDisableTiming);
+  (void)hipEventCreateWithFlags(&ctx->ev_sky_cursor, hipEventDisableTiming);
   if (hipMalloc((void**)&ctx->d_split_counters, 16) != hipSuccess) return bail("hipMalloc failed");
   (void)hipMemsetAsync(ctx->d_split_counters, 0, 16, ctx->stream);
   (void)hipEventCreate(&ctx->ev_render_begin);
@@ -573,6 +575,7 @@
   if (ctx->h_active_count) (void)hipHostFree(ctx->h_active_count);
   if (ctx->sky_stream) { (void)hipStreamSynchronize(ctx->sky_stream); (void)hipStreamDestroy(ctx->sky_stream); }
   if (ctx->ev_sky) (void)hipEventDestroy(ctx->ev_sky);
+  if (ctx->ev_sky_cursor) (void)hipEventDestroy(ctx->ev_sky_cursor);
   for (auto& s : ctx->spans) { (void)hipEventDestroy(s.a); (void)hipEventDestroy(s.b); }
   for (auto e : ctx->event_pool) (void)hipEventDestroy(e);
   for (auto e : ctx->ev_bounce) (void)hipEventDestroy(e);
diff --git a/fredholm_amd/csrc/context.h b/fredholm_amd/csrc/context.h
--- a/fredholm_amd/csrc/context.h
+++ b/fredholm_amd/csrc/context.h
@@ -101,6 +101,7 @@
   float split_key[32] = {};
   hipStream_t sky_stream = nullptr;
   hipEvent_t ev_sky = nullptr;
+  hipEvent_t ev_sky_cursor = nullptr;
   struct ShardList { uint32_t rank, world, width, height, tile_w, tile_h; uint32_t* d_owned; uint32_t n_owned; };
   struct FrameMap { uint32_t world = 0, width = 0, height = 0, tile_w = 0, tile_h = 0; uint32_t* d_all = nullptr; std::vector<uint32_t> start; };
   FrameMap frame_map;
@@ -174,7 +175,8 @@
     bool overlap_secondary = true;
     bool sky_split = true;
     uint32_t sky_split_min_log2 = 27;
-    uint32_t sky_blocks_per_cu = 0;
+    uint32_t sky_blocks_per_cu = 1;
+    uint32_t sky_filler_grid = 0;
     bool poison_pools = false;
     bool merge_trace = true;
     uint32_t shade_wgs = 0;
diff --git a/fredholm_amd/csrc/fh_sky.h b/fredholm_amd/csrc/fh_sky.h
--- a/fredholm_amd/csrc/fh_sky.h
+++ b/fredholm_amd/csrc/fh_sky.h
@@ -42,22 +42,35 @@
   return st;
 }
 
-FH_HD f3 hosek_radiance(const HosekSky& st, f3 sun_dir, float intensity, f3 v)
+template <bool ROLLED>
+FH_HD f3 hosek_radiance_form(const HosekSky& st, f3 sun_dir, float intensity, f3 v)
 {
   const float theta = fhe_acos(clampf(v.y, -1.0f, 1.0f));
   const float gamma = fhe_acos(dot(sun_dir, v));
   const float cg = fhe_cos(gamma), ct = fhe_cos(theta);
   const float rayM = cg * cg;
   const float zenith = sqrt_cr(ct);
-  float out[3];
-#pragma unroll
-  for (int ch = 0; ch < 3; ++ch) {
+  auto channel = [&](int ch) {
     const float* c = st.cfg[ch];
     const float expM = fhe_exp(c[4] * gamma);
     const float mieM = (1.0f + cg * cg) / fhe_pow1p5(1.0f + c[8] * c[8] - 2.0f * c[8] * cg);
-    out[ch] = (1.0f + c[0] * fhe_exp(c[1] / (ct + 0.01f))) * (c[2] + c[3] * expM + c[5] * rayM + c[6] * mieM + c[7] * zenith) * st.rad[ch];
+    return (1.0f + c[0] * fhe_exp(c[1] / (ct + 0.01f))) * (c[2] + c[3] * expM + c[5] * rayM + c[6] * mieM + c[7] * zenith) * st.rad[ch];
+  };
+  if constexpr (ROLLED) {
+    float r = 0.0f, g = 0.0f, b = 0.0f;
+#pragma unroll 1
+    for (int ch = 0; ch < 3; ++ch) {
+      const float o = channel(ch);
+      r = ch == 0 ? o : r; g = ch == 1 ? o : g; b = ch == 2 ? o : b;
+    }
+    return intensity * mk3(r, g, b);
+  } else {
+    float out[3];
+#pragma unroll
+    for (int ch = 0; ch < 3; ++ch) out[ch] = channel(ch);
+    return intensity * mk3(out[0], out[1], out[2]);
   }
-  return intensity * mk3(out[0], out[1], out[2]);
 }
+FH_HD f3 hosek_radiance(const HosekSky& st, f3 sun_dir, float intensity, f3 v) { return hosek_radiance_form<false>(st, sun_dir, intensity, v); }
 
 }
diff --git a/fredholm_amd/csrc/render.hip b/fredholm_amd/csrc/render.hip
--- a/fredholm_amd/csrc/render.hip
+++ b/fredholm_amd/csrc/render.hip
@@ -30,6 +30,9 @@
 #ifndef FH_STREAM_BLOCKS_CLOSEST
 #define FH_STREAM_BLOCKS_CLOSEST FH_STREAM_BLOCKS
 #endif
+#ifndef FH_STREAM_BLOCKS_FILLER
+#define FH_STREAM_BLOCKS_FILLER 6
+#endif
 #ifndef FH_SHADE_BLOCKS
 #define FH_SHADE_BLOCKS 2
 #endif
@@ -49,6 +52,14 @@
   __syncthreads();
 }
 
+#ifndef FH_PASS_PRIORITY
+#define FH_PASS_PRIORITY 1
+#endif
+FH_D void pass_priority()
+{
+  if (FH_PASS_PRIORITY) __builtin_amdgcn_s_setprio(FH_PASS_PRIORITY);
+}
+
 FH_D void stage_sky(FrameDev& fr, HosekSky& lds_sky)
 {
   if (!fr.has_hosek) return;
@@ -56,6 +67,7 @@
   fr.hosek = &lds_sky;
 }
 
+template <bool ROLLED_SKY = false>
 FH_D f3 env_radiance(const FrameDev& fr, f3 d)
 {
   if (fr.has_ibl) {
@@ -66,7 +78,7 @@
     fht_tex2d(&fr.ibl, nullptr, phi / (2.0f * kPi), theta / kPi, o);
     return fr.sky_intensity * mk3(o[0], o[1], o[2]);
   }
-  return fr.has_hosek ? hosek_radiance(*fr.hosek, fr.sun_dir, fr.sky_intensity, d) : fr.bg;
+  return fr.has_hosek ? hosek_radiance_form<ROLLED_SKY>(*fr.hosek, fr.sun_dir, fr.sky_intensity, d) : fr.bg;
 }
 
 FH_D bool camera_ray(const FrameDev& fr, const uint32_t* sobol_dim1, uint32_t image_idx, uint32_t px, uint32_t py, uint32_t n_spp, f2 u, f2 u_lens, f3& org, f3& dir);
@@ -99,6 +111,7 @@
 constexpr int kGenChunks = 4;
 __global__ void __launch_bounds__(kBlock) k_generate(FrameDev fr, PoolDev pool, const uint32_t* issued, const uint32_t* owned, const uint32_t* owned_xy, uint32_t n_owned)
 {
+  pass_priority();
   __shared__ SobolRows<1> rows;
   __shared__ HosekSky s_sky;
   stage_sky(fr, s_sky);
@@ -268,13 +281,16 @@
   uint32_t* violations;
   unsigned long long* taken;
 };
+constexpr int kSkyWaves = 6;
+constexpr uint32_t kSkyGroup = 64;
 template <bool ADAPTIVE>
-__global__ void __launch_bounds__(kBlock) k_sky_pixels(FrameDev fr, LayersDev layers, uint32_t* issued, const uint32_t* sky_px, const uint32_t* sky_xy, uint32_t n_sky, uint32_t n_samples,
-                                                     std::conditional_t<ADAPTIVE, const SkyAdaptive*, uint32_t*> violations_or_adaptive)
-{
+__global__ void __launch_bounds__(kBlock, kSkyWaves) k_sky_pixels(FrameDev fr, LayersDev layers, uint32_t* issued, const uint32_t* sky_px, const uint32_t* sky_xy, uint32_t n_sky, uint32_t n_samples,
+                                                                std::conditional_t<ADAPTIVE, const SkyAdaptive*, uint32_t*> violations_or_adaptive, uint32_t* cursor)
+{
+  static_assert(kSkyGroup == 64u, "a group is one wave's lanes");
   uint32_t* violations;
-  AdaptiveDev ad{};
-  if constexpr (ADAPTIVE) { ad = violations_or_adaptive->ad; violations = violations_or_adaptive->violations; }
+  const AdaptiveDev* adp = nullptr;
+  if constexpr (ADAPTIVE) { adp = &violations_or_adaptive->ad; violations = violations_or_adaptive->violations; }
   else violations = violations_or_adaptive;
   unsigned long long n_taken = 0;
   __shared__ SobolRows<1> rows;
@@ -282,28 +298,31 @@
   stage_sky(fr, s_sky);
   const uint32_t dims[1] = {1u};
   load_sobol_rows<1>(rows, fr.sobol_bytes, dims);
-  for (uint32_t i = blockIdx.x * blockDim.x + threadIdx.x; i < n_sky; i += gridDim.x * blockDim.x) {
+  const uint32_t n_groups = (n_sky + kSkyGroup - 1u) / kSkyGroup;
+  const uint32_t lane = threadIdx.x & 63u;
+  for (;;) {
+    uint32_t group = 0u;
+    if (lane == 0u) group = atomicAdd(cursor, 1u);
+    group = __shfl(group, 0);
+    if (group >= n_groups) break;
+    const uint32_t i = group * kSkyGroup + lane;
+    if (i < n_sky) {
     const uint32_t image_idx = sky_px[i], xy = sky_xy[i];
     const uint32_t first = issued[image_idx];
     uint32_t n_spp = layers.sample_count[image_idx];
-    f3 beauty = mk3(layers.beauty[image_idx]), position = mk3(layers.position[image_idx]), normal = mk3(layers.normal[image_idx]), albedo = mk3(layers.albedo[image_idx]);
-    float depth = layers.depth[image_idx];
-    const float4 tc4 = layers.texcoord[image_idx];
-    float tcx = tc4.x, tcy = tc4.y;
+    f3 beauty = mk3(layers.beauty[image_idx]);
     bool violated = false;
-    uint32_t blk = 0xffffffffu;
     CmjBlock b0{}, b1{};
     float2 m = make_float2(0.0f, 0.0f);
-    if constexpr (ADAPTIVE) m = ad.moments[image_idx];
-    uint32_t taken = n_samples;
-    for (uint32_t k = 0; k < n_samples; ++k) {
-      if constexpr (ADAPTIVE) { if (!ad.marks && adaptive_converged(ad, n_spp, m.x, m.y)) { taken = k; break; } }
+    if constexpr (ADAPTIVE) m = adp->moments[image_idx];
+    uint32_t taken = 0;
+    for (; taken < n_samples; ++taken) {
+      if constexpr (ADAPTIVE) { if (!adp->marks && adaptive_converged(*adp, n_spp, m.x, m.y)) break; }
       f3 org, dir;
-      const uint32_t n = first + k;
-      if ((n >> 4) != blk) {
-        blk = n >> 4;
-        b0 = cmj_block(blk, image_idx, 0u, fr.seed_hash);
-        b1 = cmj_block(blk, image_idx, 1u, fr.seed_hash);
+      const uint32_t n = first + taken;
+      if (taken == 0u || (n & 15u) == 0u) {
+        b0 = cmj_block(n >> 4, image_idx, 0u, fr.seed_hash);
+        b1 = cmj_block(n >> 4, image_idx, 1u, fr.seed_hash);
       }
       const bool alive = camera_ray(fr, rows.m[0], image_idx, xy & 0xffffu, xy >> 16, n, cmj_draw_in_block(b0, n), cmj_draw_in_block(b1, n), org, dir);
       RayPre rp;
@@ -311,31 +330,49 @@
       rp.inv = safe_reciprocal(dir);
       float tn;
       violated = violated || (alive && slab_test(rp, fr.scene_lo.x, fr.scene_lo.y, fr.scene_lo.z, fr.scene_hi.x, fr.scene_hi.y, fr.scene_hi.z, 1e9f, tn));
-      const f3 L = alive ? mk3(0.0f) + mk3(1.0f) * env_radiance(fr, dir) : mk3(0.0f);
+      const f3 L = alive ? mk3(0.0f) + mk3(1.0f) * env_radiance<true>(fr, dir) : mk3(0.0f);
       const f3 radiance = bad3(L) ? mk3(0.0f) : L;
       const float coef = 1.0f / (n_spp + 1.0f);
       const float fn = (float)n_spp;
       beauty = coef * (fn * beauty + radiance);
-      position = coef * (fn * position + mk3(0.0f));
-      normal = coef * (fn * normal + mk3(0.0f));
-      depth = coef * (fn * depth + 0.0f);
-      tcx = coef * (fn * tcx + 0.0f);
-      tcy = coef * (fn * tcy + 0.0f);
-      albedo = coef * (fn * albedo + mk3(0.0f));
       if constexpr (ADAPTIVE) moments_update(m.x, m.y, coef, fn, radiance);
       n_spp++;
     }
     if (violated) atomicAdd(violations, 1u);
-    if constexpr (ADAPTIVE) { ad.moments[image_idx] = m; n_taken += taken; issued[image_idx] = first + taken; }
-    else issued[image_idx] = first + n_samples;
+    if constexpr (ADAPTIVE) { adp->moments[image_idx] = m; n_taken += taken; }
+    issued[image_idx] = first + taken;
     layers.sample_count[image_idx] = n_spp;
     layers.beauty[image_idx] = mk4(beauty, 1.0f);
+    f3 position = mk3(layers.position[image_idx]), normal = mk3(layers.normal[image_idx]), albedo = mk3(layers.albedo[image_idx]);
+    float depth = layers.depth[image_idx];
+    const float4 tc4 = layers.texcoord[image_idx];
+    float tcx = tc4.x, tcy = tc4.y;
+    const uint32_t any_bits = __float_as_uint(position.x) | __float_as_uint(position.y) | __float_as_uint(position.z) | __float_as_uint(normal.x) | __float_as_uint(normal.y) |
+                              __float_as_uint(normal.z) | __float_as_uint(albedo.x) | __float_as_uint(albedo.y) | __float_as_uint(albedo.z) | __float_as_uint(depth) |
+                              __float_as_uint(tcx) | __float_as_uint(tcy);
+    if (any_bits != 0u) {
+      uint32_t n_aov = n_spp - taken;
+#pragma unroll 1
+      for (uint32_t k = 0; k < taken; ++k) {
+        const float coef = 1.0f / (n_aov + 1.0f);
+        const float fn = (float)n_aov;
+        position = coef * (fn * position + mk3(0.0f));
+        normal = coef * (fn * normal + mk3(0.0f));
+        depth = coef * (fn * depth + 0.0f);
+        tcx = coef * (fn * tcx + 0.0f);
+        tcy = coef * (fn * tcy + 0.0f);
+        albedo = coef * (fn * albedo + mk3(0.0f));
+        n_aov++;
+      }
+    }
     layers.position[image_idx] = mk4(position, 1.0f);
     layers.normal[image_idx] = mk4(normal, 1.0f);
     layers.depth[image_idx] = depth;
     layers.texcoord[image_idx] = make_float4(tcx, tcy, 0.0f, 1.0f);
     layers.albedo[image_idx] = mk4(albedo, 1.0f);
-  }  if constexpr (ADAPTIVE) {
+    }
+  }
+  if constexpr (ADAPTIVE) {
     __shared__ unsigned long long s_taken;
     if (threadIdx.x == 0u) s_taken = 0ull;
     __syncthreads();
@@ -423,6 +460,7 @@
 template <bool COUNT, bool WIDE, bool ALPHA>
 __global__ void __launch_bounds__(kBlock) k_trace_closest_static(SceneDev sc, PoolDev pool, uint32_t depth, TraceCounters tc)
 {
+  pass_priority();
   const uint32_t* cnt = pool.counters + depth * kCounterStride;
   const uint32_t count = cnt[CNT_RAD];
   const uint32_t* q = pool.q_rad[depth & 1u];
@@ -452,6 +490,7 @@
 template <bool COUNT, bool ALPHA>
 __global__ void __launch_bounds__(kBlock) k_trace_closest_coop(SceneDev sc, PoolDev pool, uint32_t depth, TraceCounters tc, uint32_t flush)
 {
+  pass_priority();
   extern __shared__ __attribute__((aligned(16))) uint2 lds_stack[];
   __shared__ __attribute__((aligned(16))) unsigned char lds[(kBlock / 64) * kCoopLdsBytesPerWave];
   const CoopLds cl = coop_lds(lds, threadIdx.x >> 6);
@@ -556,6 +595,7 @@
 __global__ void __launch_bounds__(kBlock, COUNT ? 1 : FH_STREAM_BLOCKS_CLOSEST) k_trace_closest_stream(SceneDev sc, PoolDev pool, uint32_t depth, TraceCounters tc, uint32_t flush, uint32_t refill, uint32_t chunk, uint32_t min_rays,
                                                                  StackSpill spill)
 {
+  pass_priority();
   __shared__ __attribute__((aligned(16))) unsigned char lds[(kBlock / 64) * kCoopLdsBytesPerWave];
   const uint32_t count = pool.counters[depth * kCounterStride + CNT_RAD];
   if (stream_block_idle(count, min_rays)) return;
@@ -581,6 +621,7 @@
 constexpr int kRouteChunks = 8;
 __global__ void __launch_bounds__(kBlock) k_route(SceneDev sc, PoolDev pool, uint32_t depth, uint32_t n_classes, unsigned long long* hit_counter)
 {
+  pass_priority();
   __shared__ uint32_t wave_cnt[kMaxClasses][kRouteChunks * (kBlock / 64)];
   __shared__ uint32_t block_base[kMaxClasses];
   uint32_t* cnt = pool.counters + depth * kCounterStride;
@@ -623,6 +664,7 @@
 
 __global__ void __launch_bounds__(kBlock) k_miss_primary(FrameDev fr, PoolDev pool)
 {
+  pass_priority();
   __shared__ HosekSky s_sky;
   stage_sky(fr, s_sky);
   __syncthreads();
@@ -931,6 +973,7 @@
 
 __global__ void __launch_bounds__(kSortBlock) k_cell_hist(const uint32_t* count_ptr, const uint16_t* keys, uint32_t* hist)
 {
+  pass_priority();
   __shared__ uint32_t h[kCells];
   for (uint32_t b = threadIdx.x; b < kCells; b += kSortBlock) h[b] = 0u;
   __syncthreads();
@@ -944,6 +987,7 @@
 
 __global__ void __launch_bounds__(kSortBlock) k_cell_scan(uint32_t* hist, uint32_t* cursor)
 {
+  pass_priority();
   __shared__ uint32_t part[kSortBlock];
   constexpr uint32_t per = kCells / kSortBlock;
   uint32_t v[per], sum = 0;
@@ -962,6 +1006,7 @@
 
 __global__ void __launch_bounds__(kSortBlock) k_cell_scatter(const uint32_t* count_ptr, const uint32_t* q_in, const uint16_t* keys, uint32_t* cursor, uint32_t* q_out)
 {
+  pass_priority();
   __shared__ uint32_t h[kCells];
   __shared__ uint32_t base[kCells];
   for (uint32_t b = threadIdx.x; b < kCells; b += kSortBlock) h[b] = 0u;
@@ -984,6 +1029,7 @@
 template <uint32_t LOBES, int BLOCKS = FH_SHADE_BLOCKS>
 __global__ void __launch_bounds__(kBlock, (LOBES == L_ALL ? 1 : BLOCKS)) k_shade(SceneDev sc, FrameDev fr, PoolDev pool, uint32_t cls, uint32_t depth)
 {
+  pass_priority();
   if (blockIdx.x * blockDim.x >= pool.counters[depth * kCounterStride + CNT_CLS + cls]) return;
   __shared__ SobolRows<4> rows;
   __shared__ float s_lut[kLutReflFloats + kLutSheenFloats];
@@ -1078,6 +1124,7 @@
 template <bool COUNT, bool WIDE, bool LIGHTS, bool ALPHA>
 __global__ void __launch_bounds__(kBlock) k_trace_secondary_static(SceneDev sc, FrameDev fr, PoolDev pool, uint32_t depth, TraceCounters tc)
 {
+  pass_priority();
   extern __shared__ __attribute__((aligned(16))) uint2 lds_stack[];
   __shared__ HosekSky s_sky;
   if (LIGHTS) { stage_sky(fr, s_sky); __syncthreads(); }
@@ -1125,6 +1172,7 @@
 template <bool COUNT, bool LIGHTS, bool ALPHA>
 __global__ void __launch_bounds__(kBlock, COUNT ? 1 : (LIGHTS ? 5 : 6)) k_trace_secondary_coop(SceneDev sc, FrameDev fr, PoolDev pool, uint32_t depth, TraceCounters tc, uint32_t flush)
 {
+  pass_priority();
   extern __shared__ __attribute__((aligned(16))) uint2 lds_stack[];
   __shared__ __attribute__((aligned(16))) unsigned char lds[(kBlock / 64) * kCoopLdsBytesPerWave];
   const CoopLds cl = coop_lds(lds, threadIdx.x >> 6);
@@ -1250,6 +1298,7 @@
 template <bool COUNT, bool LIGHTS, bool ALPHA>
 __global__ void __launch_bounds__(kBlock, COUNT ? 1 : (LIGHTS ? FH_SECONDARY_BLOCKS_HEAVY : (ALPHA ? FH_STREAM_BLOCKS_ALPHA : FH_STREAM_BLOCKS))) k_trace_secondary_stream(SceneDev sc, FrameDev fr, PoolDev pool, uint32_t depth, TraceCounters tc, uint32_t flush, uint32_t refill, uint32_t chunk, uint32_t min_rays, StackSpill spill)
 {
+  pass_priority();
   extern __shared__ __attribute__((aligned(16))) uint2 lds_stack[];
   __shared__ __attribute__((aligned(16))) unsigned char lds[(kBlock / 64) * kCoopLdsBytesPerWave];
   const uint32_t count = pool.counters[depth * kCounterStride + CNT_SEC];
@@ -1318,6 +1367,7 @@
 template <bool LIGHTS, bool ALPHA>
 __global__ void __launch_bounds__(kBlock, LIGHTS ? FH_SECONDARY_BLOCKS_HEAVY : (ALPHA ? FH_STREAM_BLOCKS_ALPHA : FH_STREAM_BLOCKS)) k_trace_merged_stream(SceneDev sc, FrameDev fr, PoolDev ps, PoolDev pn, uint32_t depth, TraceCounters tc, uint32_t flush, uint32_t refill, uint32_t chunk, uint32_t min_rays, StackSpill spill)
 {
+  pass_priority();
   extern __shared__ __attribute__((aligned(16))) uint2 lds_stack[];
   __shared__ __attribute__((aligned(16))) unsigned char lds[(kBlock / 64) * kCoopLdsBytesPerWave];
   const uint32_t n_sec = ps.counters[depth * kCounterStride + CNT_SEC], n_closest = ps.counters[(depth + 1u) * kCounterStride + CNT_RAD];
@@ -1354,6 +1404,7 @@
 template <uint32_t LOBES>
 __global__ void __launch_bounds__(kBlock, LOBES == L_ALL ? 1 : 2) k_tail(SceneDev sc, FrameDev fr, PoolDev pool, uint32_t first_depth, uint32_t coop_flush)
 {
+  pass_priority();
   extern __shared__ __attribute__((aligned(16))) uint2 lds_stack[];
   __shared__ __attribute__((aligned(16))) unsigned char lds_coop[(kBlock / 64) * kCoopLdsBytesPerWave];
   __shared__ float4 s_in[kBlock / 64][2][64];
@@ -1502,6 +1553,7 @@
 __global__ void __launch_bounds__(kBlock) k_accumulate(PoolDev pool, LayersDev layers, const uint32_t* owned, uint32_t n_owned, uint32_t n_batch,
                                                      std::conditional_t<ADAPTIVE, float2, float4>* carry)
 {
+  pass_priority();
   static_assert(!(QUIRK && ADAPTIVE), "FH_FLAG_REFERENCE_FIRSTHIT does not combine with adaptive sampling");
   for (uint32_t i = blockIdx.x * blockDim.x + threadIdx.x; i < n_owned; i += gridDim.x * blockDim.x) {
     const uint32_t image_idx = owned[i];
@@ -2109,16 +2161,38 @@
   int last_slot = 0;
   hipStream_t sky_st = ((ctx->flags & FH_FLAG_SERIAL_PASSES) != 0 || ctx->n_slots == 1) ? ctx->stream : ctx->sky_stream;
   if (n_sky && sky_st != ctx->stream) FH_HIP(hipStreamWaitEvent(sky_st, ctx->ev_enter, 0));
+  struct SkyDrain { const uint32_t* px; const uint32_t* xy; uint32_t n, n_samples; bool pending; } sky_drain{nullptr, nullptr, 0u, 0u, false};
+  uint32_t* const sky_cursor = ctx->d_split_counters + 3;
+  const uint32_t sky_filler_wgs = sky_st == ctx->stream ? 0u : (ctx->tun.sky_filler_grid ? ctx->tun.sky_filler_grid : ctx->tun.n_cus * ctx->tun.sky_blocks_per_cu);
+  auto sky_launch = [&](hipStream_t s, uint32_t wgs, const uint32_t* px, const uint32_t* xy, uint32_t n, uint32_t ns) {
+    Span sp(ctx, s, 4);
+    const uint32_t full = (n + kBlock - 1u) / kBlock;
+    const uint32_t grid = wgs < full ? wgs : full;
+    if (adaptive) hipLaunchKernelGGL(k_sky_pixels<true>, dim3(grid), dim3(kBlock), 0, s, fr, L, ctx->d_sample_issued, px, xy, n, ns, (const SkyAdaptive*)ctx->d_sky_adaptive, sky_cursor);
+    else hipLaunchKernelGGL(k_sky_pixels<false>, dim3(grid), dim3(kBlock), 0, s, fr, L, ctx->d_sample_issued, px, xy, n, ns, ctx->d_split_counters + 2, sky_cursor);
+  };
+  const uint32_t sky_full_wgs = ctx->tun.n_cus * (uint32_t)kSkyWaves;
+  auto sky_begin = [&](const uint32_t* px, const uint32_t* xy, uint32_t n, uint32_t ns) -> int {
+    FH_HIP(hipMemsetAsync(sky_cursor, 0, 4, ctx->stream));
+    if (sky_st == ctx->stream) { sky_launch(sky_st, sky_full_wgs, px, xy, n, ns); return FH_OK; }
+    if (sky_filler_wgs) {
+      FH_HIP(hipEventRecord(ctx->ev_sky_cursor, ctx->stream));
+      FH_HIP(hipStreamWaitEvent(sky_st, ctx->ev_sky_cursor, 0));
+      sky_launch(sky_st, sky_filler_wgs, px, xy, n, ns);
+    }
+    sky_drain = SkyDrain{px, xy, n, ns, true};
+    return FH_OK;
+  };
+  auto sky_end = [&]() {
+    if (!sky_drain.pending) return;
+    sky_launch(ctx->stream, sky_full_wgs, sky_drain.px, sky_drain.xy, sky_drain.n, sky_drain.n_samples);
+    sky_drain.pending = false;
+  };
   if (n_sky && !guard_blocks) {
-    Span sp(ctx, sky_st, 4);
-    uint32_t sky_grid = grid_for(n_sky);
-    if (ctx->tun.sky_blocks_per_cu && sky_grid > ctx->tun.n_cus * ctx->tun.sky_blocks_per_cu) sky_grid = ctx->tun.n_cus * ctx->tun.sky_blocks_per_cu;
-    if (adaptive) {
-      hipLaunchKernelGGL(k_sky_pixels<true>, dim3(sky_grid), dim3(kBlock), 0, sky_st, fr, L, ctx->d_sample_issued, ctx->d_split[2], ctx->d_split[3], n_sky, n_samples,
-                         (const SkyAdaptive*)ctx->d_sky_adaptive);
-      ctx->sky_taken_pending = true;
-    } else {
-      hipLaunchKernelGGL(k_sky_pixels<false>, dim3(sky_grid), dim3(kBlock), 0, sky_st, fr, L, ctx->d_sample_issued, ctx->d_split[2], ctx->d_split[3], n_sky, n_samples, ctx->d_split_counters + 2);
+    const int rc = sky_begin(ctx->d_split[2], ctx->d_split[3], n_sky, n_samples);
+    if (rc) return rc;
+    if (adaptive) ctx->sky_taken_pending = true;
+    else {
       ctx->stats.paths += (uint64_t)n_sky * n_samples;
       ctx->stats.sky_pixel_samples += (uint64_t)n_sky * n_samples;
     }
@@ -2189,8 +2263,11 @@
     if (stream && reported && reported < w) w = reported;
     return w;
   };
-  const uint32_t wgs_closest = wgs_for(stream_stack_bytes, static_lds_closest, FH_STREAM_BLOCKS_CLOSEST, ctx->occupancy_blocks);
-  const uint32_t wgs_secondary = wgs_for(stream_stack_bytes_secondary, static_lds_secondary, FH_STREAM_BLOCKS > FH_SECONDARY_BLOCKS_HEAVY ? FH_STREAM_BLOCKS : FH_SECONDARY_BLOCKS_HEAVY, ctx->occupancy_blocks_secondary);
+  const uint32_t wgs_cap = n_sky && sky_filler_wgs ? (uint32_t)FH_STREAM_BLOCKS_FILLER : 0xffffu;
+  uint32_t wgs_closest = wgs_for(stream_stack_bytes, static_lds_closest, FH_STREAM_BLOCKS_CLOSEST, ctx->occupancy_blocks);
+  uint32_t wgs_secondary = wgs_for(stream_stack_bytes_secondary, static_lds_secondary, FH_STREAM_BLOCKS > FH_SECONDARY_BLOCKS_HEAVY ? FH_STREAM_BLOCKS : FH_SECONDARY_BLOCKS_HEAVY, ctx->occupancy_blocks_secondary);
+  if (wgs_closest > wgs_cap) wgs_closest = wgs_cap;
+  if (wgs_secondary > wgs_cap) wgs_secondary = wgs_cap;
   const uint32_t stream_grid = tun.n_cus * wgs_closest;
   const uint32_t stream_grid_secondary = tun.n_cus * wgs_secondary;
   const uint32_t spill_entries = stream_entries < stream_need ? stream_need - stream_entries : 0u;
@@ -2223,17 +2300,15 @@
     const uint32_t to_boundary = ctx->adapt_growth == 1u ? ctx->adapt.step - ctx->adapt_total % ctx->adapt.step : adaptive_to_boundary(ctx);
     if (n_round > to_boundary) n_round = to_boundary;
     if (ran && last_slot != 0) FH_HIP(hipStreamWaitEvent(ctx->stream, ctx->ev_acc[last_slot], 0));
+    if (guard_blocks) sky_end();
     if (sky_ran && sky_st != ctx->stream) { FH_HIP(hipEventRecord(ctx->ev_sky, sky_st)); FH_HIP(hipStreamWaitEvent(ctx->stream, ctx->ev_sky, 0)); }
     const int rc = guard_blocks && n_sky ? adaptive_select(ctx, ctx->stream, base_px, base_xy, n_base, &n_px, ctx->d_split[2], ctx->d_split[3], n_sky, &n_sky_round)
                                          : adaptive_select(ctx, ctx->stream, base_px, base_xy, n_base, &n_px);
     if (rc) return rc;
     px_list = ctx->d_active[0]; xy_list = ctx->d_active[1];
     if (n_sky_round) {
-      Span sp(ctx, sky_st, 4);
-      uint32_t sky_grid = grid_for(n_sky_round);
-      if (ctx->tun.sky_blocks_per_cu && sky_grid > ctx->tun.n_cus * ctx->tun.sky_blocks_per_cu) sky_grid = ctx->tun.n_cus * ctx->tun.sky_blocks_per_cu;
-      hipLaunchKernelGGL(k_sky_pixels<true>, dim3(sky_grid), dim3(kBlock), 0, sky_st, fr, L, ctx->d_sample_issued, ctx->d_active[2], ctx->d_active[3], n_sky_round, n_round,
-                         (const SkyAdaptive*)ctx->d_sky_adaptive);
+      const int rc2 = sky_begin(ctx->d_active[2], ctx->d_active[3], n_sky_round, n_round);
+      if (rc2) return rc2;
       ctx->sky_taken_pending = true;
       sky_ran = true;
     }
@@ -2459,6 +2534,7 @@
   if (adaptive && n_px == 0 && n_sky_round == 0) { ctx->adapt_total += n_samples - call_done; break; }
   }
   if (last_slot != 0 && ran) FH_HIP(hipStreamWaitEvent(ctx->stream, ctx->ev_acc[last_slot], 0));
+  sky_end();
   if (n_sky && sky_st != ctx->stream) { FH_HIP(hipEventRecord(ctx->ev_sky, sky_st)); FH_HIP(hipStreamWaitEvent(ctx->stream, ctx->ev_sky, 0)); }
   FH_HIP(hipGetLastError());
   return FH_OK;
```

Measured after the change: 8191 Msamples/s (median of 6 runs). 3.3% higher.
